# adthoms/dcora

Measured on AMD Instinct MI355X. Metric: RBCD iterations/sec, sphere2500 5-agent split, higher is better.
Workload: dtype f64

## Files before the change

### dcora_amd/__init__.py

```python
import ctypes as C
import gzip
import os
import shutil
import tempfile

import numpy as np

from . import capi
from .capi import DcoraError, Dims, ROptParams, ROptResult, RbcdOptions, F, unF, check

__all__ = ["QuadraticProblem", "QuadraticOptimizer", "ROptParameters", "Dataset", "Csr", "RbcdSession", "RaRbcdSession", "DcoraError",
           "build_Q_pgo", "dual_certificate", "is_psd", "min_eig", "fast_verification", "manifold_project",
           "device_count"]


def device_count():
    return capi.lib().dcora_device_count()


class Csr:

    def __init__(self, n, rp, ci, v):
        self.n = int(n)
        self.rp = np.ascontiguousarray(rp, dtype=np.int32)
# ... 521 lines not shown
        a = np.ascontiguousarray(agents, dtype=np.int32)
        check(capi.lib().dcora_rbcd_iterate_set(self.h, a, a.size, int(allow_adjacent)))

    def set_acceleration(self, on):
        check(capi.lib().dcora_rbcd_set_acceleration(self.h, int(bool(on))))

    def colours(self):
        col, nc = np.zeros(self.R, np.int32), C.c_int()
        check(capi.lib().dcora_rbcd_agent_colours(self.h, col, C.byref(nc)))
        return col, nc.value

    def evaluate(self):
        c2, gn, nxt = C.c_double(), C.c_double(), C.c_int()
        bn = np.zeros(self.R)
        check(capi.lib().dcora_rbcd_evaluate(self.h, C.byref(c2), C.byref(gn), bn.ctypes.data_as(C.c_void_p),
                                             C.byref(nxt)))
        return c2.value, gn.value, bn, nxt.value

    def run(self, max_iters=1000, rgrad_tol=0.1):
        it = C.c_int()
        cost, gn = np.zeros(max_iters), np.zeros(max_iters)
        sel = np.zeros(max_iters, np.int32)
        check(capi.lib().dcora_rbcd_run(self.h, max_iters, rgrad_tol, C.byref(it), cost.ctypes.data_as(C.c_void_p),
                                        gn.ctypes.data_as(C.c_void_p), sel.ctypes.data_as(C.c_void_p)))
        n = it.value
        return dict(iters=n, cost=cost[:n], gradnorm=gn[:n], selected=sel[:n])

    def run_coloured(self, max_sweeps=1000, rgrad_tol=0.1):
        return _run_coloured(capi.lib().dcora_rbcd_run_coloured, self.h, max_sweeps, rgrad_tol)

    def last_result(self):
        r = ROptResult()
        check(capi.lib().dcora_rbcd_last_result(self.h, C.byref(r)))
        return r.as_dict()

    def update_weights(self, reset_to_initial=False):
        c = np.zeros(3, np.int32)
        check(capi.lib().dcora_rbcd_update_weights(self.h, int(bool(reset_to_initial)), c.ctypes.data_as(C.c_void_p)))
        return {"accepted": int(c[0]), "rejected": int(c[1]), "undecided": int(c[2])}

    def set_weights(self, w):
        w = np.ascontiguousarray(w, np.float64)
        if w.shape != (self.m,):
            raise ValueError("set_weights needs one weight per measurement")
        check(capi.lib().dcora_rbcd_set_weights(self.h, w))

    def get_weights(self):
        w = np.zeros(self.m)
        check(capi.lib().dcora_rbcd_get_weights(self.h, w))
        return w

    def robust_info(self):
        mu, n = C.c_double(), C.c_int()
        check(capi.lib().dcora_rbcd_robust_info(self.h, C.byref(mu), C.byref(n)))
        return {"mu": mu.value, "updates": n.value}

    def X_device_ptr(self):
        p = C.c_void_p()
        check(capi.lib().dcora_rbcd_X_device_ptr(self.h, C.byref(p)))
        return p.value

    def public_count(self, agent):
        c = C.c_int()
        check(capi.lib().dcora_rbcd_public_count(self.h, agent, C.byref(c)))
        return c.value

    def public_indices(self, agent):
        idx = np.zeros(max(self.public_count(agent), 1), np.int32)
        check(capi.lib().dcora_rbcd_public_indices(self.h, agent, idx))
        return idx[:self.public_count(agent)]

    def pack_public_dev(self, agent, ptr):
        check(capi.lib().dcora_rbcd_pack_public_dev(self.h, agent, C.c_void_p(ptr)))

    def unpack_public_dev(self, agent, ptr):
        check(capi.lib().dcora_rbcd_unpack_public_dev(self.h, agent, C.c_void_p(ptr)))

    def phase_nonselected(self, selected):
        check(capi.lib().dcora_rbcd_phase_nonselected(self.h, selected))

    def phase_selected(self, selected):
        check(capi.lib().dcora_rbcd_phase_selected(self.h, selected))

    def phase_evaluate_dev(self, ptr):
        check(capi.lib().dcora_rbcd_phase_evaluate_dev(self.h, C.c_void_p(ptr)))

    def synchronize(self):
        check(capi.lib().dcora_rbcd_synchronize(self.h))

    def profile_tcg_runs(self, enable=True):
        check(capi.lib().dcora_rbcd_profile_tcg_runs(self.h, int(enable)))

    def profile_tcg_read(self):
        out = np.zeros(2)
        check(capi.lib().dcora_rbcd_profile_tcg_read(self.h, out))
        return {"launches": int(out[0]), "total_us": float(out[1])}


class Exchange:
    IPC, STAGED = 1, 2

    def __init__(self, session, job_name, _handle=None):
        self.s = session
        self.h = C.c_void_p()
        if _handle is not None:
            self.h = _handle
            return
        create = capi.lib().dcora_exchange_create_ra if isinstance(session, RaRbcdSession) else capi.lib().dcora_exchange_create
        check(create(session.h, job_name.encode(), C.byref(self.h)))

    def close(self):
        if getattr(self, "h", None):
            capi.lib().dcora_exchange_destroy(self.h)
            self.h = None

    def __del__(self):
        try:
            self.close()
        except Exception:
            pass

    def info(self):
        v = np.zeros(10)
        check(capi.lib().dcora_exchange_info(self.h, v))
        return dict(transport={1: "ipc peer stores", 2: "shared host segment"}.get(int(v[0]), "?"), mode=int(v[0]),
                    halo_finegrained=bool(v[8]), wait="device (the scatter kernel polls the flag)" if v[9] else "host spin",
                    peers=int(v[1]), posts=int(v[2]), waits=int(v[3]), bytes_posted=float(v[4]), post_s=float(v[5]),
                    wait_s=float(v[6]), eval_wait_s=float(v[7]))

    def link_report(self):
        v = np.zeros(4)
        check(capi.lib().dcora_exchange_link_report(self.h, v))
        return dict(rounds=int(v[0]), gave_up_device_wait=bool(v[1]), gave_up_ipc=bool(v[2]), last_round_us=float(v[3]))

    def all_ready(self, ready):
        out = C.c_int()
        check(capi.lib().dcora_exchange_all_ready(self.h, int(bool(ready)), C.byref(out)))
        return bool(out.value)

    def certify(self, Q, eta, k):
        cert, dist = C.c_int(), C.c_int()
        th, lm, mv = C.c_double(), C.c_double(), C.c_longlong()
        v = np.zeros(k)
        if Q is None:
            check(capi.lib().dcora_exchange_certify(self.h, k, None, None, None, eta, C.byref(cert), C.byref(th),
                                                    C.byref(lm), v, C.byref(mv), C.byref(dist)))
        else:
            check(capi.lib().dcora_exchange_certify(self.h, k, Q.rp.ctypes.data, Q.ci.ctypes.data, Q.v.ctypes.data, eta,
                                                    C.byref(cert), C.byref(th), C.byref(lm), v, C.byref(mv),
                                                    C.byref(dist)))
        return bool(cert.value), th.value, lm.value, v, mv.value, bool(dist.value)

    def post(self, agents):
        a = np.ascontiguousarray(agents, dtype=np.int32)
        check(capi.lib().dcora_exchange_post(self.h, a, a.size))

    def wait(self, agents):
        a = np.ascontiguousarray(agents, dtype=np.int32)
        check(capi.lib().dcora_exchange_wait(self.h, a, a.size))

    def _eval(self, fn, *first):
        c2, gn, nxt = C.c_double(), C.c_double(), C.c_int()
        bn = np.zeros(self.s.R)
        check(fn(self.h, *first, C.byref(c2), C.byref(gn), bn.ctypes.data_as(C.c_void_p), C.byref(nxt)))
        return c2.value, gn.value, bn, nxt.value

# ... 316 lines not shown
```

### dcora_amd/capi.py

```python
import ctypes as C
import os
import subprocess

import numpy as np

_HERE = os.path.dirname(os.path.abspath(__file__))
LIB_PATH = os.path.join(_HERE, "lib", "libdcora_hip.so")
HEADER_PATH = os.path.join(os.path.dirname(_HERE), "include", "dcora_hip.h")


class DcoraError(RuntimeError):
    def __init__(self, status, msg):
        super().__init__("dcora status %d: %s" % (status, msg))
        self.status = status


class Dims(C.Structure):
    _fields_ = [("r", C.c_int), ("d", C.c_int), ("n", C.c_int), ("l", C.c_int), ("b", C.c_int), ("layout", C.c_int)]


LAYOUT_AUTO, LAYOUT_SE, LAYOUT_RA = 0, 1, 2


class ROptParams(C.Structure):
# ... 78 lines not shown
    "dcora_csr_copy": (C.c_int, [_vp, _ip, _ip, _dp]),
    "dcora_csr_destroy": (C.c_int, [_vp]),
    "dcora_cert_dual_matrix": (C.c_int, [C.POINTER(Dims), _dp, _ip, _ip, _dp, C.c_int, C.POINTER(_vp)]),
    "dcora_cert_is_psd": (C.c_int, [C.c_int, _ip, _ip, _dp, C.c_int, _PI]),
    "dcora_cert_is_psd_device": (C.c_int, [C.c_int, _ip, _ip, _dp, C.c_int, C.c_int, _PI, _dp]),
    "dcora_chol_host_selftest": (C.c_int, [C.c_int, _ip, _ip, _dp, C.c_int, _PI, _PD, _dp]),
    "dcora_chol_cache_clear": (C.c_int, []),
    "dcora_cert_min_eig": (C.c_int, [C.c_int, _ip, _ip, _dp, C.c_int, C.c_double, C.c_int, C.c_ulonglong, C.c_int,
                                     _PD, _dp, C.POINTER(C.c_long)]),
    "dcora_cert_fast_verification": (C.c_int, [C.c_int, _ip, _ip, _dp, C.c_double, C.c_int, C.c_int, _PI, _PD, _dp,
                                               _PD]),
    "dcora_cert_lambda_min_certified": (C.c_int, [C.c_int, _ip, _ip, _dp, C.c_double, C.c_int, C.c_int, _PD, _PI]),
    "dcora_cert_suboptimality_gap": (C.c_int, [C.POINTER(Dims), _dp, C.c_double, _PD, _PD]),
    "dcora_dataset_load_g2o": (C.c_int, [C.c_char_p, C.POINTER(_vp)]),
    "dcora_dataset_create": (C.c_int, [C.c_int, C.c_int, C.c_int, _ip, _dp, C.POINTER(_vp)]),
    "dcora_dataset_info": (C.c_int, [_vp, _PI, _PI, _PI]),
    "dcora_dataset_copy": (C.c_int, [_vp, _ip, _dp]),
    "dcora_dataset_destroy": (C.c_int, [_vp]),
    "dcora_dataset_chordal_init": (C.c_int, [_vp, _dp]),
    "dcora_dataset_chordal_init_device": (C.c_int, [_vp, C.c_int, _dp]),
    "dcora_graph_build_Q_pgo": (C.c_int, [C.c_int, C.c_int, C.c_int, C.c_int, _ip, _dp, C.POINTER(_vp)]),
    "dcora_radataset_load_pyfg": (C.c_int, [C.c_char_p, C.POINTER(_vp)]),
    "dcora_radataset_info": (C.c_int, [_vp, _ip]),
    "dcora_radataset_create": (C.c_int, [C.c_int] * 5 + [_vp, _vp, C.c_int, _vp, _vp, C.c_int, _vp, _vp, _vp, C.POINTER(_vp)]),
    "dcora_radataset_copy": (C.c_int, [_vp] * 7),
    "dcora_radataset_ground_truth": (C.c_int, [_vp, _dp]),
    "dcora_radataset_build_Q": (C.c_int, [_vp, C.POINTER(_vp)]),
    "dcora_radataset_odometry_init": (C.c_int, [_vp, C.c_ulonglong, _dp]),
    "dcora_radataset_ownership": (C.c_int, [_vp, _vp, _vp, _vp]),
    "dcora_radataset_agent_columns": (C.c_int, [_vp, C.c_int, _ip, _vp, _PI]),
    "dcora_radataset_agent_colours": (C.c_int, [_vp, _ip, _PI]),
    "dcora_graph_extract_agent_blocks": (C.c_int, [C.c_int, _ip, _ip, _dp, C.c_int, _ip, C.POINTER(_vp),
                                                   C.POINTER(_vp)]),
    "dcora_radataset_destroy": (C.c_int, [_vp]),
    "dcora_graph_precond_regularization": (C.c_int, [C.c_int, _ip, _ip, _dp, C.c_int, _PD]),
    "dcora_rbcd_options_default": (None, [C.POINTER(RbcdOptions)]),
    "dcora_rbcd_create": (C.c_int, [_vp, C.POINTER(RbcdOptions), C.POINTER(_vp)]),
    "dcora_rbcd_destroy": (C.c_int, [_vp]),
    "dcora_rbcd_set_X": (C.c_int, [_vp, _dp]),
    "dcora_rbcd_get_X": (C.c_int, [_vp, _dp]),
    "dcora_rbcd_iterate": (C.c_int, [_vp, C.c_int, _PD, _PD, _vp, _PI]),
    "dcora_rbcd_run": (C.c_int, [_vp, C.c_int, C.c_double, _PI, _vp, _vp, _vp]),
    "dcora_rbcd_iterate_set": (C.c_int, [_vp, _ip, C.c_int, C.c_int]),
    "dcora_rbcd_set_acceleration": (C.c_int, [_vp, C.c_int]),
    "dcora_rbcd_agent_colours": (C.c_int, [_vp, _ip, _PI]),
    "dcora_rbcd_run_coloured": (C.c_int, [_vp, C.c_int, C.c_double, _PI, _vp, _vp]),
    "dcora_rbcd_evaluate": (C.c_int, [_vp, _PD, _PD, _vp, _PI]),
    "dcora_rbcd_agent_iterate": (C.c_int, [_vp, C.c_int, C.c_int]),
    "dcora_rbcd_agent_get_X": (C.c_int, [_vp, C.c_int, _dp]),
    "dcora_rbcd_agent_set_X": (C.c_int, [_vp, C.c_int, _dp]),
    "dcora_rbcd_agent_update_neighbor": (C.c_int, [_vp, C.c_int, C.c_int, C.c_int, _ip, _dp, C.c_int]),
    "dcora_rbcd_agent_last_skipped": (C.c_int, [_vp, C.c_int, _PI]),
    "dcora_rbcd_agent_info": (C.c_int, [_vp, C.c_int, _PI, _PI, _PI]),
    "dcora_rbcd_last_result": (C.c_int, [_vp, C.POINTER(ROptResult)]),
    "dcora_rbcd_profile_tcg_runs": (C.c_int, [_vp, C.c_int]),
    "dcora_rbcd_profile_tcg_read": (C.c_int, [_vp, _dp]),
    "dcora_rbcd_create_robust": (C.c_int, [_vp, C.POINTER(RbcdOptions), C.POINTER(RobustParams), _vp, C.POINTER(_vp)]),
    "dcora_rbcd_update_weights": (C.c_int, [_vp, C.c_int, _vp]),
    "dcora_rbcd_set_weights": (C.c_int, [_vp, _dp]),
    "dcora_rbcd_get_weights": (C.c_int, [_vp, _dp]),
    "dcora_rbcd_robust_info": (C.c_int, [_vp, _PD, _PI]),
    "dcora_rbcd_create_robust_ranks": (C.c_int, [_vp, C.POINTER(RbcdOptions), C.POINTER(RobustParams), _vp, C.c_char_p,
                                                 C.POINTER(_vp), C.POINTER(_vp)]),
    "dcora_team_params_default": (None, [C.POINTER(TeamParams)]),
    "dcora_team_ready_to_terminate": (C.c_int, [C.POINTER(TeamParams), C.c_int, C.c_int, C.c_int, C.c_double, C.c_int,
                                                C.c_int, C.c_int, _PI]),
    "dcora_team_decide": (C.c_int, [C.POINTER(TeamParams), C.c_int, C.c_int, C.c_int, C.c_int, C.c_int,
                                    C.POINTER(AgentStatus), _vp, _vp, C.c_int, _PI, _PI]),
    "dcora_max_translation_distance": (C.c_int, [C.c_int, C.c_int, C.c_int, _dp, _dp, _PD]),
    "dcora_rbcd_team_enable": (C.c_int, [_vp, C.POINTER(TeamParams)]),
    "dcora_rbcd_agent_status": (C.c_int, [_vp, C.c_int, C.POINTER(AgentStatus), _PI]),
    "dcora_rbcd_loop_closure_stats": (C.c_int, [_vp, C.c_int, _ip]),
    "dcora_rbcd_should_terminate": (C.c_int, [_vp, _PI]),
    "dcora_rbcd_should_update_weights": (C.c_int, [_vp, _PI]),
    "dcora_rbcd_team_info": (C.c_int, [_vp, _ip]),
    "dcora_rbcd_run_team": (C.c_int, [_vp, _PI, _vp, _vp, _vp, _vp, _PI, _PI]),
    "dcora_rbcd_X_device_ptr": (C.c_int, [_vp, C.POINTER(_vp)]),
    "dcora_rbcd_public_count": (C.c_int, [_vp, C.c_int, _PI]),
    "dcora_rbcd_public_indices": (C.c_int, [_vp, C.c_int, _ip]),
    "dcora_rbcd_pack_public_dev": (C.c_int, [_vp, C.c_int, _vp]),
    "dcora_rbcd_unpack_public_dev": (C.c_int, [_vp, C.c_int, _vp]),
    "dcora_rbcd_phase_nonselected": (C.c_int, [_vp, C.c_int]),
    "dcora_rbcd_phase_selected": (C.c_int, [_vp, C.c_int]),
    "dcora_rbcd_phase_evaluate_dev": (C.c_int, [_vp, _vp]),
    "dcora_rbcd_synchronize": (C.c_int, [_vp]),
    "dcora_exchange_create": (C.c_int, [_vp, C.c_char_p, C.POINTER(_vp)]),
    "dcora_exchange_destroy": (C.c_int, [_vp]),
    "dcora_exchange_create_ra": (C.c_int, [_vp, C.c_char_p, C.POINTER(_vp)]),
    "dcora_exchange_info": (C.c_int, [_vp, _dp]),
    "dcora_exchange_link_report": (C.c_int, [_vp, _dp]),
    "dcora_exchange_post": (C.c_int, [_vp, _ip, C.c_int]),
    "dcora_exchange_wait": (C.c_int, [_vp, _ip, C.c_int]),
    "dcora_exchange_evaluate": (C.c_int, [_vp, _PD, _PD, _vp, _PI]),
    "dcora_exchange_rbcd_iterate": (C.c_int, [_vp, C.c_int, _PD, _PD, _vp, _PI]),
    "dcora_exchange_rbcd_tick": (C.c_int, [_vp, _ip, C.c_int, C.c_int]),
    "dcora_exchange_run_coloured": (C.c_int, [_vp, C.c_int, C.c_double, _PI, _vp, _vp]),
    "dcora_exchange_set_X": (C.c_int, [_vp, _dp]),
    "dcora_exchange_gather_X": (C.c_int, [_vp, _dp]),
    "dcora_exchange_barrier": (C.c_int, [_vp]),
    "dcora_exchange_all_ready": (C.c_int, [_vp, C.c_int, _PI]),
    "dcora_exchange_update_weights": (C.c_int, [_vp, C.c_int, _vp]),
    "dcora_exchange_set_weights": (C.c_int, [_vp, _dp]),
    "dcora_exchange_get_weights": (C.c_int, [_vp, _dp]),
    "dcora_exchange_certify": (C.c_int, [_vp, C.c_int, _vp, _vp, _vp, C.c_double, _PI, _PD, _PD, _dp,
                                         C.POINTER(C.c_longlong), _PI]),
    "dcora_exchange_host_selftest": (C.c_int, [C.c_char_p, C.c_int, C.c_int, C.c_int, C.c_int, _PD]),
    "dcora_debug_exchange_leave_stale": (C.c_int, [C.c_char_p, C.c_int, C.c_int]),
    "dcora_debug_exchange_probe_fault": (C.c_int, [C.c_int]),
    "dcora_cert_prepare": (C.c_int, [C.POINTER(Dims), _ip, _ip, C.c_int, C.c_int]),
    "dcora_debug_tcg_run_fault": (C.c_int, [C.c_int]),
    "dcora_debug_tcg_run_fault_at": (C.c_int, [C.c_int, C.c_int]),
    "dcora_problem_solver_info": (C.c_int, [_vp, _dp]),
    "dcora_ra_rbcd_create": (C.c_int, [_vp, C.POINTER(RbcdOptions), C.POINTER(_vp)]),
    "dcora_ra_rbcd_destroy": (C.c_int, [_vp]),
    "dcora_ra_rbcd_info": (C.c_int, [_vp, _PI, _vp]),
    "dcora_ra_rbcd_set_X": (C.c_int, [_vp, _dp]),
    "dcora_ra_rbcd_get_X": (C.c_int, [_vp, _dp]),
    "dcora_ra_rbcd_iterate": (C.c_int, [_vp, C.c_int, _PD, _PD, _vp, _PI]),
    "dcora_ra_rbcd_evaluate": (C.c_int, [_vp, _PD, _PD, _vp, _PI]),
    "dcora_ra_rbcd_run": (C.c_int, [_vp, C.c_int, C.c_double, _PI, _vp, _vp, _vp]),
    "dcora_ra_rbcd_iterate_set": (C.c_int, [_vp, _ip, C.c_int, C.c_int]),
    "dcora_ra_rbcd_set_acceleration": (C.c_int, [_vp, C.c_int]),
    "dcora_ra_rbcd_agent_colours": (C.c_int, [_vp, _ip, _PI]),
    "dcora_ra_rbcd_run_coloured": (C.c_int, [_vp, C.c_int, C.c_double, _PI, _vp, _vp]),
    "dcora_ra_rbcd_last_result": (C.c_int, [_vp, C.POINTER(ROptResult)]),
    "dcora_problem_time_qapply": (C.c_int, [_vp, C.c_int, _PD, _PD]),
    "dcora_problem_time_qapply_rotating": (C.c_int, [C.POINTER(_vp), C.c_int, C.c_int, _PD]),
    "dcora_problem_qapply_info": (C.c_int, [_vp, _dp]),
    "dcora_problem_time_precond": (C.c_int, [_vp, C.c_int, _PD, _PD]),
    "dcora_problem_precond_info": (C.c_int, [_vp, _dp]),
    "dcora_precond_cache_info": (C.c_int, [_dp]),
    "dcora_precond_cache_clear": (C.c_int, []),
    "dcora_robust_params_default": (None, [C.POINTER(RobustParams)]),
    "dcora_robust_weights": (C.c_int, [C.POINTER(RobustParams), C.c_int, C.c_int, _dp, _dp]),
    "dcora_chi2inv": (C.c_int, [C.c_double, C.c_int, _PD]),
    "dcora_robust_error_threshold_at_quantile": (C.c_int, [C.c_double, C.c_int, _PD]),
    "dcora_robust_single_rotation_averaging": (C.c_int, [C.c_int, C.c_int, _dp, _vp, C.c_double, _dp, _ip]),
    "dcora_robust_single_pose_averaging": (C.c_int, [C.c_int, C.c_int, _dp, _dp, _vp, _vp, C.c_double, _dp, _dp, _ip]),
    "dcora_agent_neighbor_transforms": (C.c_int, [C.c_int, C.c_int, _ip, _dp, _dp, _dp, _dp, _dp]),
    "dcora_agent_robust_neighbor_transform": (C.c_int, [C.c_int, C.c_int, _dp, C.c_int, C.c_int, _dp, _PI, _PI]),
    "dcora_log_trajectory": (C.c_int, [C.c_char_p, C.c_int, C.c_int, _dp]),
    "dcora_fixed_stiefel_variable": (C.c_int, [C.c_int, C.c_int, _dp]),
    "dcora_agent_initialize_in_global_frame": (C.c_int, [C.POINTER(Dims), _dp, _dp, _dp, _dp]),
    "dcora_measurement_errors": (C.c_int, [_vp, C.c_int, _dp, _dp, C.c_int]),
    "dcora_solve_pgo": (C.c_int, [_vp, C.POINTER(ROptParams), _vp, _dp, C.POINTER(ROptResult), C.c_int]),
    "dcora_solve_robust_pgo": (C.c_int, [_vp, C.POINTER(ROptParams), C.POINTER(RobustParams), _vp, _vp, _dp, _vp,
                                         C.c_int]),
    "dcora_round_align_trajectory": (C.c_int, [C.POINTER(Dims), _dp, _vp, C.c_int, _dp, _vp, _vp, C.c_int]),
    "dcora_round_project_solution_raslam": (C.c_int, [C.POINTER(Dims), _dp, _dp, C.c_int]),
}

_lib = None


def lib():
    global _lib
    if _lib is None:
        if not os.path.exists(LIB_PATH):
            raise DcoraError(-1, "libdcora_hip.so is not built (run __graft_entry__.build()); there is no fallback")
        L = C.CDLL(LIB_PATH)
        for name, (res, args) in SIGNATURES.items():
            fn = getattr(L, name)
            fn.restype = res
            fn.argtypes = args
        _lib = L
    return _lib
# ... 26 lines not shown
```

### dcora_amd/csrc/capi.hip

```cpp
#include <cstdio>
#include <cstring>
#include <new>

#include "../../include/dcora_hip.h"
#include "cert.h"
#include "device_chol.h"
#include "device_problem.h"
#include "host_graph.h"
#include "host_threads.h"
#include "ra_rbcd.h"
#include "rbcd.h"
#include "precond_cache.h"
#include "exchange.h"
#include "host_robust.h"
#include "robust.h"
#include "round.h"

namespace dcora {
const std::string &get_last_error();
}
using namespace dcora;

struct dcora_problem_s {
  DeviceProblem p;
// ... 1137 lines not shown
    const int rc = team_session(s);
    if (rc) return rc;
    if (!agent_ok(s, agent)) return bad("bad agent");
    for (int c = 0; c < 3; ++c) counts[c] = s->s.team->lc[(size_t)agent * 3 + c];
    return (int)DCORA_OK;
  });
}
int dcora_rbcd_should_terminate(dcora_rbcd_t s, int *yes) {
  return abi_call({s, yes}, [&] {
    const int rc = team_session(s);
    return rc ? rc : s->s.team_decide(yes, nullptr);
  });
}
int dcora_rbcd_should_update_weights(dcora_rbcd_t s, int *yes) {
  return abi_call({s, yes}, [&] {
    const int rc = team_session(s);
    return rc ? rc : s->s.team_decide(nullptr, yes);
  });
}
int dcora_rbcd_team_info(dcora_rbcd_t s, int info[4]) {
  return abi_call({s, info}, [&] {
    const int rc = team_session(s);
    if (rc) return rc;
    info[0] = s->s.team_inner_iter();
    info[1] = s->s.team->latest_weight_update_iteration;
    info[2] = s->s.team_weight_updates();
    info[3] = s->s.team->resets_done;
    return (int)DCORA_OK;
  });
}
int dcora_rbcd_run_team(dcora_rbcd_t s, int *iters_done, double *cost2_trace, double *gradnorm_trace,
                        int *selected_trace, int *updated_trace, int *weight_updates, int *stop_reason) {
  return abi_call({s}, [&] {
    const int rc = team_session(s);
    return rc ? rc
              : s->s.run_team(iters_done, cost2_trace, gradnorm_trace, selected_trace, updated_trace, weight_updates,
                              stop_reason);
  });
}
int dcora_rbcd_last_result(dcora_rbcd_t s, dcora_ropt_result *res) {
  return abi_call({s, res}, [&] { return s->s.last_result(res); });
}
int dcora_rbcd_X_device_ptr(dcora_rbcd_t s, double **X_dev) {
  return abi_call({s, X_dev}, [&] {
    *X_dev = s->s.Xg.p;
    return DCORA_OK;
  });
}
int dcora_rbcd_public_count(dcora_rbcd_t s, int agent, int *count) {
  return abi_call({s, count}, [&] {
    if (!agent_ok(s, agent)) return bad("bad agent");
    *count = (int)s->s.agents[agent].public_poses.size();
    return (int)DCORA_OK;
  });
}
int dcora_rbcd_public_indices(dcora_rbcd_t s, int agent, int *idx) {
  return abi_call({s, idx}, [&] {
    if (!agent_ok(s, agent)) return bad("bad agent");
    const auto &v = s->s.agents[agent].public_poses;
    std::copy(v.begin(), v.end(), idx);
    return (int)DCORA_OK;
  });
}
int dcora_rbcd_pack_public_dev(dcora_rbcd_t s, int agent, double *packed_dev) {
  return abi_call({s}, [&] {
    if (!agent_ok(s, agent)) return bad("bad agent");
    if (!packed_dev && !s->s.agents[agent].public_poses.empty()) return bad("null argument");
    return s->s.pack_public(agent, packed_dev);
  });
}
int dcora_rbcd_unpack_public_dev(dcora_rbcd_t s, int agent, const double *packed_dev) {
  return abi_call({s}, [&] {
    if (!agent_ok(s, agent)) return bad("bad agent");
    if (!packed_dev && !s->s.agents[agent].public_poses.empty()) return bad("null argument");
    return s->s.unpack_public(agent, packed_dev);
  });
}
int dcora_rbcd_phase_nonselected(dcora_rbcd_t s, int selected) {
  return abi_call({s}, [&] { return s->s.phase_nonselected(selected); });
}
int dcora_rbcd_phase_selected(dcora_rbcd_t s, int selected) {
  return abi_call({s}, [&] { return s->s.phase_selected(selected); });
}
int dcora_rbcd_phase_evaluate_dev(dcora_rbcd_t s, double *out_dev) {
  return abi_call({s, out_dev}, [&] { return s->s.phase_evaluate_dev(out_dev); });
}
int dcora_rbcd_profile_tcg_runs(dcora_rbcd_t s, int enable) {
  return abi_call({s}, [&] {
    for (auto &a : s->s.agents)
      if (a.prob) a.prob->profile_tcg_runs = enable != 0;
    return DCORA_OK;
  });
}
int dcora_rbcd_profile_tcg_read(dcora_rbcd_t s, double *out2) {
  return abi_call({s, out2}, [&] {
    out2[0] = out2[1] = 0;
    for (auto &a : s->s.agents) {
      if (!a.prob) continue;
      double n = 0, us = 0;
      const int rc = a.prob->profile_tcg_read(&n, &us);
      if (rc) return rc;
      out2[0] += n;
      out2[1] += us;
    }
    return (int)DCORA_OK;
  });
}
int dcora_rbcd_synchronize(dcora_rbcd_t s) {
  return abi_call({s}, [&]() -> int {
    DCORA_HIP(hipStreamSynchronize(s->s.st));
    return DCORA_OK;
  });
}

int dcora_exchange_create(dcora_rbcd_t s, const char *job_name, dcora_exchange_t *out) {
  return abi_call({s, job_name, out}, [&] {
    return create(out, [&](dcora_exchange_s &h) { return h.e.init(&s->s, job_name); });
  });
}
int dcora_exchange_destroy(dcora_exchange_t ex) {
  delete ex;
  return DCORA_OK;
}
int dcora_exchange_info(dcora_exchange_t ex, double *info) {
  return abi_call({ex, info}, [&] {
    const Exchange &e = ex->e;
    info[0] = e.mode;
    info[1] = e.num_peers();
    info[2] = (double)e.posts;
    info[3] = (double)e.waits;
    info[4] = e.bytes_posted;
    info[5] = e.post_s;
    info[6] = e.wait_s;
    info[7] = e.eval_wait_s;
    info[8] = e.halo_is_finegrained() ? 1 : 0;
    info[9] = e.waits_on_device() ? 1 : 0;
    return DCORA_OK;
  });
}
int dcora_debug_exchange_probe_fault(int rounds) {
  g_probe_fault_rounds.store(rounds);
  return DCORA_OK;
}
int dcora_exchange_link_report(dcora_exchange_t ex, double *out4) {
  return abi_call({ex, out4}, [&] {
    const Exchange &e = ex->e;
    out4[0] = e.link_rounds;
    out4[1] = e.link_gave_up_device_wait;
    out4[2] = e.link_gave_up_ipc;
    out4[3] = e.link_last_us;
    return DCORA_OK;
  });
}
int dcora_exchange_post(dcora_exchange_t ex, const int *agents, int count) {
  return abi_call({ex}, [&] { return !agents && count > 0 ? bad("null argument") : ex->e.post(agents, count); });
}
int dcora_exchange_wait(dcora_exchange_t ex, const int *agents, int count) {
  return abi_call({ex}, [&] { return !agents && count > 0 ? bad("null argument") : ex->e.wait(agents, count); });
}
int dcora_exchange_evaluate(dcora_exchange_t ex, double *cost2, double *gradnorm, double *block_norms,
                            int *next_selected) {
  return abi_call({ex}, [&] { return ex->e.evaluate(cost2, gradnorm, block_norms, next_selected); });
}
int dcora_exchange_rbcd_iterate(dcora_exchange_t ex, int selected, double *cost2, double *gradnorm,
                                double *block_norms, int *next_selected) {
  return abi_call({ex}, [&] { return ex->e.rbcd_iterate(selected, cost2, gradnorm, block_norms, next_selected); });
// ... 454 lines not shown
```

### dcora_amd/csrc/device_problem.h

```cpp
#pragma once
#include <hip/hip_runtime.h>

#include <functional>
#include <memory>
#include <string>
#include <vector>

#include "../../include/dcora_hip.h"
#include "host_sparse.h"
#include "kernels.h"
#include "sparse_precond.h"

namespace dcora {

void set_last_error(const std::string &s);
int hip_fail(hipError_t e, const char *what, const char *file, int line);
#define DCORA_HIP(call)                                                        \
  do {                                                                         \
    hipError_t e_ = (call);                                                    \
    if (e_ != hipSuccess) return ::dcora::hip_fail(e_, #call, __FILE__, __LINE__); \
  } while (0)

template <class T>
struct DevBuf {
// ... 84 lines not shown

struct SpImage {
  int k = 0, npieces = 0;
  long nnzL = 0, nmwaves_total = 0;
  double weights_per_apply = 0, rows_total = 0;
  std::vector<SpLevel> levels;
  DevBuf<double> vals;
  DevBuf<int> idxs, perm, out_off;
  DevBuf<MWave> mwaves;
  int nhub = 0;
  long hub_nnz = 0;
  DevBuf<int> hub_idx;
  DevBuf<double> hub_U, hub_Sinv;
  DevBuf<int> in_pos, out_pos;
  int upload(const PartInvHost &P, struct DeviceWeightSink *streamed = nullptr);
  size_t device_bytes() const;
};

struct DeviceWeightSink : WeightSink {
  explicit DeviceWeightSink(int device_) : device(device_) {}
  ~DeviceWeightSink() override;
  bool fill_on_device(const std::vector<partinv::Fill> &fills, long long total, const std::vector<MirrorRange> &mirrors,
                      int nthreads) override;
  bool wants_device_sources() const override;
  bool begin(long long total) override;
  long long chunk_cap() const override { return kChunk; }
  double *acquire(long long n) override;
  bool commit(long long off, long long n) override;
  bool end() override;
  static constexpr long long kChunk = 8ll << 20;
  static constexpr int kBuffers = 3;
  int device;
  DevBuf<double> vals;
  hipStream_t st = nullptr;
  double *pin[kBuffers] = {nullptr, nullptr, nullptr};
  hipEvent_t ev[kBuffers] = {nullptr, nullptr, nullptr};
  bool busy[kBuffers] = {false, false, false};
  int cur = -1;
};

class SparsePrecond {
 public:
  std::shared_ptr<const SpImage> im;
  int rcap = 0;
  DevBuf<double> y, hub_w, hub_x2;
  double weights_per_apply = 0;
  bool foldable() const { return im && im->nhub == 0 && im->in_pos.p != nullptr; }
  SpFold fold() const {
    SpFold f;
    if (foldable()) {
      f.y = y.p;
      f.in_pos = im->in_pos.p;
      f.out_pos = im->out_pos.p;
    }
    return f;
  }
  SpFold fold_generic() const;
  int attach(std::shared_ptr<const SpImage> image, int rcap);
  int launches() const { return (int)im->levels.size() + 2; }
  void apply(hipStream_t st, int r, Buf2 R, double *Z, Gate g, bool levels_only = false,
             const std::function<bool()> *after_first = nullptr) const;
  double bytes_per_apply(int r) const;
};

int stream_acquire(int device, hipStream_t *out);
void stream_release(int device, hipStream_t st);
int host_flags_acquire(HostFlags **host, HostFlags **dev, int *slot);
void host_flags_release(HostFlags *host, int slot);

int precond_prebuild_dense(const std::vector<const HostCsr *> &Qs, double reg, int block, int device);

class DeviceProblem {
 public:
  ManiDesc m{};
  int device = 0;
  hipStream_t st = nullptr;
  bool own_stream = false;
  DevCsr Q;
  DevBsr Qb;
  bool has_bsr = false;
  int enq_qapply(Buf2 X, int selX, const double *Gp, Buf2 Y, int selY, double *partials, Gate g);
  DevBuf<double> G;
  bool has_G = false;
  DevBuf<double> Minv;
  int ldm = 0;
  SparsePrecond sp;
  std::shared_ptr<const DevBuf<double>> Minv_shared;
  bool precond_cache_hit = false;
  bool sparse_precond = false;
  bool has_precond = false;
  double precond_setup_ms = 0;
  long precond_nnzL = 0;

  DevBuf<double> X0, X1, EG0, EG1, RG0, RG1, S0, S1;
  DevBuf<double> delta, eta, Heta, res, z, Hd, W, Zt;
  DevBuf<double> delta2, res2, Zpart;
  bool tcg_run_ok = false;
  bool concurrent_solves = false;
  DevBuf<unsigned> tcg_sync;
  bool profile_tcg_runs = false;
  std::vector<hipEvent_t> run_events;
  size_t run_events_used = 0;
  int profile_tcg_read(double *launches, double *total_us);
  bool fused = false;
  bool group = false;
  DevBuf<double> pA, pB, pC, p1, p2, p3, scal;
  DevBuf<SolverCtl> ctl;
  DevBuf<double> arena;
  int hf_slot = -1;
  HostFlags *hf = nullptr;
  HostFlags *hf_dev = nullptr;
  std::vector<double> stage;

  long nelem() const { return (long)m.r * m.k; }
  Buf2 Xb() const { return Buf2{{X0.p, X1.p}}; }
  Buf2 EGb() const { return Buf2{{EG0.p, EG1.p}}; }
  Buf2 RGb() const { return Buf2{{RG0.p, RG1.p}}; }
  Buf2 Sb() const { return Buf2{{S0.p, S1.p}}; }

  ~DeviceProblem();
  int init(const dcora_dims &dims, const HostCsr &Qh, const double *Gh, double reg, int device_, hipStream_t shared);
  int set_G_host(const double *Gh);
  int build_preconditioner(const HostCsr &Qh, double reg);
  int set_values(const HostCsr &Q_on_pattern, hipStream_t stream, std::vector<double> *stage);

  int npA() const { return has_bsr ? spmm_bsr_grid(m.n) : spmm_grid(m.k, m.r) + Q.n_long; }
  int npPose() const { return pose_grid(m); }
  int enq_rgrad(Buf2 X, Buf2 EG, Buf2 RG, Buf2 S, int sel, double *partials, Gate g, double *posenorm = nullptr);
  int enq_retract(Buf2 X, const double *V, double alpha, Buf2 out, int selOut, Buf2 grad, const double *HV,
                  double *partials, Gate g);
  int npVec() const { return vec_grid(nelem()); }
  void enqueue_egrad(const double *X, double *EG, double *partials);
  void enqueue_precond(const double *X, const double *V, double *out);
  void enq_minv(Buf2 R, double *Z, const double *p2, int np2, Gate g);

  int cost(const double *Xh, double *f);
  int eucgrad(const double *Xh, double *out);
  int riegrad(const double *Xh, double *out, double *norm);
  int hessvec(const double *Xh, const double *Vh, double *out);
  int hessvec_solver_form(const double *Xh, const double *Vh, double *out, double *dots);
  bool hess_one_launch() const;
  int precondition(const double *Xh, const double *Vh, double *out);
  int retract(const double *Xh, const double *Vh, double *out);
  int tangent_project(const double *Xh, const double *Vh, double *out);
  int optimize(const dcora_ropt_params &prm, const double *X0h, double *Xout, dcora_ropt_result *res);
  int escape_saddle(const double *Xopt, double theta, const double *v, double gtol, double pgtol, bool second_order,
                    double *Xout, int *success);

  int optimize_dev(const dcora_ropt_params &prm);
  int fetch_result(dcora_ropt_result *res);
  Buf2 result_pick(const SolverCtl **c) const;
  int result(double **X);
  int eval_dev(const double *Xd, double *f, double *gradnorm);

  int time_qapply(int reps, double *avg_ms, double *bytes);
  int time_precond(int reps, double *avg_ms, double *bytes);
  bool use_pc() const;

 private:
  enum class TcgForm { generic, split, pc, run };
  struct RtrForm;
  int rtr_dev(const dcora_ropt_params &prm, TcgForm form);
  int rgd_dev(const dcora_ropt_params &prm);
  int seq_ = 0;
  bool pending_ = false;
  bool rgd_ = false;
  double t0_ms_ = 0;
  dcora_ropt_result last_res_{};
  int cur_after_fetch_ = 0;
  int upload(const double *h, double *d, size_t n);
  int download(const double *d, double *h, size_t n);
};

}
```

### dcora_amd/csrc/device_problem.hip

```cpp
#include <atomic>

#include "device_problem.h"
#include "env.h"
#include "device_chol.h"
#include "host_threads.h"
#include "precond_cache.h"

#include <algorithm>
#include <chrono>
#include <cmath>
#include <cstdio>
#include <cstdlib>
#include <cstring>
#include <map>
#include <mutex>

namespace dcora {

static thread_local std::string g_last_error;
void set_last_error(const std::string &s) { g_last_error = s; }
const std::string &get_last_error() { return g_last_error; }
int hip_fail(hipError_t e, const char *what, const char *file, int line) {
  char buf[512];
  std::snprintf(buf, sizeof buf, "HIP error %d (%s) at %s:%d in %s", (int)e, hipGetErrorString(e), file, line, what);
// ... 546 lines not shown
  for (double &v : neg) v = -v;
  rc = upload(neg.data(), z.p, nelem());
  if (rc) return rc;
  rc = upload(Vh, delta2.p, nelem());
  if (rc) return rc;
  enqueue_egrad(X0.p, EG0.p, nullptr);
  launch_rgrad(st, m, buf1(X0.p), buf1(EG0.p), buf1(RG0.p), buf1(S0.p), 0, pB.p, Gate{});
  DCORA_HIP(hipMemsetAsync(p3.p, 0, sizeof(double), st));
  const int np = launch_spmm_dir_fix(st, m, Q.view(), buf1(X0.p), buf1(S0.p), z.p, delta2.p, delta.p, Hd.p, p3.p, 1, p1.p,
                                     ctl.p, 0, 0);
  std::vector<double> part((size_t)np);
  rc = download(p1.p, part.data(), part.size());
  if (rc) return rc;
  dots[0] = 0;
  for (double v : part) dots[0] += v;
  rc = download(Hd.p, out, nelem());
  if (rc) return rc;
  launch_spmm(st, m.r, Q.view(), buf1(delta.p), 0, nullptr, buf1(W.p), 0, nullptr, Gate{});
  launch_hessfix(st, m, buf1(X0.p), buf1(S0.p), delta.p, W.p, Hd.p, p1.p, Gate{});
  part.assign((size_t)npPose(), 0.0);
  rc = download(p1.p, part.data(), part.size());
  if (rc) return rc;
  dots[1] = 0;
  for (double v : part) dots[1] += v;
  return DCORA_OK;
}
int DeviceProblem::precondition(const double *Xh, const double *Vh, double *out) {
  if (!has_precond) {
    set_last_error("problem has no preconditioner");
    return DCORA_ERR_NO_PRECONDITIONER;
  }
  DCORA_HIP(hipSetDevice(device));
  int rc = upload(Xh, X0.p, nelem());
  if (rc) return rc;
  rc = upload(Vh, res.p, nelem());
  if (rc) return rc;
  enqueue_precond(X0.p, res.p, z.p);
  return download(z.p, out, nelem());
}
int DeviceProblem::retract(const double *Xh, const double *Vh, double *out) {
  DCORA_HIP(hipSetDevice(device));
  int rc = upload(Xh, X0.p, nelem());
  if (rc) return rc;
  rc = upload(Vh, eta.p, nelem());
  if (rc) return rc;
  launch_retract(st, m, buf1(X0.p), eta.p, 1.0, buf1(X1.p), 0, buf1(RG0.p), nullptr, nullptr, Gate{});
  return download(X1.p, out, nelem());
}
int DeviceProblem::tangent_project(const double *Xh, const double *Vh, double *out) {
  DCORA_HIP(hipSetDevice(device));
  int rc = upload(Xh, X0.p, nelem());
  if (rc) return rc;
  rc = upload(Vh, eta.p, nelem());
  if (rc) return rc;
  launch_tangent(st, m, buf1(X0.p), eta.p, z.p, nullptr, nullptr, nullptr, 0, nullptr, nullptr, 0, 0, 0);
  return download(z.p, out, nelem());
}

int DeviceProblem::eval_dev(const double *Xd, double *f, double *gradnorm) {
  enqueue_egrad(Xd, EG1.p, pA.p);
  launch_rgrad(st, m, buf1(Xd), buf1(EG1.p), Buf2{{nullptr, nullptr}}, Buf2{{nullptr, nullptr}}, 0, pB.p, Gate{});
  launch_sum_partials(st, pA.p, npA(), 2, 2, scal.p);
  launch_sum_partials(st, pB.p, npPose(), 1, 1, scal.p + 2);
  double s[3];
  int rc = download(scal.p, s, 3);
  if (rc) return rc;
  if (f) *f = 0.5 * s[0] + s[1];
  if (gradnorm) *gradnorm = std::sqrt(s[2]);
  return DCORA_OK;
}

int DeviceProblem::optimize(const dcora_ropt_params &prm, const double *X0h, double *Xout, dcora_ropt_result *res_out) {
  DCORA_HIP(hipSetDevice(device));
  int rc = upload(X0h, X0.p, nelem());
  if (rc) return rc;
  double *X = nullptr;
  if ((rc = optimize_dev(prm)) || (rc = result(&X)) || (rc = fetch_result(res_out))) return rc;
  return download(X, Xout, nelem());
}

int DeviceProblem::optimize_dev(const dcora_ropt_params &prm) {
  pending_ = false;
  rgd_ = prm.method != 0;
  if (rgd_) return rgd_dev(prm);
  if (!has_precond) {
    set_last_error("RTR requires the preconditioner (ref src/QuadraticProblem.cpp:78-82)");
    return DCORA_ERR_NO_PRECONDITIONER;
  }
  TcgForm form = TcgForm::generic;
  if (fused) form = !use_pc() ? TcgForm::split : (tcg_run_ok && !concurrent_solves) ? TcgForm::run : TcgForm::pc;
  return rtr_dev(prm, form);
}

int DeviceProblem::fetch_result(dcora_ropt_result *res_out) {
  if (pending_) {
    SolverCtl h;
    DCORA_HIP(hipMemcpyAsync(&h, ctl.p, sizeof h, hipMemcpyDeviceToHost, st));
    DCORA_HIP(hipStreamSynchronize(st));
    DCORA_HIP(hipGetLastError());
    const double now = std::chrono::duration<double, std::milli>(std::chrono::steady_clock::now().time_since_epoch())
                           .count();
    cur_after_fetch_ = h.cur & 1;
    last_res_.success = 1;
    last_res_.fInit = h.fInit;
    last_res_.gradNormInit = h.gradNormInit;
    last_res_.fOpt = h.f1;
    last_res_.gradNormOpt = h.ngf;
    last_res_.elapsedMs = now - t0_ms_;
    last_res_.tCGStatus = h.tcg_status;
    last_res_.outer_iterations = h.outer_it;
    last_res_.inner_iterations = h.inner_total;
    last_res_.accepted_steps = h.accepted;
    pending_ = false;
  }
  if (res_out) *res_out = last_res_;
  return DCORA_OK;
}

Buf2 DeviceProblem::result_pick(const SolverCtl **c) const {
  *c = rgd_ ? nullptr : ctl.p;
  return rgd_ ? buf1(X1.p) : Xb();
}

int DeviceProblem::result(double **X) {
  const int rc = fetch_result(nullptr);
  if (rc) return rc;
  *X = cur_after_fetch_ ? X1.p : X0.p;
  return DCORA_OK;
}

int DeviceProblem::rgd_dev(const dcora_ropt_params &prm) {
  const auto t0 = std::chrono::steady_clock::now();
  double f0 = 0, g0 = 0;
  int rc = eval_dev(X0.p, &f0, &g0);
  if (rc) return rc;
  enqueue_egrad(X0.p, EG0.p, nullptr);
  launch_rgrad(st, m, buf1(X0.p), buf1(EG0.p), buf1(RG0.p), buf1(S0.p), 0, pB.p, Gate{});
  const double *dir = RG0.p;
  if (prm.RGD_use_preconditioner) {
    if (!has_precond) {
      set_last_error("RGD with preconditioning requested but the problem has none");
      return DCORA_ERR_NO_PRECONDITIONER;
    }
    enqueue_precond(X0.p, RG0.p, z.p);
    dir = z.p;
  }
  launch_retract(st, m, buf1(X0.p), dir, -prm.RGD_stepsize, buf1(X1.p), 0, buf1(RG0.p), nullptr, nullptr, Gate{});
  double f1 = 0, g1 = 0;
  rc = eval_dev(X1.p, &f1, &g1);
  if (rc) return rc;
  last_res_.success = 1;
  last_res_.fInit = f0;
  last_res_.gradNormInit = g0;
  last_res_.fOpt = f1;
  last_res_.gradNormOpt = g1;
  last_res_.elapsedMs = std::chrono::duration<double, std::milli>(std::chrono::steady_clock::now() - t0).count();
  last_res_.tCGStatus = TR_MAXITER;
  last_res_.outer_iterations = 1;
  last_res_.inner_iterations = 0;
  last_res_.accepted_steps = 1;
  cur_after_fetch_ = 1;
  return DCORA_OK;
}

namespace {
template <class Pred>
bool spin_until(Pred p, double timeout_s) {
  const auto t0 = std::chrono::steady_clock::now();
  unsigned it = 0;
  while (!p()) {
    if ((++it & 1023u) == 0) {
      if (std::chrono::duration<double>(std::chrono::steady_clock::now() - t0).count() > timeout_s) return false;
    }
// ... 1 lines not shown
    __builtin_ia32_pause();
#endif
  }
  return true;
}
}

int DeviceProblem::profile_tcg_read(double *launches, double *total_us) {
  DCORA_HIP(hipSetDevice(device));
  DCORA_HIP(hipStreamSynchronize(st));
  double us = 0;
  for (size_t i = 0; i + 1 < run_events_used; i += 2) {
    float ms = 0;
    if (hipEventElapsedTime(&ms, run_events[i], run_events[i + 1]) == hipSuccess) us += 1e3 * ms;
  }
  *launches = (double)(run_events_used / 2);
  *total_us = us;
  run_events_used = 0;
  return DCORA_OK;
}

bool DeviceProblem::use_pc() const {
  const int forced = env::solver_bc();
  if (sparse_precond || !has_precond) return false;
  if (forced < 0) return false;
  if (!forced && !fused_pc_preferred(m, ldm)) return false;
  return fused_pc_ready(m, ldm);
}

struct DeviceProblem::RtrForm {
  DeviceProblem &p;
  TcgForm form;
  int &seq;
  const int solve_first;
  SolverCtl *const c;
  const CsrDev Qv;
  const BsrDev Qbv;
  const double *const Gp;
  const long N;
  const int nA, nP, nV, nPB;
  const bool sparse;
  const SpFold sfg;
  const bool hess_fused;
  const int nPG;
  const double *const Mi;
  const bool folded;
  const SpFold sf;
  const int nsl;
  const int nZ;
  const bool gf, gfb;
  unsigned *const sync_p;
  const int nsync;
  double *const dbuf[2];
  double *const rbuf[2];

  RtrForm(DeviceProblem &p_, TcgForm f, int &seq_)
      : p(p_), form(f), seq(seq_), solve_first(seq_ + 1), c(p.ctl.p), Qv(p.Q.view()),
        Qbv(p.has_bsr ? p.Qb.view() : BsrDev{}), Gp(p.has_G ? p.G.p : nullptr), N(p.nelem()), nA(p.npA()),
        nP(p.npPose()), nV(p.npVec()), nPB(fused_pose_blocks(p.m)), sparse(p.sparse_precond),
        sfg(f == TcgForm::generic && sparse ? p.sp.fold_generic() : SpFold()),
        hess_fused(f == TcgForm::generic && p.hess_one_launch()),
        nPG(sparse ? fused_update_grid(p.m) : fused_precond_grid(p.m)), Mi(sparse ? nullptr : p.Minv.p),
        folded(sparse && p.sp.foldable()), sf(folded ? p.sp.fold() : SpFold{}), nsl(sparse ? 1 : -1),
        nZ(f == TcgForm::pc || f == TcgForm::run ? fused_pc_blocks(p.m) : nPB),
        gf(f != TcgForm::generic && !p.has_bsr && p.Q.n_long == 0), gfb(f != TcgForm::generic && p.has_bsr),
        sync_p(f == TcgForm::run ? p.tcg_sync.p : nullptr), nsync(f == TcgForm::run ? tcg_run_sync_words() : 0),
        dbuf{p.delta.p, p.delta2.p}, rbuf{p.res.p, p.res2.p} {}

  bool outer_done() const { return p.hf->outer_done_seq >= solve_first; }
  bool stopped(int tcg_first) const { return p.hf->tcg_done_seq >= tcg_first || outer_done(); }
  int nAe() const { return gf ? nPB : nA; }

  int eval(int sel) {
    const auto g = [&] {
      ++seq;
      return sel ? Gate{c, seq, 1} : Gate{};
    };
    const Buf2 kNoBuf{{nullptr, nullptr}};
    if (form == TcgForm::generic) {
      p.enq_qapply(p.Xb(), sel, Gp, p.EGb(), sel, p.pA.p, g());
      launch_rgrad(p.st, p.m, p.Xb(), p.EGb(), p.RGb(), p.Sb(), sel, p.pB.p, g());
      return nP;
    }
    if (gf) return launch_fused_grad(p.st, p.m, Qv, p.Xb(), Gp, p.EGb(), p.RGb(), p.Sb(), sel, p.pA.p, p.pB.p, nullptr, g());
    if (gfb)
      return launch_fused_grad_bsr(p.st, p.m.r, p.m.d, Qbv, p.Xb(), Gp, kNoBuf, p.RGb(), p.Sb(), sel, p.pA.p, p.pB.p,
                                   nullptr, g());
    p.enq_qapply(p.Xb(), sel, Gp, p.EGb(), sel, p.pA.p, g());
    return p.enq_rgrad(p.Xb(), p.EGb(), p.RGb(), p.Sb(), sel, p.pB.p, g());
  }

  int first() {
    switch (form) {
      case TcgForm::generic: {
        launch_tcg_begin(p.st, N, p.RGb(), p.eta.p, p.Heta.p, p.res.p, c, ++seq);
        const int s = seq;
        p.enq_minv(buf1(p.res.p), p.Zt.p, nullptr, 0, Gate{c, ++seq, 1});
        launch_tangent(p.st, p.m, p.Xb(), p.Zt.p, p.z.p, p.res.p, p.p3.p, nullptr, 0, c, p.hf_dev, ++seq, 1, 0);
        return s;
      }
      case TcgForm::run: {
        const int s = launch_run();
        if (s != 0) return s;
        p.tcg_run_ok = false;
        form = TcgForm::pc;
      }
        [[fallthrough]];
      case TcgForm::pc:
        if (launch_fused_pc(p.st, p.m, p.ldm, Mi, p.RGb(), p.Xb(), nullptr, nullptr, p.eta.p, p.Heta.p, nullptr, rbuf[0],
                            p.z.p, nullptr, 0, p.p3.p, c, p.hf_dev, ++seq, 0, 1) < 0) {
          set_last_error("k_fused_pc could not be launched on this device");
          return -1;
        }
        return seq;
      case TcgForm::split:
        launch_fused_precond(p.st, p.m, p.ldm, Mi, p.RGb(), nullptr, nullptr, p.eta.p, p.Heta.p, nullptr, rbuf[0],
                             p.Zpart.p, nullptr, 0, p.p2.p, c, p.hf_dev, ++seq, 0, 1, sf);
        return seq;
    }
    return -1;
  }
  int launch_run() {
    hipEvent_t e1 = nullptr;
    if (p.profile_tcg_runs) {
      while (p.run_events.size() < p.run_events_used + 2) {
        hipEvent_t e = nullptr;
        if (hipEventCreate(&e) != hipSuccess) {
          set_last_error("hipEventCreate failed (k_tcg_run profile)");
          return -1;
        }
        p.run_events.push_back(e);
      }
      (void)hipEventRecord(p.run_events[p.run_events_used], p.st);
      e1 = p.run_events[p.run_events_used + 1];
      p.run_events_used += 2;
    }
    if (launch_tcg_run(p.st, p.m, p.ldm, Mi, Qv, p.RGb(), p.Xb(), p.Sb(), dbuf[0], dbuf[1], p.Hd.p, p.eta.p, p.Heta.p,
                       p.z.p, p.p1.p, p.p3.p, p.pC.p, p.tcg_sync.p, c, p.hf_dev, ++seq) < 0) {
      if (e1) p.run_events_used -= 2;
      return 0;
    }
    if (e1) (void)hipEventRecord(e1, p.st);
    return seq;
  }
  void rest(bool rejected) {
    if (form != TcgForm::split) return;
    if (sparse && rejected) {
      launch_fused_finish(p.st, p.m, p.Xb(), p.W.p, rbuf[0], p.z.p, nullptr, 0, p.p3.p, c, p.hf_dev, ++seq, 0, 1, 1,
                          SpFold{});
      return;
    }
    if (sparse) p.sp.apply(p.st, p.m.r, buf1(rbuf[0]), p.Zpart.p, Gate{c, ++seq, 1}, folded);
    launch_fused_finish(p.st, p.m, p.Xb(), p.Zpart.p, rbuf[0], p.z.p, nullptr, 0, p.p3.p, c, p.hf_dev, ++seq, 0, 1, nsl,
                        sf, sparse ? p.W.p : nullptr);
  }

  int replay(Buf2 R, double *Z, bool levels_only, int tcg_first) {
    const int seq_step = seq;
    bool timed = false;
    const std::function<bool()> verdict = [&]() {
      if (!spin_until([&] { return p.hf->go_seq >= seq_step || stopped(tcg_first); }, 20.0)) {
        timed = true;
        return false;
      }
      return !stopped(tcg_first);
    };
    p.sp.apply(p.st, p.m.r, R, Z, Gate{c, ++seq, 2}, levels_only, &verdict);
// ... 276 lines not shown
```

### dcora_amd/csrc/env.cpp

```cpp
#include "env.h"

#include <cstdlib>
#include <cstring>

namespace dcora {
namespace env {
namespace {
bool is(const char *name, const char *value) {
  const char *e = std::getenv(name);
  return e && std::strcmp(e, value) == 0;
}
}

bool init_timing() {
  static const bool v = std::getenv("DCORA_INIT_TIMING") != nullptr;
  return v;
}
int precond_mode() {
  return is("DCORA_PRECOND", "dense") ? 1 : is("DCORA_PRECOND", "sparse") ? 2 : 0;
}
bool generic_solver() {
  return is("DCORA_SOLVER", "generic");
}
int solver_tcg() {
  return is("DCORA_SOLVER_TCG", "launch") ? -1 : is("DCORA_SOLVER_TCG", "run") ? 1 : 0;
}
int solver_bc() {
  static const int v = is("DCORA_SOLVER_BC", "pc") ? 1 : is("DCORA_SOLVER_BC", "split") ? -1 : 0;
  return v;
}
bool factor_on_host() {
  static const bool v = is("DCORA_FACTOR", "host");
  return v;
}
bool fill_on_host() {
  static const bool v = is("DCORA_SP_FILL", "host");
  return v;
}
bool lanczos_sync() {
  static const bool v = is("DCORA_LANCZOS", "sync");
  return v;
}
int host_threads() {
  static const int v = [] {
    const char *e = std::getenv("DCORA_HOST_THREADS");
    return e ? (std::atoi(e) > 0 ? std::atoi(e) : 1) : 0;
  }();
  return v;
}
double precond_cache_mb() {
  static const double v = [] {
    const char *e = std::getenv("DCORA_PRECOND_CACHE_MB");
    return e ? std::atof(e) : 8192.0;
  }();
  return v;
}
const char *exchange() {
  static const char *v = std::getenv("DCORA_EXCHANGE");
  return v;
}
const char *exchange_wait() {
  static const char *v = std::getenv("DCORA_EXCHANGE_WAIT");
  return v;
}
double exchange_timeout_s() {
  static const double v = [] {
    const char *e = std::getenv("DCORA_EXCHANGE_TIMEOUT_S");
    const double x = e ? std::atof(e) : 0.0;
    return x > 0 ? x : 120.0;
  }();
  return v;
}

}
}
```

### dcora_amd/csrc/env.h

```cpp
#pragma once

namespace dcora {
namespace env {

bool init_timing();
int precond_mode();
bool generic_solver();
int solver_tcg();
int solver_bc();
bool factor_on_host();
bool fill_on_host();
bool lanczos_sync();
int host_threads();
double precond_cache_mb();
const char *exchange();
const char *exchange_wait();
double exchange_timeout_s();

}
}
```

### dcora_amd/csrc/kernels.h

```cpp
#pragma once
#include <hip/hip_runtime.h>

#include <atomic>
#include <climits>
#include <vector>

namespace dcora {

constexpr int kMaxPartials = 1024;
constexpr int kBsrMaxGrid = 4096;
constexpr int kBlock = 256;

struct ManiDesc {
  int r, d, n, l, b, k, se;
  __host__ __device__ int rot_col(int i) const { return se ? i * (d + 1) : i * d; }
  __host__ __device__ int sphere_col(int i) const { return d * n + i; }
  __host__ __device__ int num_euc() const { return se ? n : n + b; }
  __host__ __device__ int euc_col(int e) const { return se ? e * (d + 1) + d : d * n + l + e; }
};
inline ManiDesc make_mani(int r, int d, int n, int l, int b, int layout = 0) {
  ManiDesc m;
  m.r = r; m.d = d; m.n = n; m.l = l; m.b = b;
  m.se = (layout == 2) ? 0 : ((l == 0 && b == 0) ? 1 : 0);
  m.k = (d + 1) * n + l + b;
  return m;
}
template <class Dims>
inline ManiDesc make_mani(const Dims &dims) {
  return make_mani(dims.r, dims.d, dims.n, dims.l, dims.b, dims.layout);
}

constexpr int kLongSplit = 8;
constexpr int kLongRow = 512;
struct CsrDev {
  int nrows = 0;
  int nnz = 0;
  const int *rp = nullptr;
  const int *ci = nullptr;
  const double *v = nullptr;
  int n_long = 0;
  const int *long_rows = nullptr;
  double *long_part = nullptr;
  int *long_cnt = nullptr;
};

struct BsrDev {
  int nbrows = 0;
  int nblocks = 0;
  const int *bp = nullptr;
  const int *bc = nullptr;
  const double *bv = nullptr;
};

struct Buf2 {
  double *p[2];
};
inline Buf2 buf1(double *x) { return Buf2{{x, x}}; }
inline Buf2 buf1(const double *x) { return Buf2{{const_cast<double *>(x), const_cast<double *>(x)}}; }

struct SolverCtl {
  double f1, ngf, Delta, maxDelta, tol, f2, rho, fInit, gradNormInit;
  int cur;
  int outer_it, max_outer, accepted, last_accepted, stop_on_accept;
  int outer_done_stamp;
  double z_r[2], d_Pd[2], e_Pe[2], e_Pd[2];
  double alpha, e_Pe_n, norm_r0;
  int tcg_done_stamp, tcg_status, tcg_iters, inner_total, max_inner;
};
enum TcgStatus : int { TR_NEGCURVTURE = 0, TR_EXCREGION = 1, TR_LCON = 2, TR_SCON = 3, TR_MAXITER = 4 };
constexpr int kMaxAgents = 64;
struct EvalOut {
  double cost2, gradnorm;
  double block_norms[kMaxAgents];
  int next;
  volatile int seq;
};
struct HostFlags {
  volatile int last_seq_done;
  volatile int tcg_done_seq;
  volatile int outer_done_seq;
  volatile int go_seq;
  volatile int reject_seq;
  volatile int tcg_abort_seq;
};

struct Gate {
  const SolverCtl *ctl = nullptr;
  int seq = 0;
  int gate = 0;
};

int spmm_grid(int nrows, int r);
int spmm_dir_fix_grid(const ManiDesc &m, int nrows);
int launch_spmm_dir_fix(hipStream_t st, const ManiDesc &m, const CsrDev &A, Buf2 X, Buf2 Sblk, const double *z,
                        const double *d_old, double *d_new, double *Hd, const double *p3, int np3, double *p1,
                        SolverCtl *ctl, int seq, int iter);
void launch_spmm_dir(hipStream_t st, int r, const CsrDev &A, const double *z, const double *d_old, double *d_new,
                     double *W, const double *p3, int np3, SolverCtl *ctl, int seq, int iter);
inline int spmm_slots(const CsrDev &A, int r) { return spmm_grid(A.nrows, r) + A.n_long; }
void launch_spmm(hipStream_t st, int r, const CsrDev &A, Buf2 X, int selX, const double *G, Buf2 Y, int selY,
                 double *partials, Gate g);

int spmm_bsr_grid(int nbrows);
void launch_spmm_bsr(hipStream_t st, int r, int d, const BsrDev &A, Buf2 X, int selX, const double *G, Buf2 Y,
                     int selY, double *partials, Gate g);

int pose_grid(const ManiDesc &m);
void launch_rgrad(hipStream_t st, const ManiDesc &m, Buf2 X, Buf2 EG, Buf2 RG, Buf2 Sblk, int sel,
                  double *partials, Gate g);
struct SpFold {
  double *y = nullptr;
  const int *in_pos = nullptr, *out_pos = nullptr;
  int h = 0;
  const int *hub_idx = nullptr;
  const double *hub_U = nullptr, *hub_x2 = nullptr;
};
void launch_tangent(hipStream_t st, const ManiDesc &m, Buf2 X, const double *V, double *out, const double *R,
                    double *partials, const double *p2, int np2, SolverCtl *ctl, HostFlags *hf, int seq,
                    int gate, int iter, SpFold sf = SpFold());
void launch_hessfix(hipStream_t st, const ManiDesc &m, Buf2 X, Buf2 Sblk, const double *V, const double *W,
                    double *HV, double *partials, Gate g);
void launch_retract(hipStream_t st, const ManiDesc &m, Buf2 X, const double *V, double alpha, Buf2 out,
                    int selOut, Buf2 grad, const double *HV, double *partials, Gate g);
void launch_polar(hipStream_t st, const ManiDesc &m, double c0, const double *A, double c1, const double *B,
                  double c2, const double *C, double *out);

void launch_nesterov(hipStream_t st, const ManiDesc &m, int mode, int restart, int skip_lo, int skip_hi, double alpha,
                     double gamma, double *X, double *V, double *Y, double *XPrev, double *Yloc,
                     const double *Xloc);

void launch_dense_apply(hipStream_t st, int r, int k, int ldm, const double *Minv, Buf2 R, double *Z,
                        const double *p2, int np2, Gate g);

int vec_grid(long nelem);
struct CtlInit {
  int enable = 0;
  double tol = 0, Delta = 0, maxDelta = 0;
  int max_outer = 0, stop_on_accept = 0, max_inner = 0;
};
void launch_rtr_init(hipStream_t st, const double *pA, int npA, const double *pB, int npB, SolverCtl *ctl,
                     HostFlags *hf, int seq, CtlInit ci = CtlInit(), unsigned *tcg_sync = nullptr, int nsync = 0);
void launch_tcg_begin(hipStream_t st, long nelem, Buf2 grad, double *eta, double *Heta, double *res,
                      SolverCtl *ctl, int seq);
void launch_tcg_update1(hipStream_t st, long nelem, const double *delta, const double *Hd, double *eta,
                        double *Heta, double *res, const double *p1, int np1, double *p2, SolverCtl *ctl,
                        HostFlags *hf, int seq, int iter, int r = 1, SpFold sf = SpFold());
void launch_tcg_update2(hipStream_t st, long nelem, const double *z, double *delta, const double *p3, int np3,
                        SolverCtl *ctl, HostFlags *hf, int seq, int iter);
void launch_rtr_decide(hipStream_t st, const double *pA, int npA, const double *pB, int npB, const double *pC,
                       int npC, SolverCtl *ctl, HostFlags *hf, int seq, unsigned *tcg_sync = nullptr, int nsync = 0);

void launch_axpby(hipStream_t st, long nelem, double a, const double *x, double b, const double *y, double *out);
void launch_sum_partials(hipStream_t st, const double *partials, int np, int stride, int count, double *out);
void launch_dot(hipStream_t st, long nelem, const double *x, const double *y, double *partials);
void launch_gather_cols(hipStream_t st, int r, int ncols, const int *src_col, const double *X, double *out);
void launch_scatter_cols(hipStream_t st, int r, int ncols, const int *dst_col, const double *in, double *X);
void launch_block_dots(hipStream_t st, int r, int nagents, const int *col_start, const double *A, const double *B,
                       double *out);

void launch_lambda_blocks(hipStream_t st, const ManiDesc &m, const double *X, const double *XQ, double *Lblk);
void launch_lanczos_proj(hipStream_t st, int n, int nv, const double *V, const double *w, double *partials);
void launch_lanczos_sub(hipStream_t st, int n, int nv, const double *V, const double *h, double *w);
constexpr int kLanczosFuseParts = 256;
void launch_lanczos_sub_sum(hipStream_t st, int n, int nv, const double *V, const double *partials, int npart,
                            double *hout, double *w, double *dotpart);
void launch_lanczos_keep(hipStream_t st, int nv, const double *h, double *hout);
constexpr double kLanczosDead = 1e-10;
void launch_lanczos_next(hipStream_t st, int n, const double *partials, int npart, double *beta_out, int *flag,
                         const double *w, double *vnext, const double *hrow, int nv);
void launch_scale_shift(hipStream_t st, int n, double shift, const double *x, double *y);
void launch_scale(hipStream_t st, int n, const double *alpha_dev_inv_sqrt ,
                  const double *w, double *out);

bool fused_supported(const ManiDesc &m);
bool group_supported(const ManiDesc &m);
int fused_pose_blocks(const ManiDesc &m);
int fused_nsplit(const ManiDesc &m);
int fused_precond_grid(const ManiDesc &m);
int fused_update_grid(const ManiDesc &m);
int launch_fused_hess(hipStream_t st, const ManiDesc &m, const CsrDev &Q, const double *z, const double *d_old,
                       double *d_new, Buf2 X, Buf2 S, double *Hd, const double *p3, int np3, double *p1,
                       SolverCtl *ctl, int seq, int iter,
                      const BsrDev *Ab = nullptr );
void launch_fused_precond(hipStream_t st, const ManiDesc &m, int ldm, const double *Minv, Buf2 grad,
                          const double *delta, const double *Hd, double *eta, double *Heta, const double *res_old,
                          double *res_new, double *Zpart, const double *p1, int np1, double *p2, SolverCtl *ctl,
                          HostFlags *hf, int seq, int iter, int first, SpFold sf = SpFold());
int fused_pc_blocks(const ManiDesc &m);
bool tcg_run_supported(const ManiDesc &m, int ldm, int cus, int max_rows_nnz);
int tcg_run_sync_words();
extern std::atomic<int> g_tcg_run_fault;
extern std::atomic<int> g_tcg_run_fault_skip;
int tcg_run_max_rows_nnz(const ManiDesc &m, const int *rowptr);
int launch_tcg_run(hipStream_t st, const ManiDesc &m, int ldm, const double *Minv, const CsrDev &Q, Buf2 grad, Buf2 X,
                   Buf2 S, double *d0, double *d1, double *Hd, double *eta, double *Heta, double *z, double *p1r,
                   double *p3, double *pC, unsigned *sync, SolverCtl *ctl, HostFlags *hf, int seq);
bool fused_pc_preferred(const ManiDesc &m, int ldm);
bool fused_pc_ready(const ManiDesc &m, int ldm);
int launch_fused_pc(hipStream_t st, const ManiDesc &m, int ldm, const double *Minv, Buf2 grad, Buf2 X,
                    const double *delta, const double *Hd, double *eta, double *Heta, const double *res_old,
                    double *res_new, double *z, const double *p1, int np1, double *p3, SolverCtl *ctl, HostFlags *hf,
                    int seq, int iter, int first, double *pC = nullptr );
void launch_fused_finish(hipStream_t st, const ManiDesc &m, Buf2 X, const double *Zpart, const double *res,
                         double *z, const double *p2, int np2, double *p3, SolverCtl *ctl, HostFlags *hf, int seq,
                         int iter, int first, int nsplit = -1 , SpFold sf = SpFold(),
                         double *zraw = nullptr );
int launch_fused_grad_bsr(hipStream_t st, int r, int d, const BsrDev &A, Buf2 X, const double *G, Buf2 EG, Buf2 RG, Buf2 S,
                          int sel, double *pA, double *pB, double *posenorm, Gate g,
                          const int *agent_start = nullptr, int agents = 0, int *wg_per_agent = nullptr);
int launch_fused_grad(hipStream_t st, const ManiDesc &m, const CsrDev &Q, Buf2 X, const double *G, Buf2 EG, Buf2 RG,
                      Buf2 Sblk, int sel, double *pA, double *pB, double *posenorm, Gate g);
int launch_g_rgrad(hipStream_t st, const ManiDesc &m, Buf2 X, Buf2 EG, Buf2 RG, Buf2 Sblk, int sel, double *partials,
                   double *posenorm, Gate g);
void launch_ctl_init(hipStream_t st, SolverCtl *c, double tol, double Delta, double maxDelta, int max_outer,
                     int stop_on_accept, int max_inner);
void launch_eval_finish(hipStream_t st, int R, const int *pose_start, const double *posenorm, const double *pA,
                        int npA, EvalOut *out_dev, int seq, double *split_scratch = nullptr, int nposes = 0,
                        const double *agent_partials = nullptr, int wg_per_agent = 0);
int eval_split_doubles();
struct RelChangeSet {
  int count;
  int agent[kMaxAgents];
};
void launch_rel_change(hipStream_t st, int r, int d, const double *X, const double *XPrev, const int *pose_start,
                       const RelChangeSet &set, double *out);
int max_translation_distance(int r, int d, int n, const double *X, const double *Y, double *out);
int launch_g_retract(hipStream_t st, const ManiDesc &m, Buf2 X, const double *V, double alpha, Buf2 out, int selOut,
                     Buf2 grad, const double *HV, double *partials, Gate g);
void launch_g_nesterov(hipStream_t st, const ManiDesc &m, int mode, int restart, int skip_lo, int skip_hi,
                       double alpha, double gamma, double *X, double *V, double *Y, double *XPrev, double *Yloc,
                       Buf2 Xloc, const SolverCtl *ctl, double *inner_Yloc = nullptr);

#if defined(__HIPCC__)
template <int CTRL>
__device__ __forceinline__ double dpp_move(double v) {
  int lo = __double2loint(v), hi = __double2hiint(v);
  lo = __builtin_amdgcn_update_dpp(0, lo, CTRL, 0xF, 0xF, true);
  hi = __builtin_amdgcn_update_dpp(0, hi, CTRL, 0xF, 0xF, true);
  return __hiloint2double(hi, lo);
}
__device__ __forceinline__ double readlane_f64(double v, int lane) {
  const int lo = __builtin_amdgcn_readlane(__double2loint(v), lane);
  const int hi = __builtin_amdgcn_readlane(__double2hiint(v), lane);
  return __hiloint2double(hi, lo);
}
__device__ __forceinline__ double wave_sum_dpp(double v) {
  v += dpp_move<0xB1>(v);
  v += dpp_move<0x4E>(v);
  v += dpp_move<0x141>(v);
  v += dpp_move<0x140>(v);
  return (readlane_f64(v, 0) + readlane_f64(v, 16)) + (readlane_f64(v, 32) + readlane_f64(v, 48));
}
__device__ __forceinline__ double wave_sum(double v) { return wave_sum_dpp(v); }
__device__ __forceinline__ double block_sum(double v, double *sm) {
  v = wave_sum(v);
  const int w = threadIdx.x >> 6, nw = (blockDim.x + 63) >> 6;
  __syncthreads();
  if ((threadIdx.x & 63) == 0) sm[w] = v;
  __syncthreads();
  double t = 0;
  for (int i = 0; i < nw; ++i) t += sm[i];
  return t;
}
__device__ __forceinline__ double sum_partials(const double *p, int np, int stride, int off, double *sm) {
  double v = 0;
  for (int i = threadIdx.x; i < np; i += blockDim.x) v += p[(size_t)i * stride + off];
  return block_sum(v, sm);
}
__device__ __forceinline__ void host_store(volatile int *p, int v) {
  __hip_atomic_store(const_cast<int *>(p), v, __ATOMIC_RELAXED, __HIP_MEMORY_SCOPE_SYSTEM);
}

__device__ __forceinline__ bool gated(const SolverCtl *ctl, int seq, int gate) {
  if (ctl == nullptr || gate == 0) return false;
  if (seq > ctl->outer_done_stamp) return true;
  if (gate == 2 && seq > ctl->tcg_done_stamp) return true;
  return false;
}
struct GateWords {
  int outer, tcg;
};
__device__ __forceinline__ GateWords gate_words(const SolverCtl *ctl) {
  GateWords w{0x7fffffff, 0x7fffffff};
  if (ctl) {
    w.outer = ctl->outer_done_stamp;
    w.tcg = ctl->tcg_done_stamp;
  }
  return w;
}
__device__ __forceinline__ bool gated(const GateWords &w, const SolverCtl *ctl, int seq, int gate) {
  if (ctl == nullptr || gate == 0) return false;
  if (seq > w.outer) return true;
  if (gate == 2 && seq > w.tcg) return true;
  return false;
// ... 8 lines not shown
```

### dcora_amd/csrc/kernels.hip

```cpp
#include "kernels.h"
#include "tcg_rules.h"

namespace dcora {

template <int N>
__device__ __forceinline__ void sum_partials_n(const double *const (&p)[N], const int (&np)[N], const int (&st)[N],
                                               const int (&off)[N], double *sm, double (&out)[N]) {
  double v[N];
#pragma unroll
  for (int q = 0; q < N; ++q) v[q] = ((int)threadIdx.x < np[q]) ? p[q][(size_t)threadIdx.x * st[q] + off[q]] : 0.0;
#pragma unroll
  for (int q = 0; q < N; ++q)
    for (int i = threadIdx.x + blockDim.x; i < np[q]; i += blockDim.x) v[q] += p[q][(size_t)i * st[q] + off[q]];
#pragma unroll
  for (int q = 0; q < N; ++q) v[q] = wave_sum(v[q]);
  const int w = threadIdx.x >> 6, nw = (blockDim.x + 63) >> 6;
  __syncthreads();
  if ((threadIdx.x & 63) == 0)
#pragma unroll
    for (int q = 0; q < N; ++q) sm[q * 4 + w] = v[q];
  __syncthreads();
#pragma unroll
  for (int q = 0; q < N; ++q) {
    double t = 0;
    for (int i = 0; i < nw; ++i) t += sm[q * 4 + i];
    out[q] = t;
  }
}

int vec_grid(long nelem) {
  long g = (nelem + kBlock - 1) / kBlock;
  if (g < 1) g = 1;
  if (g > kMaxPartials) g = kMaxPartials;
  return (int)g;
}

constexpr int kSpmmTile = 1536;

int spmm_grid(int nrows, int r) {
  const int RB = kBlock / r;
  long nrb = (nrows + RB - 1) / RB;
  if (nrb < 1) nrb = 1;
  if (nrb > kMaxPartials) nrb = kMaxPartials;
  return (int)nrb;
}

template <bool DOTS>
__global__ __launch_bounds__(kBlock) void k_spmm(int r, CsrDev A, Buf2 Xb, int selX, const double *__restrict__ G,
                                                 Buf2 Yb, int selY, double *__restrict__ partials, Gate g,
                                                 int main_grid) {
  if (gated(g.ctl, g.seq, g.gate)) return;
  __shared__ int s_ci[kSpmmTile];
  __shared__ double s_v[kSpmmTile];
  __shared__ double s_red[16];
  const double *__restrict__ X = pick(Xb, g.ctl, selX);
  double *__restrict__ Y = pick(Yb, g.ctl, selY);
  const int RB = kBlock / r;
  const int nrb = (A.nrows + RB - 1) / RB;
  const int lj = threadIdx.x / r, t = threadIdx.x - lj * r;
  double d0 = 0, d1 = 0;
  if ((int)blockIdx.x >= main_grid) {
    const int li = ((int)blockIdx.x - main_grid) / kLongSplit, sl = ((int)blockIdx.x - main_grid) % kLongSplit;
    const int j = A.long_rows[li];
    const int rb0 = A.rp[j], re0 = A.rp[j + 1];
    const int per = (re0 - rb0 + kLongSplit - 1) / kLongSplit;
    const int pb = rb0 + sl * per, pe = min(re0, pb + per);
    double acc = 0;
    if (lj < RB) {
      for (int p = pb + lj; p < pe; p += 8 * RB) {
        int c8[8];
        double w8[8], x8[8];
#pragma unroll
        for (int q = 0; q < 8; ++q) {
          const int pp = p + q * RB;
          const bool ok = pp < pe;
          c8[q] = A.ci[ok ? pp : rb0];
          w8[q] = ok ? A.v[pp] : 0.0;
        }
#pragma unroll
        for (int q = 0; q < 8; ++q) x8[q] = X[(size_t)c8[q] * r + t];
#pragma unroll
        for (int q = 0; q < 8; ++q) acc += w8[q] * x8[q];
      }
    }
    double *s_part = s_v;
    __shared__ int s_last;
    __syncthreads();
    s_part[threadIdx.x] = (lj < RB) ? acc : 0.0;
    __syncthreads();
    if ((int)threadIdx.x < r) {
      double y = 0;
      for (int q = 0; q < RB; ++q) y += s_part[q * r + threadIdx.x];
      __hip_atomic_store(A.long_part + ((size_t)li * kLongSplit + sl) * 16 + threadIdx.x, y, __ATOMIC_RELAXED,
                         __HIP_MEMORY_SCOPE_AGENT);
    }
    __threadfence();
    __syncthreads();
    if (threadIdx.x == 0)
      s_last = (__hip_atomic_fetch_add(A.long_cnt + li, 1, __ATOMIC_ACQ_REL, __HIP_MEMORY_SCOPE_AGENT) ==
                kLongSplit - 1);
    __syncthreads();
    if (!s_last) return;
    if (threadIdx.x == 0) __hip_atomic_store(A.long_cnt + li, 0, __ATOMIC_RELAXED, __HIP_MEMORY_SCOPE_AGENT);
    if ((int)threadIdx.x < r) {
      double y = 0;
      for (int q = 0; q < kLongSplit; ++q)
        y += __hip_atomic_load(A.long_part + ((size_t)li * kLongSplit + q) * 16 + threadIdx.x, __ATOMIC_RELAXED,
                               __HIP_MEMORY_SCOPE_AGENT);
      const size_t o = (size_t)j * r + threadIdx.x;
      if (DOTS) {
        const double x = X[o];
        d0 = y * x;
        if (G) d1 = x * G[o];
      }
      if (G) y += G[o];
      Y[o] = y;
    }
    if (DOTS) {
      const double a = block_sum(d0, s_red);
      const double b = block_sum(d1, s_red);
// ... 396 lines not shown
      kind = (a < D) ? 0 : 2;
    } else if (active && !m.se && j < n_rot_rows + m.l) {
      kind = 1;
      it = j - n_rot_rows;
    }
    __syncthreads();
    s_V[threadIdx.x] = own;
    s_Y[threadIdx.x] = xo;
    __syncthreads();
    double T = acc;
    const int l0 = lj - a;
    if (kind == 0) {
      double sres = 0;
#pragma unroll
      for (int b = 0; b < D; ++b) sres += s_V[(l0 + b) * r + t] * Sblk[(size_t)it * D * D + b + a * D];
      T = acc - sres;
    } else if (kind == 1) {
      T = acc - own * Sblk[(size_t)m.n * D * D + it];
    }
    s_T[threadIdx.x] = T;
    __syncthreads();
    double hv = T;
    if (kind == 0) {
      double sres = 0;
#pragma unroll
      for (int b = 0; b < D; ++b) {
        double pba = 0, pab = 0;
        for (int u = 0; u < r; ++u) {
          pba += s_Y[(l0 + b) * r + u] * s_T[(l0 + a) * r + u];
          pab += s_Y[(l0 + a) * r + u] * s_T[(l0 + b) * r + u];
        }
        sres += s_Y[(l0 + b) * r + t] * (0.5 * (pba + pab));
      }
      hv = T - sres;
    } else if (kind == 1) {
      double yt = 0;
      for (int u = 0; u < r; ++u) yt += s_Y[lj * r + u] * s_T[lj * r + u];
      hv = T - xo * yt;
    }
    if (active && !is_long) {
      Hd[o] = hv;
      d_new[o] = own;
      dacc += own * hv;
    }
  }
  const double tot = block_sum(dacc, s_red);
  if (threadIdx.x == 0) p1[blockIdx.x] = tot;
}

int spmm_dir_fix_grid(const ManiDesc &m, int nrows) {
  const int al = m.se ? m.d + 1 : m.d;
  const int RB = ((kBlock / m.r) / al) * al;
  if (RB < al) return 0;
  long nrb = (nrows + RB - 1) / RB;
  if (nrb < 1) nrb = 1;
  if (nrb > kMaxPartials) nrb = kMaxPartials;
  return (int)nrb;
}

int launch_spmm_dir_fix(hipStream_t st, const ManiDesc &m, const CsrDev &A, Buf2 X, Buf2 Sblk, const double *z,
                        const double *d_old, double *d_new, double *Hd, const double *p3, int np3, double *p1,
                        SolverCtl *ctl, int seq, int iter) {
  const int main_grid = spmm_dir_fix_grid(m, A.nrows);
  const int grid = main_grid + A.n_long * kLongSplit;
  if (m.d == 3)
    hipLaunchKernelGGL(k_spmm_dir_fix<3>, dim3(grid), dim3(kBlock), 0, st, m, A, X, Sblk, z, d_old, d_new, Hd, p3, np3,
                       p1, ctl, seq, iter, main_grid);
  else
    hipLaunchKernelGGL(k_spmm_dir_fix<2>, dim3(grid), dim3(kBlock), 0, st, m, A, X, Sblk, z, d_old, d_new, Hd, p3, np3,
                       p1, ctl, seq, iter, main_grid);
  return main_grid + A.n_long;
}

void launch_spmm_dir(hipStream_t st, int r, const CsrDev &A, const double *z, const double *d_old, double *d_new,
                     double *W, const double *p3, int np3, SolverCtl *ctl, int seq, int iter) {
  const int main_grid = spmm_grid(A.nrows, r);
  const int grid = main_grid + A.n_long * kLongSplit;
  hipLaunchKernelGGL(k_spmm_dir, dim3(grid), dim3(kBlock), 0, st, r, A, z, d_old, d_new, W, p3, np3, ctl, seq, iter,
                     main_grid);
}

void launch_spmm(hipStream_t st, int r, const CsrDev &A, Buf2 X, int selX, const double *G, Buf2 Y, int selY,
                 double *partials, Gate g) {
  const int main_grid = spmm_grid(A.nrows, r);
  const int grid = main_grid + A.n_long * kLongSplit;
  if (partials)
    hipLaunchKernelGGL(k_spmm<true>, dim3(grid), dim3(kBlock), 0, st, r, A, X, selX, G, Y, selY, partials, g,
                       main_grid);
  else
    hipLaunchKernelGGL(k_spmm<false>, dim3(grid), dim3(kBlock), 0, st, r, A, X, selX, G, Y, selY, partials, g,
                       main_grid);
}

template <int D, int RM>
struct Blk {
  double a[D][RM];
};
template <int D, int RM>
__device__ __forceinline__ void ld_blk(const double *__restrict__ p, int r, Blk<D, RM> &B) {
#pragma unroll
  for (int c = 0; c < D; ++c)
#pragma unroll
    for (int t = 0; t < RM; ++t) B.a[c][t] = (t < r) ? p[c * r + t] : 0.0;
}
template <int D, int RM>
__device__ __forceinline__ void st_blk(double *__restrict__ p, int r, const Blk<D, RM> &B) {
#pragma unroll
  for (int c = 0; c < D; ++c)
#pragma unroll
    for (int t = 0; t < RM; ++t)
      if (t < r) p[c * r + t] = B.a[c][t];
}
template <int D, int RM>
__device__ __forceinline__ void sym_gram(const Blk<D, RM> &Y, const Blk<D, RM> &E, double (&S)[D][D]) {
  double P[D][D];
#pragma unroll
  for (int a = 0; a < D; ++a)
#pragma unroll
    for (int b = 0; b < D; ++b) {
      double s = 0;
#pragma unroll
      for (int t = 0; t < RM; ++t) s += Y.a[a][t] * E.a[b][t];
      P[a][b] = s;
    }
#pragma unroll
  for (int a = 0; a < D; ++a)
#pragma unroll
    for (int b = 0; b < D; ++b) S[a][b] = 0.5 * (P[a][b] + P[b][a]);
}
template <int D, int RM>
__device__ __forceinline__ void sub_AS(Blk<D, RM> &V, const Blk<D, RM> &A, const double (&S)[D][D]) {
#pragma unroll
  for (int b = 0; b < D; ++b)
#pragma unroll
    for (int t = 0; t < RM; ++t) {
      double s = 0;
#pragma unroll
      for (int a = 0; a < D; ++a) s += A.a[a][t] * S[a][b];
      V.a[b][t] -= s;
    }
}
template <int D, int RM>
__device__ __forceinline__ double blk_dot(const Blk<D, RM> &A, const Blk<D, RM> &B) {
  double s = 0;
#pragma unroll
  for (int c = 0; c < D; ++c)
#pragma unroll
    for (int t = 0; t < RM; ++t) s += A.a[c][t] * B.a[c][t];
  return s;
}
template <int D, int RM>
__device__ __forceinline__ void qf_blk(Blk<D, RM> &A) {
#pragma unroll
  for (int j = 0; j < D; ++j) {
#pragma unroll
    for (int pass = 0; pass < 2; ++pass)
#pragma unroll
      for (int c = 0; c < D; ++c)
        if (c < j) {
          double s = 0;
#pragma unroll
          for (int t = 0; t < RM; ++t) s += A.a[c][t] * A.a[j][t];
#pragma unroll
          for (int t = 0; t < RM; ++t) A.a[j][t] -= s * A.a[c][t];
        }
    double nn = 0;
// ... 795 lines not shown
    const double h = Hd[i];
    eta[i] += step * delta[i];
    Heta[i] += step * h;
    if (!boundary) {
      const double rr = res[i] + alpha * h;
      res[i] = rr;
      acc += rr * rr;
      if (sf.y) {
        const long col = i / r;
        const int jp = sf.in_pos[col];
        if (jp >= 0) sf.y[(size_t)jp * r + (i - col * r)] = rr;
      }
    }
  }
  const double tot = block_sum(acc, s_red);
  if (threadIdx.x == 0) p2[blockIdx.x] = tot;
  if (blockIdx.x == 0 && threadIdx.x == 0) {
    ctl->alpha = alpha;
    ctl->e_Pe_n = e_Pe_new;
    if (boundary) tcg_end_run(ctl, hf, seq, tcg_boundary_status(d_Hd), iter + 1);
  }
}

__global__ __launch_bounds__(kBlock) void k_tcg_update2(long nelem, const double *__restrict__ z,
                                                        double *__restrict__ delta, const double *__restrict__ p3,
                                                        int np3, SolverCtl *ctl, HostFlags *hf, int seq, int iter) {
  if (gated(ctl, seq, 2)) return;
  __shared__ double s_red[16];
  const int par = iter & 1;
  const double z_r_new = sum_partials(p3, np3, 1, 0, s_red);
  const double beta = tcg_beta(z_r_new, ctl->z_r[par]);
  for (long i = (long)blockIdx.x * kBlock + threadIdx.x; i < nelem; i += (long)gridDim.x * kBlock)
    delta[i] = -z[i] + beta * delta[i];
  if (blockIdx.x == 0 && threadIdx.x == 0) {
    tcg_put_dir(ctl, par ^ 1, tcg_dir_next(z_r_new, beta, ctl->alpha, ctl->d_Pd[par], ctl->e_Pd[par]), ctl->e_Pe_n);
    if (iter + 1 >= ctl->max_inner) tcg_end_run_at_cap(ctl, hf, seq, iter + 1);
    host_store(&hf->last_seq_done, seq);
  }
}

__global__ __launch_bounds__(kBlock) void k_rtr_decide(const double *pA, int npA, const double *pB, int npB,
                                                       const double *pC, int npC, SolverCtl *ctl, HostFlags *hf,
                                                       int seq, unsigned *tcg_sync, int nsync) {
  if (gated(ctl, seq, 1)) return;
  __shared__ double s_red[20];
  for (int i = threadIdx.x; i < nsync; i += kBlock) tcg_sync[i] = 0u;
  const double *const ps[5] = {pA, pA, pB, pC, pC};
  const int nps[5] = {npA, npA, npB, npC, npC}, sts[5] = {2, 2, 1, 2, 2}, offs[5] = {0, 1, 0, 0, 1};
  double sums[5];
  sum_partials_n<5>(ps, nps, sts, offs, s_red, sums);
  const double fq = sums[0], fg = sums[1], g2 = sums[2], eg = sums[3], eh = sums[4];
  if (threadIdx.x == 0) {
    const double f2 = 0.5 * fq + fg;
    const double rho = (ctl->f1 - f2) / (-(eg + 0.5 * eh));
    ctl->f2 = f2;
    ctl->rho = rho;
    if (rho > 0.75) {
      if (ctl->tcg_status == TR_NEGCURVTURE || ctl->tcg_status == TR_EXCREGION) ctl->Delta = fmin(2.0 * ctl->Delta, ctl->maxDelta);
    } else if (rho < 0.25) {
      ctl->Delta *= 0.25;
    }
    const bool accept = (rho > 0.1) && isfinite(rho);
    if (accept) {
      ctl->cur ^= 1;
      ctl->f1 = f2;
      ctl->ngf = sqrt(g2);
      ctl->accepted += 1;
      ctl->last_accepted = 1;
    } else {
      ctl->last_accepted = 0;
      host_store(&hf->reject_seq, seq);
    }
    ctl->outer_it += 1;
    if (ctl->ngf < ctl->tol || ctl->outer_it >= ctl->max_outer || (ctl->stop_on_accept && accept)) {
      ctl->outer_done_stamp = seq;
      host_store(&hf->outer_done_seq, seq);
    }
    host_store(&hf->last_seq_done, seq);
  }
}

void launch_rtr_init(hipStream_t st, const double *pA, int npA, const double *pB, int npB, SolverCtl *ctl,
                     HostFlags *hf, int seq, CtlInit ci, unsigned *tcg_sync, int nsync) {
  hipLaunchKernelGGL(k_rtr_init, dim3(1), dim3(kBlock), 0, st, pA, npA, pB, npB, ctl, hf, seq, ci, tcg_sync, nsync);
}
void launch_tcg_begin(hipStream_t st, long nelem, Buf2 grad, double *eta, double *Heta, double *res,
                      SolverCtl *ctl, int seq) {
  hipLaunchKernelGGL(k_tcg_begin, dim3(vec_grid(nelem)), dim3(kBlock), 0, st, nelem, grad, eta, Heta, res, ctl,
                     seq);
}
void launch_tcg_update1(hipStream_t st, long nelem, const double *delta, const double *Hd, double *eta,
                        double *Heta, double *res, const double *p1, int np1, double *p2, SolverCtl *ctl,
                        HostFlags *hf, int seq, int iter, int r, SpFold sf) {
  hipLaunchKernelGGL(k_tcg_update1, dim3(vec_grid(nelem)), dim3(kBlock), 0, st, nelem, delta, Hd, eta, Heta, res,
                     p1, np1, p2, ctl, hf, seq, iter, r, sf);
}
void launch_tcg_update2(hipStream_t st, long nelem, const double *z, double *delta, const double *p3, int np3,
                        SolverCtl *ctl, HostFlags *hf, int seq, int iter) {
  hipLaunchKernelGGL(k_tcg_update2, dim3(vec_grid(nelem)), dim3(kBlock), 0, st, nelem, z, delta, p3, np3, ctl, hf,
                     seq, iter);
}
void launch_rtr_decide(hipStream_t st, const double *pA, int npA, const double *pB, int npB, const double *pC,
                       int npC, SolverCtl *ctl, HostFlags *hf, int seq, unsigned *tcg_sync, int nsync) {
  hipLaunchKernelGGL(k_rtr_decide, dim3(1), dim3(kBlock), 0, st, pA, npA, pB, npB, pC, npC, ctl, hf, seq, tcg_sync,
                     nsync);
}

__global__ __launch_bounds__(kBlock) void k_axpby(long nelem, double a, const double *__restrict__ x, double b,
                                                  const double *__restrict__ y, double *__restrict__ out) {
  for (long i = (long)blockIdx.x * kBlock + threadIdx.x; i < nelem; i += (long)gridDim.x * kBlock)
    out[i] = a * x[i] + (y ? b * y[i] : 0.0);
}
void launch_axpby(hipStream_t st, long nelem, double a, const double *x, double b, const double *y, double *out) {
  hipLaunchKernelGGL(k_axpby, dim3(vec_grid(nelem)), dim3(kBlock), 0, st, nelem, a, x, b, y, out);
}

__global__ __launch_bounds__(kBlock) void k_sum_partials(const double *partials, int np, int stride, int count,
                                                         double *out) {
  __shared__ double s_red[16];
  for (int c = 0; c < count; ++c) {
    const double s = sum_partials(partials, np, stride, c, s_red);
    if (threadIdx.x == 0) out[c] = s;
  }
}
void launch_sum_partials(hipStream_t st, const double *partials, int np, int stride, int count, double *out) {
  hipLaunchKernelGGL(k_sum_partials, dim3(1), dim3(kBlock), 0, st, partials, np, stride, count, out);
}

__global__ __launch_bounds__(kBlock) void k_dot(long nelem, const double *__restrict__ x,
                                                const double *__restrict__ y, double *__restrict__ partials) {
  __shared__ double s_red[16];
  double acc = 0;
  for (long i = (long)blockIdx.x * kBlock + threadIdx.x; i < nelem; i += (long)gridDim.x * kBlock)
    acc += x[i] * y[i];
  const double t = block_sum(acc, s_red);
  if (threadIdx.x == 0) partials[blockIdx.x] = t;
}
void launch_dot(hipStream_t st, long nelem, const double *x, const double *y, double *partials) {
  hipLaunchKernelGGL(k_dot, dim3(vec_grid(nelem)), dim3(kBlock), 0, st, nelem, x, y, partials);
}

__global__ __launch_bounds__(kBlock) void k_gather_cols(int r, int ncols, const int *__restrict__ src,
                                                        const double *__restrict__ X, double *__restrict__ out) {
  const long N = (long)ncols * r;
  for (long i = (long)blockIdx.x * kBlock + threadIdx.x; i < N; i += (long)gridDim.x * kBlock) {
    const int c = (int)(i / r), t = (int)(i - (long)c * r);
    out[i] = X[(size_t)src[c] * r + t];
  }
}
__global__ __launch_bounds__(kBlock) void k_scatter_cols(int r, int ncols, const int *__restrict__ dst,
                                                         const double *__restrict__ in, double *__restrict__ X) {
  const long N = (long)ncols * r;
  for (long i = (long)blockIdx.x * kBlock + threadIdx.x; i < N; i += (long)gridDim.x * kBlock) {
    const int c = (int)(i / r), t = (int)(i - (long)c * r);
    X[(size_t)dst[c] * r + t] = in[i];
  }
}
void launch_gather_cols(hipStream_t st, int r, int ncols, const int *src_col, const double *X, double *out) {
  if (ncols <= 0) return;
  hipLaunchKernelGGL(k_gather_cols, dim3(vec_grid((long)ncols * r)), dim3(kBlock), 0, st, r, ncols, src_col, X, out);
}
void launch_scatter_cols(hipStream_t st, int r, int ncols, const int *dst_col, const double *in, double *X) {
  if (ncols <= 0) return;
  hipLaunchKernelGGL(k_scatter_cols, dim3(vec_grid((long)ncols * r)), dim3(kBlock), 0, st, r, ncols, dst_col, in, X);
}

__global__ __launch_bounds__(kBlock) void k_block_dots(int r, const int *__restrict__ cs,
                                                       const double *__restrict__ A, const double *__restrict__ B,
                                                       double *__restrict__ out) {
  __shared__ double s_red[16];
  const int a = blockIdx.x;
  const long lo = (long)cs[a] * r, hi = (long)cs[a + 1] * r;
  double s0 = 0, s1 = 0;
  for (long i = lo + threadIdx.x; i < hi; i += kBlock) {
    const double x = A[i];
    s0 += x * x;
    if (B) s1 += x * B[i];
  }
  const double t0 = block_sum(s0, s_red);
  const double t1 = block_sum(s1, s_red);
  if (threadIdx.x == 0) {
    out[2 * a] = t0;
    out[2 * a + 1] = t1;
  }
}
void launch_block_dots(hipStream_t st, int r, int nagents, const int *col_start, const double *A, const double *B,
// ... 123 lines not shown
```

### dcora_amd/csrc/rbcd.h

```cpp
#pragma once
#include <chrono>
#include <functional>
#include <memory>
#include <string>
#include <vector>

#include "device_problem.h"
#include "host_graph.h"
#include "host_robust.h"
#include "robust.h"
#include "session_core.h"
#include "team_rules.h"

namespace dcora {

struct AgentDev : AgentCore {
  int id = 0, n = 0, col0 = 0;
  bool v_feasible = false;
  std::vector<int> public_poses;
  std::vector<int> required;
  bool detached = false;
  DevBuf<double> nbr[2];
  std::vector<char> got[2];
  bool last_skipped = false;
// ... 7 lines not shown
  std::vector<PoseMeas> meas;
  std::vector<char> update;
  std::vector<char> meas_zero;
  RobustEdges edges;
  bool ranked = false;
  std::vector<int> edge_ids;
  DevBuf<double> X_initial;
  std::vector<HostCsr> Qpat, Cpat;
  HostCsr central_pat;
};

struct TeamState {
  dcora_team_params params{};
  double *rel_host = nullptr, *rel_dev = nullptr;
  TeamState() = default;
  TeamState(const TeamState &) = delete;
  TeamState &operator=(const TeamState &) = delete;
  ~TeamState() {
    if (rel_host) (void)hipHostFree((void *)rel_host);
  }
  std::vector<dcora_agent_status> status;
  std::vector<int> have;
  struct Pending {
    bool on = false, success = false;
    int updates = 0, lc[3] = {0, 0, 0};
  };
  std::vector<Pending> pending;
  std::vector<int> lc;
  int latest_weight_update_iteration = 0, resets_done = 0;
};

class RbcdSession : public SessionCore {
 public:
  int d = 0, n = 0;
  Partition P;
  ManiDesc mg{};
  std::vector<AgentDev> agents;
  std::unique_ptr<DeviceProblem> central;
  DevBuf<double> Vg, Yg, XPrevg;
  DevBuf<int> col_start;
  DevBuf<double> evalbuf, posenorm, eval_split;
  DevBuf<int> pose_start;
  EvalOut *eval_host = nullptr;
  double *x_stage = nullptr;
  EvalOut *eval_dev = nullptr;
  int eval_seq = 0;
  dcora_ropt_result last{};
  int last_result(dcora_ropt_result *res);

  RbcdSession() : SessionCore("rbcd") { R = 1; }
  ~RbcdSession();
  int init(const HostDataset &ds, const dcora_rbcd_options &o);
  std::unique_ptr<RobustSession> robust;
  int init_robust(const HostDataset &ds, const dcora_rbcd_options &o, const dcora_robust_params &p, const int *fixed,
                  bool ranked = false);
  int update_weights(bool reset_to_initial, int counts[3]);
  int compute_weights(double *shared_w, std::vector<double> *w, double counts[3]);
  int apply_weights(const std::vector<double> &w, bool reset_to_initial);
  int set_weights(const double *w);
  int get_weights(double *w) const;
  int set_X(const double *Xh) override;
  int get_X(double *Xh);
  int set_acceleration(bool on);
  int phase_nonselected(int selected) override;
  int phase_selected(int selected) override;
  int evaluate_central(double *cost2, double *gradnorm, double *block_norms, int *next_selected);
  int phase_evaluate_dev(double *out_dev) override;
  int iterate(int selected, double *cost2, double *gradnorm, double *block_norms, int *next_selected);
  int agent_iterate(int agent, bool do_optimization);
  int agent_get_X(int agent, double *Xh);
  int agent_set_X(int agent, const double *Xh);
  int agent_update_neighbor(int agent, int neighbor, int count, const int *frames, const double *poses, bool aux);
  std::vector<int> agent_it;
  int agent_iteration_number(int agent) const;
  std::unique_ptr<TeamState> team;
  int team_enable(const dcora_team_params &p);
  int team_agent_status(int agent, dcora_agent_status *status, int *known);
  int team_decide(int *should_terminate, int *should_update_weights);
  bool team_robust() const { return robust && robust->params.cost_type != DCORA_ROBUST_L2; }
  int team_weight_updates() const { return robust ? robust->updates : 0; }
  int team_inner_iter() const { return team_robust() ? inner_rounds : 0; }
  int run_team(int *iters_done, double *cost2_trace, double *gradnorm_trace, int *selected_trace, int *updated_trace,
               int *weight_updates, int *stop_reason);
  int pack_public(int agent, double *packed_dev);
  int unpack_public(int agent, const double *packed_dev);

  AgentCore &agent_core(int a) override { return agents[(size_t)a]; }
  long num_cols() const override { return (long)(d + 1) * n; }
  int x_stage_hosted(double *host_area) override;

 private:
  bool seq_advanced_ = false;
  int staged_selected_ = -1;
  int staged_iteration_ = -1;
  bool pending_reset_ = false;
  std::vector<char> set_marks_;
  int update_nonselected_agent(AgentDev &a, bool restart);
  int update_selected_agent(AgentDev &a, bool restart);
  int restart_step(AgentDev &a);
  void tick_begins() override;
  int stage(AgentCore &a) override;
  int write_back(AgentCore &a, hipStream_t run_on) override;
  bool serial_set(const std::vector<AgentCore *> &work) override;
  int tick_done(const std::vector<AgentCore *> &work) override;
  int team_note_optimized(const int *ids, int count);
  int team_settle(bool visible);
  void team_refresh_counts();
  void team_clear_statuses();
  void team_restart_rounds();
  std::vector<int> lc_id_, lc_r1_, lc_r2_;
  std::vector<double> lc_w0_;
  struct MeasSplit;
  struct Assembly {
    std::vector<int> ids;
    std::vector<HostCsr> Q, C;
  };
  int assemble(const MeasSplit &split, const std::function<void(size_t, const Assembly &)> &each,
               const std::function<int(const Assembly &)> &agents_ready,
               const std::function<int(const HostCsr &)> &central_ready);
  int attach_preconditioners(const std::vector<HostCsr> &Q, const std::function<int(size_t)> &attach);
  std::chrono::steady_clock::time_point t0_;
  void lap(const char *what) const;
  int rebuild_values(const std::vector<PoseMeas> &meas);
  int adopt_weights(std::vector<PoseMeas> &meas, bool from_device, bool reset_to_initial);
  int initialize_acceleration();
};

}
```

### dcora_amd/csrc/rbcd.hip

```cpp
#include "rbcd.h"
#include "env.h"
#include "host_threads.h"

#include <algorithm>
#include <atomic>
#include <chrono>
#include <cmath>
#include <cstdlib>
#include <cstring>
#include <set>

namespace dcora {

static bool group_kernels(const ManiDesc &m) {
  return group_supported(m) && !env::generic_solver();
}

static void nesterov(hipStream_t st, const ManiDesc &m, int mode, int restart, int skip_lo, int skip_hi, double alpha,
                     double gamma, double *X, double *V, double *Y, double *XPrev, double *Yloc, Buf2 Xloc,
                     const SolverCtl *ctl) {
  if (group_kernels(m))
    launch_g_nesterov(st, m, mode, restart, skip_lo, skip_hi, alpha, gamma, X, V, Y, XPrev, Yloc, Xloc, ctl);
  else
    launch_nesterov(st, m, mode, restart & 1, skip_lo, skip_hi, alpha, gamma, X, V, Y, XPrev, Yloc, Xloc.p[0]);
}

static int nesterov_solved(hipStream_t st, DeviceProblem &pb, int mode, double alpha, double gamma, double *X,
                           double *V, double *Y, double *XPrev) {
  const SolverCtl *c = nullptr;
  Buf2 Xres = pb.result_pick(&c);
  if (!group_kernels(pb.m)) {
    const int rc = pb.result(&Xres.p[0]);
    if (rc) return rc;
    c = nullptr;
  }
  nesterov(st, pb.m, mode, 0, -1, -1, alpha, gamma, X, V, Y, XPrev, nullptr, Xres, c);
  return DCORA_OK;
}

namespace {
constexpr double kPrecondReg = 0.1;
constexpr int kAgentThreads = 8;

int first_failure(const std::vector<int> &rcs, const std::vector<std::string> &errs) {
  for (size_t i = 0; i < rcs.size(); ++i)
    if (rcs[i]) {
      set_last_error(errs[i]);
      return rcs[i];
    }
  return DCORA_OK;
}
}

struct RbcdSession::MeasSplit {
  std::vector<std::vector<PoseMeas>> touching;
  std::vector<PoseMeas> global;
  MeasSplit(const std::vector<PoseMeas> &meas, const Partition &P) : touching((size_t)P.R), global(meas) {
    for (PoseMeas e : meas) {
      e.r1 = P.robot_of(e.p1);
      e.r2 = P.robot_of(e.p2);
      e.p1 -= P.start(e.r1);
      e.p2 -= P.start(e.r2);
      touching[(size_t)e.r1].push_back(e);
      if (e.r2 != e.r1) touching[(size_t)e.r2].push_back(e);
    }
    for (PoseMeas &e : global) e.r1 = e.r2 = 0;
  }
};

RbcdSession::~RbcdSession() {
  if (eval_host) (void)hipHostFree((void *)eval_host);
  if (x_stage) (void)hipHostFree((void *)x_stage);
  team.reset();
  for (AgentDev &a : agents) release_tick_resources(a);
  agents.clear();
  central.reset();
  release_stream();
}

int RbcdSession::init(const HostDataset &ds, const dcora_rbcd_options &o) {
  t0_ = std::chrono::steady_clock::now();
  opt = o;
  d = ds.d;
  n = ds.n;
  r = o.r;
  R = o.num_robots;
  if (R < 1 || n / R < 1 || o.world_size < 1 || o.rank < 0 || o.rank >= o.world_size) {
    set_last_error("rbcd: bad num_robots / rank / world_size");
    return DCORA_ERR_BAD_ARG;
  }
  if (o.acceleration && o.restart_interval < 1) {
    set_last_error("rbcd: acceleration needs restart_interval >= 1 (AgentParameters::restartInterval)");
    return DCORA_ERR_BAD_ARG;
  }
  if (r < d || r > 16) {
    set_last_error("rbcd: relaxation rank must satisfy d <= r <= 16");
    return DCORA_ERR_BAD_ARG;
  }
  P.R = R;
  P.n = n;
  P.per = n / R;
  const int dh = d + 1;
  int ndev = 0;
  if (hipGetDeviceCount(&ndev) != hipSuccess || ndev <= 0) {
    set_last_error("no HIP device available: libdcora_hip has no CPU fallback");
    return DCORA_ERR_NO_DEVICE;
  }
  DCORA_HIP(hipSetDevice(o.device));
  {
    const int rcs = acquire_stream(o.stream);
    if (rcs) return rcs;
  }
  mg = make_mani(r, d, n, 0, 0);
  const size_t N = (size_t)r * dh * n;
  DCORA_HIP(Xg.alloc(N));
  DCORA_HIP(Vg.alloc(N));
  DCORA_HIP(Yg.alloc(N));
  DCORA_HIP(XPrevg.alloc(N));
  if (R > kMaxAgents) {
    set_last_error("rbcd: more agents than kMaxAgents");
    return DCORA_ERR_UNSUPPORTED;
  }
  DCORA_HIP(posenorm.alloc(n));
  DCORA_HIP(eval_split.alloc((size_t)eval_split_doubles()));
  DCORA_HIP(hipHostMalloc((void **)&eval_host, sizeof(EvalOut), hipHostMallocMapped));
  std::memset((void *)eval_host, 0, sizeof(EvalOut));
  DCORA_HIP(hipHostGetDevicePointer((void **)&eval_dev, (void *)eval_host, 0));
  DCORA_HIP(hipHostMalloc((void **)&x_stage, sizeof(double) * N, hipHostMallocDefault));
  DCORA_HIP(hipMemcpyAsync(x_stage, Xg.p, sizeof(double) * N, hipMemcpyDeviceToHost, st));
  DCORA_HIP(hipStreamSynchronize(st));
  DCORA_HIP(evalbuf.alloc(2 * R + 16));
  DCORA_HIP(hipMemset(evalbuf.p, 0, sizeof(double) * (2 * R + 16)));

  lap("buffers");
  const MeasSplit split(ds.meas, P);
  for (size_t e = 0; e < ds.meas.size(); ++e) {
    const PoseMeas &q = ds.meas[e];
    const int r1 = P.robot_of(q.p1), r2 = P.robot_of(q.p2);
    if (r1 == r2 && q.p2 == q.p1 + 1) continue;
    lc_id_.push_back((int)e);
    lc_r1_.push_back(r1);
    lc_r2_.push_back(r2);
    lc_w0_.push_back(q.weight);
  }
  agents.resize(R);
  std::vector<int> cs(R + 1);
  for (int b = 0; b < R; ++b) {
    AgentDev &a = agents[b];
    a.id = b;
    a.n = P.end(b) - P.start(b);
    a.col0 = P.start(b) * dh;
    cs[b] = a.col0;
    a.hosted = (b / ((R + o.world_size - 1) / o.world_size)) == o.rank;
    std::set<int> pub, nb, req;
    for (const PoseMeas &e : split.touching[(size_t)b]) {
      if (e.r1 == e.r2) continue;
      const bool first = e.r1 == b;
      const int other = first ? e.r2 : e.r1;
      pub.insert(P.start(b) + (first ? e.p1 : e.p2));
      req.insert(P.start(other) + (first ? e.p2 : e.p1));
      nb.insert(other);
    }
    a.public_poses.assign(pub.begin(), pub.end());
    a.neighbors.assign(nb.begin(), nb.end());
    a.required.assign(req.begin(), req.end());
// ... 395 lines not shown
               Buf2{{nullptr, nullptr}}, nullptr);
    }
    for (AgentDev &a : agents)
      if (a.id != selected) a.v_feasible = true;
  } else {
    for (AgentDev &a : agents) {
      if (!a.hosted || a.id == selected) continue;
      const int rc = update_nonselected_agent(a, (restart & 1) != 0);
      if (rc) return rc;
    }
  }
  return DCORA_OK;
}

int RbcdSession::update_nonselected_agent(AgentDev &a, bool restart) {
  const size_t off = (size_t)a.col0 * r;
  nesterov(st, a.prob->m, 0, (restart ? 1 : 0) | (a.v_feasible ? 2 : 0), -1, -1, alpha, gamma, Xg.p + off, Vg.p + off,
           Yg.p + off, XPrevg.p + off, nullptr, Buf2{{nullptr, nullptr}}, nullptr);
  a.v_feasible = true;
  return DCORA_OK;
}

int RbcdSession::phase_selected(int selected) {
  if (const int rc = check_selected(selected)) return rc;
  DCORA_HIP(hipSetDevice(opt.device));
  if (!seq_advanced_) advance_sequences();
  seq_advanced_ = false;
  const bool restart = restart_now();
  AgentDev &a = agents[selected];
  if (a.hosted) {
    int rc = update_selected_agent(a, restart);
    if (!rc && team) rc = team_note_optimized(&selected, 1);
    if (rc) return rc;
  }
  if (restart) gamma = alpha = 0;
  return DCORA_OK;
}

static bool cache_complete(const AgentDev &a, int which) {
  return std::find(a.got[which].begin(), a.got[which].end(), 0) == a.got[which].end();
}

int RbcdSession::restart_step(AgentDev &a) {
  DeviceProblem &pb = *a.prob;
  const size_t off = (size_t)a.col0 * r;
  if (a.detached && !cache_complete(a, 0)) {
    const Buf2 Xprev{{XPrevg.p + off, XPrevg.p + off}};
    nesterov(st, pb.m, 3, 0, -1, -1, alpha, gamma, Xg.p + off, Vg.p + off, Yg.p + off, XPrevg.p + off, nullptr, Xprev,
             nullptr);
    return DCORA_OK;
  }
  if (a.detached)
    launch_spmm(st, r, a.coupling.view(), buf1(a.nbr[0].p), 0, nullptr, buf1(pb.G.p), 0, nullptr, Gate{});
  pb.has_G = true;
  last_solver = &pb;
  DCORA_HIP(hipMemcpyAsync(pb.X0.p, XPrevg.p + off, sizeof(double) * (size_t)pb.nelem(), hipMemcpyDeviceToDevice, st));
  const int rc = pb.optimize_dev(opt.local);
  return rc ? rc : nesterov_solved(st, pb, 3, alpha, gamma, Xg.p + off, Vg.p + off, Yg.p + off, XPrevg.p + off);
}

int RbcdSession::update_selected_agent(AgentDev &a, bool restart) {
  int rc = DCORA_OK;
  {
    DeviceProblem &pb = *a.prob;
    const size_t off = (size_t)a.col0 * r;
    const size_t B = sizeof(double) * (size_t)pb.nelem();
    a.last_skipped = false;
    if (a.detached && !cache_complete(a, opt.acceleration ? 1 : 0)) {
      a.last_skipped = true;
      if (opt.acceleration) {
        if (staged_selected_ != a.id || staged_iteration_ != iteration)
          nesterov(st, pb.m, 1, 0, -1, -1, alpha, gamma, Xg.p + off, Vg.p + off, Yg.p + off, XPrevg.p + off, pb.X0.p,
                   Buf2{{nullptr, nullptr}}, nullptr);
        staged_selected_ = -1;
        const Buf2 Xself{{Xg.p + off, Xg.p + off}};
        nesterov(st, pb.m, 2, 0, -1, -1, alpha, gamma, Xg.p + off, Vg.p + off, Yg.p + off, XPrevg.p + off, nullptr, Xself,
                 nullptr);
        a.v_feasible = true;
        if (restart) return restart_step(a);
      }
      return DCORA_OK;
    }
    const double *nsrc = a.detached ? a.nbr[opt.acceleration ? 1 : 0].p : Xg.p;
    launch_spmm(st, r, a.coupling.view(), buf1(nsrc), 0, nullptr, buf1(pb.G.p), 0, nullptr, Gate{});
    pb.has_G = true;
    last_solver = &pb;
    if (opt.acceleration) {
      if (staged_selected_ != a.id || staged_iteration_ != iteration)
        nesterov(st, pb.m, 1, 0, -1, -1, alpha, gamma, Xg.p + off, Vg.p + off, Yg.p + off, XPrevg.p + off, pb.X0.p,
                 Buf2{{nullptr, nullptr}}, nullptr);
      staged_selected_ = -1;
      rc = pb.optimize_dev(opt.local);
      if (!rc) rc = nesterov_solved(st, pb, 2, alpha, gamma, Xg.p + off, Vg.p + off, Yg.p + off, XPrevg.p + off);
      if (rc) return rc;
      a.v_feasible = true;
      if (restart) return restart_step(a);
    } else {
      DCORA_HIP(hipMemcpyAsync(XPrevg.p + off, Xg.p + off, B, hipMemcpyDeviceToDevice, st));
      DCORA_HIP(hipMemcpyAsync(pb.X0.p, Xg.p + off, B, hipMemcpyDeviceToDevice, st));
      double *Xres = nullptr;
      if ((rc = pb.optimize_dev(opt.local)) || (rc = pb.result(&Xres))) return rc;
      DCORA_HIP(hipMemcpyAsync(Xg.p + off, Xres, B, hipMemcpyDeviceToDevice, st));
    }
  }
  return DCORA_OK;
}

int RbcdSession::agent_iterate(int agent, bool do_optimization) {
  staged_selected_ = -1;
  if (agent < 0 || agent >= R) {
    set_last_error("rbcd: agent out of range");
    return DCORA_ERR_BAD_ARG;
  }
  AgentDev &a = agents[agent];
  if (!a.hosted) {
    set_last_error("rbcd: agent is hosted by another rank");
    return DCORA_ERR_BAD_ARG;
  }
  DCORA_HIP(hipSetDevice(opt.device));
  set_marks_.assign(R, 0);
  bool level = (int)agent_it.size() == R;
  for (int q = 0; level && q < R; ++q) level = !agents[q].hosted || agent_it[q] == agent_it[agent];
  if ((int)agent_it.size() != R || (level && agent_it[agent] != iteration)) agent_it.assign(R, iteration);
  if (agent_it[agent] == iteration) {
    for (int q = 0; q < R; ++q)
      if (agents[q].hosted && agent_it[q] != iteration) {
        set_last_error("rbcd: agent " + std::to_string(agent) + " starts a new round before agent " +
                       std::to_string(q) + " has iterated in the current one (agents advance in lockstep)");
        return DCORA_ERR_BAD_ARG;
      }
    if (pending_reset_) gamma = alpha = 0;
    pending_reset_ = false;
    advance_sequences();
    seq_advanced_ = false;
    for (int q = 0; q < R; ++q)
      if (!agents[q].hosted) agent_it[q] = iteration;
  } else if (agent_it[agent] != iteration - 1) {
    set_last_error("rbcd: agents advance in lockstep");
    return DCORA_ERR_BAD_ARG;
  }
  agent_it[agent] = iteration;
  const bool restart = restart_now();
  int rc;
  if (do_optimization) {
    rc = update_selected_agent(a, restart);
    if (!rc && team) rc = team_note_optimized(&agent, 1);
  } else {
    rc = opt.acceleration ? update_nonselected_agent(a, restart) : DCORA_OK;
  }
  if (restart) pending_reset_ = true;
  return rc;
}

int RbcdSession::agent_update_neighbor(int agent, int neighbor, int count, const int *frames, const double *poses,
                                       bool aux) {
  if (agent < 0 || agent >= R || neighbor < 0 || neighbor >= R || neighbor == agent || count < 0) {
    set_last_error("rbcd: bad agent / neighbour");
    return DCORA_ERR_BAD_ARG;
  }
  AgentDev &a = agents[agent];
  if (!a.hosted) {
    set_last_error("rbcd: agent is hosted by another rank");
    return DCORA_ERR_BAD_ARG;
  }
  DCORA_HIP(hipSetDevice(opt.device));
  const int dh = d + 1;
  const size_t blk = (size_t)r * dh;
// ... 91 lines not shown
  if (!gf && !gfb) c.enqueue_egrad(Xg.p, c.EG0.p, c.pA.p);
  if (c.group) {
    int nA = c.npA();
    int wpa = 0;
    if (gf)
      nA = launch_fused_grad(st, c.m, c.Q.view(), buf1(Xg.p), nullptr, buf1(c.EG0.p), buf1(c.RG0.p),
                             Buf2{{nullptr, nullptr}}, 0, c.pA.p, c.pB.p, posenorm.p, Gate{});
    else if (gfb)
      nA = launch_fused_grad_bsr(st, c.m.r, c.m.d, c.Qb.view(), buf1(Xg.p), nullptr, Buf2{{nullptr, nullptr}},
                                 Buf2{{nullptr, nullptr}}, Buf2{{nullptr, nullptr}}, 0, c.pA.p, c.pB.p, posenorm.p,
                                 Gate{}, pose_start.p, R, &wpa);
    else
      c.enq_rgrad(buf1(Xg.p), buf1(c.EG0.p), buf1(c.RG0.p), Buf2{{nullptr, nullptr}}, 0, c.pB.p, Gate{}, posenorm.p);
    const int want = ++eval_seq;
    launch_eval_finish(st, R, pose_start.p, posenorm.p, c.pA.p, nA, eval_dev, want, eval_split.p, n,
                       wpa > 0 ? c.pB.p : nullptr, wpa);
    const auto t0 = std::chrono::steady_clock::now();
    unsigned spins = 0;
    while (eval_host->seq != want) {
      if ((++spins & 4095u) == 0 &&
          std::chrono::duration<double>(std::chrono::steady_clock::now() - t0).count() > 20.0) {
        set_last_error("rbcd: evaluation epilogue did not complete (spin timeout)");
        return DCORA_ERR_HIP;
      }
    }
    std::atomic_thread_fence(std::memory_order_acquire);
    if (block_norms)
      for (int b = 0; b < R; ++b) block_norms[b] = eval_host->block_norms[b];
    if (cost2) *cost2 = eval_host->cost2;
    if (gradnorm) *gradnorm = eval_host->gradnorm;
    if (next_selected) *next_selected = eval_host->next;
    return team ? team_settle(true) : (int)DCORA_OK;
  }
  launch_rgrad(st, mg, buf1(Xg.p), buf1(c.EG0.p), buf1(c.RG0.p), Buf2{{nullptr, nullptr}}, 0, c.pB.p, Gate{});
  launch_block_dots(st, r, R, col_start.p, c.RG0.p, nullptr, evalbuf.p);
  launch_sum_partials(st, c.pA.p, c.npA(), 2, 2, evalbuf.p + 2 * R);
  std::vector<double> h(2 * R + 2);
  DCORA_HIP(hipMemcpyAsync(h.data(), evalbuf.p, sizeof(double) * (2 * R + 2), hipMemcpyDeviceToHost, st));
  DCORA_HIP(hipStreamSynchronize(st));
  double g2 = 0, best = -1;
  int arg = 0;
  for (int b = 0; b < R; ++b) {
    const double nb = std::sqrt(h[2 * b]);
    if (block_norms) block_norms[b] = nb;
    g2 += h[2 * b];
    if (nb > best) {
      best = nb;
      arg = b;
    }
  }
  if (cost2) *cost2 = 2.0 * (0.5 * h[2 * R] + h[2 * R + 1]);
  if (gradnorm) *gradnorm = std::sqrt(g2);
  if (next_selected) *next_selected = arg;
  return team ? team_settle(true) : (int)DCORA_OK;
}

int RbcdSession::last_result(dcora_ropt_result *res) {
  if (last_solver) return last_solver->fetch_result(res);
  *res = last;
  return DCORA_OK;
}

int RbcdSession::phase_evaluate_dev(double *out_dev) {
  DCORA_HIP(hipSetDevice(opt.device));
  DCORA_HIP(hipMemsetAsync(out_dev, 0, sizeof(double) * 2 * R, st));
  for (AgentDev &a : agents) {
    if (!a.hosted) continue;
    DeviceProblem &pb = *a.prob;
    const double *Xb = Xg.p + (size_t)a.col0 * r;
    launch_spmm(st, r, a.coupling.view(), buf1(Xg.p), 0, nullptr, buf1(pb.G.p), 0, nullptr, Gate{});
    pb.has_G = true;
    pb.enqueue_egrad(Xb, pb.EG1.p, nullptr);
    launch_rgrad(st, pb.m, buf1(Xb), buf1(pb.EG1.p), buf1(pb.RG1.p), Buf2{{nullptr, nullptr}}, 0, pb.pB.p, Gate{});
    launch_sum_partials(st, pb.pB.p, pb.npPose(), 1, 1, out_dev + 2 * a.id);
    launch_dot(st, pb.nelem(), Xb, pb.EG1.p, pb.p3.p);
    launch_sum_partials(st, pb.p3.p, pb.npVec(), 1, 1, out_dev + 2 * a.id + 1);
  }
  return DCORA_OK;
}

int RbcdSession::iterate(int selected, double *cost2, double *gradnorm, double *block_norms, int *next_selected) {
  int rc = check_selected(selected);
  if (rc) return rc;
  rc = phase_nonselected(selected);
  if (rc) return rc;
  rc = phase_selected(selected);
  if (rc) return rc;
  int nxt = selected;
  rc = evaluate_central(cost2, gradnorm, block_norms, &nxt);
  if (rc) return rc;
  if (next_selected) *next_selected = (agents[selected].coupling.nnz > 0) ? nxt : selected;
  return DCORA_OK;
}

void RbcdSession::tick_begins() {
  staged_selected_ = -1;
  seq_advanced_ = false;
  set_marks_.assign(R, 0);
}

int RbcdSession::stage(AgentCore &core) {
  AgentDev &a = static_cast<AgentDev &>(core);
  DeviceProblem &pb = *a.prob;
  const size_t off = (size_t)a.col0 * r;
  const size_t B = sizeof(double) * (size_t)pb.nelem();
  launch_spmm(st, r, a.coupling.view(), buf1(Xg.p), 0, nullptr, buf1(pb.G.p), 0, nullptr, Gate{});
  pb.has_G = true;
  DCORA_HIP(hipMemcpyAsync(XPrevg.p + off, Xg.p + off, B, hipMemcpyDeviceToDevice, st));
  DCORA_HIP(hipMemcpyAsync(pb.X0.p, Xg.p + off, B, hipMemcpyDeviceToDevice, st));
  return DCORA_OK;
}

int RbcdSession::write_back(AgentCore &core, hipStream_t run_on) {
  AgentDev &a = static_cast<AgentDev &>(core);
  DeviceProblem &pb = *a.prob;
  const size_t off = (size_t)a.col0 * r;
  if (group_kernels(pb.m))
    return nesterov_solved(run_on, pb, 3, 0.0, 0.0, Xg.p + off, Vg.p + off, Yg.p + off, XPrevg.p + off);
  double *Xres = nullptr;
  const int rc = pb.result(&Xres);
  if (rc) return rc;
  DCORA_HIP(hipMemcpyAsync(Xg.p + off, Xres, sizeof(double) * (size_t)pb.nelem(), hipMemcpyDeviceToDevice, run_on));
  return DCORA_OK;
}

bool RbcdSession::serial_set(const std::vector<AgentCore *> &work) {
  bool serial = true;
  for (const AgentCore *a : work) serial = serial && a->prob->tcg_run_ok && a->prob->use_pc();
  return serial;
}

int RbcdSession::tick_done(const std::vector<AgentCore *> &work) {
  if (!team) return DCORA_OK;
  std::vector<int> ids;
  for (const AgentCore *a : work) ids.push_back(static_cast<const AgentDev *>(a)->id);
  return team_note_optimized(ids.data(), (int)ids.size());
}

int RbcdSession::pack_public(int agent, double *packed_dev) {
  AgentDev &a = agents[agent];
  launch_gather_cols(st, r, (int)a.public_poses.size() * (d + 1), a.public_cols.p, Xg.p, packed_dev);
  return DCORA_OK;
}
int RbcdSession::unpack_public(int agent, const double *packed_dev) {
  AgentDev &a = agents[agent];
  launch_scatter_cols(st, r, (int)a.public_poses.size() * (d + 1), a.public_cols.p, packed_dev, Xg.p);
  return DCORA_OK;
}

int RbcdSession::x_stage_hosted(double *host_area) {
  DCORA_HIP(hipSetDevice(opt.device));
  for (const AgentDev &a : agents) {
    if (!a.hosted) continue;
    const size_t off = (size_t)a.col0 * r;
    DCORA_HIP(hipMemcpyAsync(host_area + off, Xg.p + off, sizeof(double) * (size_t)r * (d + 1) * a.n,
                             hipMemcpyDeviceToHost, st));
  }
  DCORA_HIP(hipStreamSynchronize(st));
  return DCORA_OK;
}

int RbcdSession::agent_iteration_number(int agent) const {
  if ((int)agent_it.size() != R) return iteration;
  for (int q = 0; q < R; ++q)
    if (agents[(size_t)q].hosted && agent_it[(size_t)q] != agent_it[(size_t)agent]) return agent_it[(size_t)agent];
  return iteration;
}

int RbcdSession::team_enable(const dcora_team_params &p) {
  if (opt.world_size != 1) {
    set_last_error("rbcd team: only single-process sessions (world_size 1) keep the team's statuses; the ranks of a "
                   "job exchange their flags with dcora_exchange_all_ready");
// ... 154 lines not shown
```

### dcora_amd/csrc/solver_fused.hip

```cpp
#include <algorithm>
#include <stdexcept>
#include <atomic>
#include <type_traits>
#include <vector>
#include <cstdlib>
#include <cstring>

#include "kernels.h"
#include "tcg_rules.h"

namespace dcora {

namespace {

constexpr int GW = 8;

__device__ __forceinline__ double f_partial4_load(const double *__restrict__ p, int np) {
  const int l = (int)(threadIdx.x & 63u);
  const double a = (l < np) ? p[l] : 0.0, b = (l + 64 < np) ? p[l + 64] : 0.0;
  const double c = (l + 128 < np) ? p[l + 128] : 0.0, d = (l + 192 < np) ? p[l + 192] : 0.0;
  return (a + b) + (c + d);
}
__device__ __forceinline__ int f_partial_index(int np) { return np <= 64 ? (int)(threadIdx.x & 63u) : (int)threadIdx.x; }
__device__ __forceinline__ double f_partial_total(double v, int np, double *sm) {
// ... 265 lines not shown
  ld_row<D>(X + o, r, tt, pact, Y);
  double S[D][D];
#pragma unroll
  for (int a = 0; a < D; ++a)
#pragma unroll
    for (int b = 0; b < D; ++b) S[a][b] = (g < npose) ? Sblk[(size_t)(pose0 + g) * D * D + a + b * D] : 0.0;
  for (int i = threadIdx.x + kBlock; i < np3; i += kBlock) myp += p3[i];
  if (seq > st_o || seq > st_t) return;
  __syncthreads();
  constexpr int GB = 16;
  double ga[GB], gz[GB], gw[GB];
  const int lo0 = myb - pbeg;
  const int hi0 = min(mye, pbeg + kHessTile) - pbeg;
#pragma unroll
  for (int q = 0; q < GB; ++q) {
    const bool ok = act && (lo0 + q < hi0);
    const size_t oo = ok ? (size_t)s_ci[lo0 + q] * r + t : 0;
    gw[q] = ok ? s_v[lo0 + q] : 0.0;
    gz[q] = z[oo];
    ga[q] = (iter > 0) ? d_old[oo] : 0.0;
  }
  const double z_r_new = p3_wave ? wave_sum(myp) : f_partial_total(myp, np3, s_red);
  double beta = 0;
  if (iter > 0) beta = tcg_beta(z_r_new, c_zr);
  if (blockIdx.x == 0 && threadIdx.x == 0) {
    if (iter == 0)
      tcg_put_dir(ctl, 0, tcg_dir_start(z_r_new), 0.0);
    else
      tcg_put_dir(ctl, par, tcg_dir_next(z_r_new, beta, c_alpha, c_dPd, c_ePd), c_ePen);
  }
  double acc = 0;
#pragma unroll
  for (int q = 0; q < GB; ++q) acc += gw[q] * (beta * ga[q] - gz[q]);
  for (int base = pbeg; base < pend; base += kHessTile) {
    const int cnt = min(kHessTile, pend - base);
    if (base != pbeg) {
      __syncthreads();
      for (int i = threadIdx.x; i < cnt; i += kBlock) {
        s_ci[i] = Q.ci[base + i];
        s_v[i] = Q.v[base + i];
      }
      __syncthreads();
    }
    int lo = max(myb, base) - base;
    const int hi = min(mye, base + cnt) - base;
    if (base == pbeg) lo += GB;
    for (int p = lo; p < hi; p += 8) {
      double a8[8], b8[8], w8[8];
#pragma unroll
      for (int q = 0; q < 8; ++q) {
        const bool ok = p + q < hi;
        const size_t oo = ok ? (size_t)s_ci[p + q] * r + t : 0;
        w8[q] = ok ? s_v[p + q] : 0.0;
        b8[q] = z[oo];
        a8[q] = (iter > 0) ? d_old[oo] : 0.0;
      }
#pragma unroll
      for (int q = 0; q < 8; ++q) acc += w8[q] * (beta * a8[q] - b8[q]);
    }
  }
  if (act) {
    const double dn = (iter > 0) ? beta * d_own - z_own : -z_own;
    d_new[oown] = dn;
    s_W[e] = acc;
    s_D[e] = dn;
  }
  __syncthreads();
  Row<D> V, W;
#pragma unroll
  for (int a = 0; a < DH; ++a) {
    W.e[a] = pact ? s_W[(g * DH + a) * r + tt] : 0.0;
    V.e[a] = pact ? s_D[(g * DH + a) * r + tt] : 0.0;
  }
  row_sub_AS<D>(W, V, S);
  row_tangent<D>(Y, W);
  st_row<D>(Hd + o, r, tt, pact, W);
  double dacc = 0;
#pragma unroll
  for (int a = 0; a < DH; ++a) dacc += V.e[a] * W.e[a];
  const double tot = block_sum(dacc, s_red);
  if (threadIdx.x == 0) p1[blockIdx.x] = tot;
}

template <int D>
__global__ __launch_bounds__(kBlock) void k_fused_grad(ManiDesc m, CsrDev Q, Buf2 Xb, const double *__restrict__ G,
                                                       Buf2 EGb, Buf2 RGb, Buf2 Sb, int sel,
                                                       double *__restrict__ pA, double *__restrict__ pB,
                                                       double *__restrict__ posenorm, Gate g) {
  if (gated(g.ctl, g.seq, g.gate)) return;
  __shared__ int s_ci[kHessTile];
  __shared__ double s_v[kHessTile];
  __shared__ double s_W[kBlock], s_X[kBlock];
  __shared__ double s_red[16];
  constexpr int DH = D + 1;
  const int idx = g.ctl ? ((g.ctl->cur ^ sel) & 1) : 0;
  const double *__restrict__ X = Xb.p[idx];
  double *__restrict__ EG = EGb.p[idx];
  double *__restrict__ RG = RGb.p[idx];
  double *__restrict__ Sblk = Sb.p[idx];
  const int r = m.r;
  const int PB = fused_pb(r, DH);
  const int pose0 = blockIdx.x * PB;
  const int npose = min(PB, m.n - pose0);
  const int j0 = pose0 * DH, ncol = npose * DH, nout = ncol * r;
  const int e = threadIdx.x;
  const bool act = e < nout;
  const int lc = e / r, t = e - lc * r;
  const int j = j0 + lc;
  const int pbeg = Q.rp[j0], pend = Q.rp[j0 + ncol];
  const int myb = act ? Q.rp[j] : 0, mye = act ? Q.rp[j + 1] : 0;
  const size_t oown = (size_t)j * r + t;
  const double x_own = act ? X[oown] : 0.0;
  const double g_own = (act && G) ? G[oown] : 0.0;
  double acc = 0;
  for (int base = pbeg; base < pend; base += kHessTile) {
    const int cnt = min(kHessTile, pend - base);
    if (base != pbeg) __syncthreads();
    {
      constexpr int SU = kHessTile / kBlock;
      int ci_r[SU];
      double v_r[SU];
      const int last = max(pend - 1, 0);
#pragma unroll
      for (int u = 0; u < SU; ++u) {
        const int i = min(base + (int)threadIdx.x + u * kBlock, last);
        ci_r[u] = Q.ci[i];
        v_r[u] = Q.v[i];
      }
#pragma unroll
      for (int u = 0; u < SU; ++u) {
        const int i = threadIdx.x + u * kBlock;
        if (i < cnt) {
          s_ci[i] = ci_r[u];
          s_v[i] = v_r[u];
        }
      }
    }
    __syncthreads();
    const int lo = max(myb, base) - base, hi = min(mye, base + cnt) - base;
    for (int p = lo; p < hi; p += 8) {
      double b8[8], w8[8];
#pragma unroll
      for (int q = 0; q < 8; ++q) {
        const bool ok = p + q < hi;
        const size_t oo = ok ? (size_t)s_ci[p + q] * r + t : 0;
        w8[q] = ok ? s_v[p + q] : 0.0;
        b8[q] = X[oo];
      }
#pragma unroll
      for (int q = 0; q < 8; ++q) acc += w8[q] * b8[q];
    }
  }
  double d0 = 0, d1 = 0;
  if (act) {
    const double eg = acc + g_own;
    EG[oown] = eg;
    s_W[e] = eg;
    s_X[e] = x_own;
    d0 = acc * x_own;
    d1 = x_own * g_own;
  }
  __syncthreads();
  const int gp = threadIdx.x >> 3, tt = threadIdx.x & (GW - 1);
  const bool pact = (gp < npose) && (tt < r);
  const int pose = pose0 + gp;
  const size_t o = (size_t)pose * DH * r;
  Row<D> Y, E;
#pragma unroll
  for (int a = 0; a < DH; ++a) {
    E.e[a] = pact ? s_W[(gp * DH + a) * r + tt] : 0.0;
    Y.e[a] = pact ? s_X[(gp * DH + a) * r + tt] : 0.0;
  }
  double S[D][D];
  grp_sym_gram<D>(Y, E, S);
  if (Sblk && gp < npose && tt == 0)
#pragma unroll
    for (int a = 0; a < D; ++a)
#pragma unroll
      for (int b = 0; b < D; ++b) Sblk[(size_t)pose * D * D + a + b * D] = S[a][b];
  row_sub_AS<D>(E, Y, S);
  double pa = 0;
#pragma unroll
  for (int a = 0; a < DH; ++a) pa += E.e[a] * E.e[a];
  if (posenorm) {
    const double ps = grp_sum(pa);
    if (gp < npose && tt == 0) posenorm[pose] = ps;
  }
  st_row<D>(RG + o, r, tt, pact, E);
  const double t0 = block_sum(d0, s_red);
  const double t1 = block_sum(d1, s_red);
  const double t2 = block_sum(pact ? pa : 0.0, s_red);
  if (threadIdx.x == 0) {
    pA[2 * blockIdx.x] = t0;
    pA[2 * blockIdx.x + 1] = t1;
    pB[blockIdx.x] = t2;
  }
// ... 1589 lines not shown
                                                        const double *__restrict__ pA, int npA, EvalOut *out,
                                                        int seq, const double *__restrict__ part,
                                                        const double *__restrict__ agent_partials, int wpa) {
  __shared__ double s_red[16];
  __shared__ double s_bn[kMaxAgents];
  double q0 = ((int)threadIdx.x < npA) ? pA[2 * threadIdx.x] : 0.0;
  double q1 = ((int)threadIdx.x < npA) ? pA[2 * threadIdx.x + 1] : 0.0;
  if (agent_partials) {
    const int w = threadIdx.x >> 6, lane = threadIdx.x & 63, nw = kBlock / 64;
    for (int b = w; b < R; b += nw) {
      const int lo = b * wpa, hi = lo + wpa;
      double v = 0;
      for (int i0 = lo + lane; i0 < hi; i0 += 64 * 8) {
        double t8[8];
#pragma unroll
        for (int u = 0; u < 8; ++u) t8[u] = agent_partials[min(i0 + 64 * u, hi - 1)];
#pragma unroll
        for (int u = 0; u < 8; ++u) v += (i0 + 64 * u < hi) ? t8[u] : 0.0;
      }
      v = wave_sum(v);
      if (lane == 0) s_bn[b] = v;
    }
  } else if (part) {
    if ((int)threadIdx.x < R) {
      double v = 0;
      for (int u = 0; u < kEvalSplit; ++u) v += part[threadIdx.x * kEvalSplit + u];
      s_bn[threadIdx.x] = v;
    }
  } else
  {
    const int w = threadIdx.x >> 6, lane = threadIdx.x & 63, nw = kBlock / 64;
    for (int b = w; b < R; b += nw) {
      const int lo = pose_start[b], hi = pose_start[b + 1];
      double v = 0;
      for (int i0 = lo + lane; i0 < hi; i0 += 64 * 8) {
        double t8[8];
#pragma unroll
        for (int u = 0; u < 8; ++u) t8[u] = posenorm[min(i0 + 64 * u, hi - 1)];
#pragma unroll
        for (int u = 0; u < 8; ++u) v += (i0 + 64 * u < hi) ? t8[u] : 0.0;
      }
      v = wave_sum(v);
      if (lane == 0) s_bn[b] = v;
    }
  }
  for (int i0 = threadIdx.x + kBlock; i0 < npA; i0 += 8 * kBlock) {
    double a8[8], c8[8];
#pragma unroll
    for (int u = 0; u < 8; ++u) {
      const int i = i0 + u * kBlock;
      a8[u] = i < npA ? pA[2 * i] : 0.0;
      c8[u] = i < npA ? pA[2 * i + 1] : 0.0;
    }
#pragma unroll
    for (int u = 0; u < 8; ++u) {
      q0 += a8[u];
      q1 += c8[u];
    }
  }
  const double fq = block_sum(q0, s_red);
  const double fg = block_sum(q1, s_red);
  if (threadIdx.x == 0) {
    double g2 = 0, best = -1;
    int arg = 0;
    for (int b = 0; b < R; ++b) {
      const double nb = sqrt(s_bn[b]);
      out->block_norms[b] = nb;
      g2 += s_bn[b];
      if (nb > best) {
        best = nb;
        arg = b;
      }
    }
    out->cost2 = 2.0 * (0.5 * fq + fg);
    out->gradnorm = sqrt(g2);
    out->next = arg;
    __threadfence_system();
    __hip_atomic_store(const_cast<int *>(&out->seq), seq, __ATOMIC_RELEASE, __HIP_MEMORY_SCOPE_SYSTEM);
  }
}
void launch_eval_finish(hipStream_t st, int R, const int *pose_start, const double *posenorm, const double *pA,
                        int npA, EvalOut *out_dev, int seq, double *split_scratch, int nposes,
                        const double *agent_partials, int wg_per_agent) {
  const bool split = !agent_partials && split_scratch && nposes >= 16384;
  if (split)
    hipLaunchKernelGGL(k_eval_partial, dim3(R * kEvalSplit), dim3(kBlock), 0, st, pose_start, posenorm, split_scratch);
  hipLaunchKernelGGL(k_eval_finish, dim3(1), dim3(kBlock), 0, st, R, pose_start, posenorm, pA, npA, out_dev, seq,
                     split ? split_scratch : nullptr, agent_partials, wg_per_agent);
}
int eval_split_doubles() { return kMaxAgents * kEvalSplit; }

int spmm_bsr_grid(int nbrows) {
  const int cap = kBsrMaxGrid, per = kPosesPerBlock;
  long g = ((long)nbrows + per - 1) / per;
  if (g < 1) g = 1;
  if (g > cap) g = cap;
  return (int)g;
}
template <bool DOTS, bool GRAD>
static bool launch_bsrq(hipStream_t st, int grid, int r, int d, const BsrDev &A, Buf2 X, int selX, const double *G, Buf2 Y,
                        int selY, double *partials, Gate g, const BsrGradOut &go) {
#define DCORA_BSRQ(D_, R_)                                                                                              \
  if (d == D_ && r == R_) {                                                                                             \
    hipLaunchKernelGGL((k_spmm_bsrq<D_, R_, DOTS, GRAD>), dim3(grid), dim3(kQBlock), 0, st, A, X, selX, G, Y, selY, \
                       partials, g, go);                                                                                \
    return true;                                                                                                        \
  }
  DCORA_BSRQ(3, 3) DCORA_BSRQ(3, 4) DCORA_BSRQ(3, 5) DCORA_BSRQ(3, 6) DCORA_BSRQ(3, 7) DCORA_BSRQ(3, 8)
  DCORA_BSRQ(2, 2) DCORA_BSRQ(2, 3) DCORA_BSRQ(2, 4) DCORA_BSRQ(2, 5) DCORA_BSRQ(2, 6) DCORA_BSRQ(2, 7) DCORA_BSRQ(2, 8)
#undef DCORA_BSRQ
  return false;
}
void launch_spmm_bsr(hipStream_t st, int r, int d, const BsrDev &A, Buf2 X, int selX, const double *G, Buf2 Y,
                     int selY, double *partials, Gate g) {
  const int grid = spmm_bsr_grid(A.nbrows);
  const BsrGradOut none{};
  const bool ok = partials ? launch_bsrq<true, false>(st, grid, r, d, A, X, selX, G, Y, selY, partials, g, none)
                           : launch_bsrq<false, false>(st, grid, r, d, A, X, selX, G, Y, selY, partials, g, none);
  if (!ok) throw std::logic_error("block Q-apply: no instantiation for this (d, r); the block structure is built for d <= r <= 8 only");
}
int launch_fused_grad_bsr(hipStream_t st, int r, int d, const BsrDev &A, Buf2 X, const double *G, Buf2 EG, Buf2 RG, Buf2 S,
                          int sel, double *pA, double *pB, double *posenorm, Gate g, const int *agent_start, int agents,
                          int *wg_per_agent) {
  int grid = spmm_bsr_grid(A.nbrows);
  BsrGradOut go;
  go.RG = RG;
  go.S = S;
  go.pB = pB;
  go.posenorm = posenorm;
  if (agent_start && agents > 0 && wg_per_agent) {
    const int wpa = std::max(1, grid / agents);
    grid = wpa * agents;
    go.agent_start = agent_start;
    go.wg_per_agent = wpa;
    go.posenorm = nullptr;
    *wg_per_agent = wpa;
  }
  if (!launch_bsrq<true, true>(st, grid, r, d, A, X, sel, G, EG, sel, pA, g, go))
    throw std::logic_error("block evaluation: no instantiation for this (d, r); the block structure is built for d <= r <= 8 only");
  return grid;
}

bool group_supported(const ManiDesc &m) { return m.se && m.r <= GW && m.n > 0; }
bool fused_supported(const ManiDesc &m) {
  return m.se && m.r <= GW && m.n > 0 && (m.n + fused_pb(m.r, m.d + 1) - 1) / fused_pb(m.r, m.d + 1) <= 2 * kMaxPartials;
}
int fused_pose_blocks(const ManiDesc &m) {
  const int pb = fused_pb(m.r, m.d + 1);
  return (m.n + pb - 1) / pb;
}
int fused_nsplit(const ManiDesc &m) {
  const int njc = (m.k + kJChunk - 1) / kJChunk;
  const int aim = 512, cap = 32;
  int ns = (aim + njc - 1) / njc;
  if (ns < 1) ns = 1;
  if (ns > cap) ns = cap;
  while (ns > 1 && (m.k + ns - 1) / ns < 16) --ns;
  return ns;
}
int fused_precond_grid(const ManiDesc &m) { return ((m.k + kJChunk - 1) / kJChunk) * fused_nsplit(m); }
int fused_update_grid(const ManiDesc &m) {
  const long blocks = ((long)m.r * m.k + kBlock - 1) / kBlock;
  return (int)(blocks < 1024 ? blocks : 1024);
}

int launch_fused_hess(hipStream_t st, const ManiDesc &m, const CsrDev &Q, const double *z, const double *d_old,
                      double *d_new, Buf2 X, Buf2 S, double *Hd, const double *p3, int np3, double *p1,
                      SolverCtl *ctl, int seq, int iter, const BsrDev *Ab) {
  if (Ab) {
    const int gridb = (m.n + kPosesPerBlock - 1) / kPosesPerBlock;
    if (m.d == 3)
      hipLaunchKernelGGL(k_fused_hess_bsr<3>, dim3(gridb), dim3(kBlock), 0, st, m, *Ab, z, d_old, d_new, X, S, Hd, p3,
                         np3, p1, ctl, seq, iter);
    else
      hipLaunchKernelGGL(k_fused_hess_bsr<2>, dim3(gridb), dim3(kBlock), 0, st, m, *Ab, z, d_old, d_new, X, S, Hd, p3,
                         np3, p1, ctl, seq, iter);
    return gridb;
  }
  const int grid = fused_pose_blocks(m);
  if (m.d == 3)
    hipLaunchKernelGGL(k_fused_hess<3>, dim3(grid), dim3(kBlock), 0, st, m, Q, z, d_old, d_new, X, S, Hd, p3, np3,
                       p1, ctl, seq, iter);
  else
    hipLaunchKernelGGL(k_fused_hess<2>, dim3(grid), dim3(kBlock), 0, st, m, Q, z, d_old, d_new, X, S, Hd, p3, np3,
                       p1, ctl, seq, iter);
  return grid;
}
void launch_fused_precond(hipStream_t st, const ManiDesc &m, int ldm, const double *Minv, Buf2 grad,
                          const double *delta, const double *Hd, double *eta, double *Heta, const double *res_old,
                          double *res_new, double *Zpart, const double *p1, int np1, double *p2, SolverCtl *ctl,
                          HostFlags *hf, int seq, int iter, int first, SpFold sf) {
  const int grid = Minv ? fused_precond_grid(m) : fused_update_grid(m);
  const int ns = Minv ? fused_nsplit(m) : 1;
#define DCORA_LAUNCH_PRECOND(RM, HM)                                                                               \
  hipLaunchKernelGGL((k_fused_precond<RM, HM>), dim3(grid), dim3(kBlock), 0, st, m.r, m.k, ldm, ns, Minv, grad,     \
                     delta, Hd, eta, Heta, res_old, res_new, Zpart, p1, np1, p2, ctl, hf, seq, iter, first, sf)
  if (m.r <= 4) {
    if (Minv) DCORA_LAUNCH_PRECOND(4, true); else DCORA_LAUNCH_PRECOND(4, false);
  } else {
    if (Minv) DCORA_LAUNCH_PRECOND(8, true); else DCORA_LAUNCH_PRECOND(8, false);
  }
#undef DCORA_LAUNCH_PRECOND
}
int fused_pc_pb(const ManiDesc &m) { return m.n <= 768 ? 2 : 4; }
int fused_pc_blocks(const ManiDesc &m) {
  const int pb = fused_pc_pb(m);
  return (m.n + pb - 1) / pb;
}
constexpr int kPcLdsCap = 128 * 1024;
static int pc_chunk(const ManiDesc &m, int ldm) { return std::min((kPcLdsCap / (8 * m.r)) / 128 * 128, ldm); }
bool fused_pc_preferred(const ManiDesc &m, int ldm) {
  return m.k <= pc_chunk(m, ldm) && (long)m.r * m.k <= 2L * kPcSB * kPcBlock && m.r <= 7;
}
template <int D, int PB, int R, bool MULTI>
static int pc_launch(hipStream_t st, const ManiDesc &m, int ldm, const double *Minv, Buf2 grad, Buf2 X,
                     const double *delta, const double *Hd, double *eta, double *Heta, const double *res_old,
                     double *res_new, double *z, const double *p1, int np1, double *p3, SolverCtl *ctl, HostFlags *hf,
                     int seq, int iter, int first, double *pC, bool prepare_only) {
  static std::atomic<unsigned long long> tried{0}, ok{0};
  int dev = 0;
  if (hipGetDevice(&dev) != hipSuccess || dev < 0 || dev >= 64) return -1;
  const unsigned long long bit = 1ull << dev;
  if (!(tried.load(std::memory_order_acquire) & bit)) {
    const hipError_t e = hipFuncSetAttribute(reinterpret_cast<const void *>(&k_fused_pc<D, PB, R, MULTI>),
                                             hipFuncAttributeMaxDynamicSharedMemorySize, kPcLdsCap);
    if (e == hipSuccess)
      ok.fetch_or(bit, std::memory_order_release);
    else
      (void)hipGetLastError();
    tried.fetch_or(bit, std::memory_order_release);
  }
  const int chk = pc_chunk(m, ldm);
  const size_t lds = (size_t)chk * m.r * sizeof(double);
  if (!(ok.load(std::memory_order_acquire) & bit) && lds > 64 * 1024) return -1;
  const int grid = (m.n + PB - 1) / PB;
  if (prepare_only) return grid;
  hipLaunchKernelGGL((k_fused_pc<D, PB, R, MULTI>), dim3(grid), dim3(kPcBlock), lds, st, m, ldm, chk, Minv, grad, X,
                     delta, Hd, eta, Heta, res_old, res_new, z, p1, np1, p3, ctl, hf, seq, iter, first, pC);
  if (hipGetLastError() != hipSuccess) return -1;
  return grid;
}
static int fused_pc_dispatch(hipStream_t st, const ManiDesc &m, int ldm, const double *Minv, Buf2 grad, Buf2 X,
                             const double *delta, const double *Hd, double *eta, double *Heta, const double *res_old,
                             double *res_new, double *z, const double *p1, int np1, double *p3, SolverCtl *ctl,
                             HostFlags *hf, int seq, int iter, int first, double *pC, bool prepare_only) {
#define DCORA_PC(D_, PB_, R_, MULTI_)                                                                                \
  return pc_launch<D_, PB_, R_, MULTI_>(st, m, ldm, Minv, grad, X, delta, Hd, eta, Heta, res_old, res_new, z, p1, np1, \
                                        p3, ctl, hf, seq, iter, first, pC, prepare_only)
#define DCORA_PC_FIXED_R(D_, PB_, MULTI_)      \
  do {                                          \
    if (D_ == 3 && m.r == 3) DCORA_PC(D_, PB_, 3, MULTI_); \
    if (D_ == 3 && m.r == 4) DCORA_PC(D_, PB_, 4, MULTI_); \
    if (D_ == 3 && m.r == 5) DCORA_PC(D_, PB_, 5, MULTI_); \
    if (D_ == 3 && m.r == 6) DCORA_PC(D_, PB_, 6, MULTI_); \
    if (D_ == 3 && m.r == 7) DCORA_PC(D_, PB_, 7, MULTI_); \
  } while (0)
#define DCORA_PC_R(D_, PB_, MULTI_)             \
  do {                                          \
    DCORA_PC_FIXED_R(D_, PB_, MULTI_);          \
    DCORA_PC(D_, PB_, 0, MULTI_);               \
  } while (0)
  const int pb = fused_pc_pb(m);
  const bool multi = m.k > pc_chunk(m, ldm);
  if (m.d == 3) {
    if (pb == 2 && !multi) DCORA_PC_R(3, 2, false);
    if (pb == 2) DCORA_PC_R(3, 2, true);
    if (m.r == 3) DCORA_PC(3, 4, 3, true);
    if (m.r == 4) DCORA_PC(3, 4, 4, true);
    if (m.r == 5) DCORA_PC(3, 4, 5, true);
    if (m.r == 6) DCORA_PC(3, 4, 6, true);
    return -1;
  }
  if (pb == 2 && !multi) DCORA_PC(2, 2, 0, false);
  if (pb == 2) DCORA_PC(2, 2, 0, true);
  DCORA_PC(2, 4, 0, true);
#undef DCORA_PC_R
#undef DCORA_PC_FIXED_R
#undef DCORA_PC
}
constexpr int kRunNS = 4;
int tcg_run_sync_words() { return kRunSyncWords; }
std::atomic<int> g_tcg_run_fault{0};
std::atomic<int> g_tcg_run_fault_skip{0};
int tcg_run_max_rows_nnz(const ManiDesc &m, const int *rp) {
  const int dh = m.d + 1;
  int worst = 0;
  for (int p0 = 0; p0 < m.n; p0 += 2) {
    const int j0 = p0 * dh, j1 = std::min(m.n, p0 + 2) * dh;
    worst = std::max(worst, rp[j1] - rp[j0]);
  }
  return worst;
}
bool tcg_run_supported(const ManiDesc &m, int ldm, int cus, int max_rows_nnz) {
  if (!m.se || m.d != 3 || m.r < 4 || m.r > 6) return false;
  if (fused_pb(m.r, m.d + 1) % 2 != 0) return false;
  if (!fused_pc_preferred(m, ldm) || fused_pc_pb(m) != 2) return false;
  const int grid = (m.n + 1) / 2;
  if (grid > cus || grid > 256) return false;
  if (m.k > kRunNS * kPcNW * 128) return false;
  const int rows_per = fused_pb(m.r, m.d + 1) / 2;
  if ((grid + rows_per - 1) / rows_per > 64) return false;
  return max_rows_nnz <= kRunQCap;
}
template <int R>
static int tcg_run_launch(hipStream_t st, const TcgRunArgs &a) {
  static std::atomic<unsigned long long> tried{0}, ok{0};
  int dev = 0;
  if (hipGetDevice(&dev) != hipSuccess || dev < 0 || dev >= 64) return -1;
  const unsigned long long bit = 1ull << dev;
  if (!(tried.load(std::memory_order_acquire) & bit)) {
    const hipError_t e = hipFuncSetAttribute(reinterpret_cast<const void *>(&k_tcg_run<3, R, kRunNS>),
                                             hipFuncAttributeMaxDynamicSharedMemorySize, kPcLdsCap);
    if (e == hipSuccess)
      ok.fetch_or(bit, std::memory_order_release);
    else
      (void)hipGetLastError();
    tried.fetch_or(bit, std::memory_order_release);
  }
  const int cpad = ((a.m.k + 127) / 128) * 128;
  const size_t lds = (size_t)cpad * R * sizeof(double);
  if (!(ok.load(std::memory_order_acquire) & bit) && lds > 40 * 1024) return -1;
  const int grid = (a.m.n + 1) / 2;
  hipLaunchKernelGGL((k_tcg_run<3, R, kRunNS>), dim3(grid), dim3(kPcBlock), lds, st, a);
  if (hipGetLastError() != hipSuccess) return -1;
  return grid;
}
int launch_tcg_run(hipStream_t st, const ManiDesc &m, int ldm, const double *Minv, const CsrDev &Q, Buf2 grad, Buf2 X,
                   Buf2 S, double *d0, double *d1, double *Hd, double *eta, double *Heta, double *z, double *p1r,
                   double *p3, double *pC, unsigned *sync, SolverCtl *ctl, HostFlags *hf, int seq) {
  int fault = 0;
  bool skipped = false;
  for (int sk = g_tcg_run_fault_skip.load(); sk > 0;)
    if (g_tcg_run_fault_skip.compare_exchange_weak(sk, sk - 1)) {
      skipped = true;
      break;
    }
  for (int left = skipped ? 0 : g_tcg_run_fault.load(); left > 0;)
    if (g_tcg_run_fault.compare_exchange_weak(left, left - 1)) {
      fault = 1;
      break;
    }
  TcgRunArgs a{m, ldm, Minv, Q, grad, X, S, d0, d1, Hd, eta, Heta, z, p1r, p3, pC, sync, ctl, hf, seq,
               fused_pb(m.r, m.d + 1), fault};
#ifdef DCORA_RUN_STAMPS
  {
    static long long *buf = nullptr;
    if (!buf) (void)hipHostMalloc((void **)&buf, 64 * sizeof(long long), hipHostMallocMapped);
    static int count = 0;
    if (buf && count > 0) {
      static double acc[64];
      static int n = 0;
      long long s0 = buf[0];
      if (buf[3] > s0 && buf[5 + 7 * 3] > 0) {
        for (int i = 0; i < 40; ++i) acc[i] += (double)(buf[i] - s0) * 0.01;
        ++n;
      }
      for (int i = 0; i < 64; ++i) buf[i] = 0;
      if (n == 500) {
        fprintf(stderr, "k_tcg_run stamps (us from start, workgroup 0, mean of %d runs with >= 4 iterations):", n);
        for (int i = 0; i < 34; ++i) fprintf(stderr, " %.2f", acc[i] / n);
        fprintf(stderr, "\n");
        n = -1000000;
      }
    }
    ++count;
    a.stamps = buf;
  }
#endif
  if (m.r == 4) return tcg_run_launch<4>(st, a);
  if (m.r == 5) return tcg_run_launch<5>(st, a);
  if (m.r == 6) return tcg_run_launch<6>(st, a);
  return -1;
}
int launch_fused_pc(hipStream_t st, const ManiDesc &m, int ldm, const double *Minv, Buf2 grad, Buf2 X,
                    const double *delta, const double *Hd, double *eta, double *Heta, const double *res_old,
                    double *res_new, double *z, const double *p1, int np1, double *p3, SolverCtl *ctl, HostFlags *hf,
                    int seq, int iter, int first, double *pC) {
  return fused_pc_dispatch(st, m, ldm, Minv, grad, X, delta, Hd, eta, Heta, res_old, res_new, z, p1, np1, p3, ctl, hf,
                           seq, iter, first, pC, false);
}
bool fused_pc_ready(const ManiDesc &m, int ldm) {
  Buf2 none{};
  return fused_pc_dispatch(nullptr, m, ldm, nullptr, none, none, nullptr, nullptr, nullptr, nullptr, nullptr, nullptr,
                           nullptr, nullptr, 0, nullptr, nullptr, nullptr, 0, 0, 0, nullptr, true) >= 0;
}
void launch_fused_finish(hipStream_t st, const ManiDesc &m, Buf2 X, const double *Zpart, const double *res,
                         double *z, const double *p2, int np2, double *p3, SolverCtl *ctl, HostFlags *hf, int seq,
                         int iter, int first, int nsplit, SpFold sf, double *zraw) {
  const int grid = fused_pose_blocks(m);
  const int ns = nsplit > 0 ? nsplit : fused_nsplit(m);
  if (m.d == 3)
    hipLaunchKernelGGL(k_fused_finish<3>, dim3(grid), dim3(kBlock), 0, st, m, ns, X, Zpart, res, z, p2, np2, p3, ctl,
                       hf, seq, iter, first, sf, zraw);
  else
    hipLaunchKernelGGL(k_fused_finish<2>, dim3(grid), dim3(kBlock), 0, st, m, ns, X, Zpart, res, z, p2, np2, p3, ctl,
                       hf, seq, iter, first, sf, zraw);
}

int launch_g_rgrad(hipStream_t st, const ManiDesc &m, Buf2 X, Buf2 EG, Buf2 RG, Buf2 Sblk, int sel, double *partials,
                   double *posenorm, Gate g) {
  const int grid = group_grid(m.n);
  if (m.d == 3)
    hipLaunchKernelGGL(k_g_rgrad<3>, dim3(grid), dim3(kBlock), 0, st, m, X, EG, RG, Sblk, sel, partials, posenorm, g);
  else
    hipLaunchKernelGGL(k_g_rgrad<2>, dim3(grid), dim3(kBlock), 0, st, m, X, EG, RG, Sblk, sel, partials, posenorm, g);
  return grid;
}
int launch_fused_grad(hipStream_t st, const ManiDesc &m, const CsrDev &Q, Buf2 X, const double *G, Buf2 EG, Buf2 RG,
                      Buf2 Sblk, int sel, double *pA, double *pB, double *posenorm, Gate g) {
  const int grid = fused_pose_blocks(m);
  if (m.d == 3)
    hipLaunchKernelGGL(k_fused_grad<3>, dim3(grid), dim3(kBlock), 0, st, m, Q, X, G, EG, RG, Sblk, sel, pA, pB, posenorm,
                       g);
  else
    hipLaunchKernelGGL(k_fused_grad<2>, dim3(grid), dim3(kBlock), 0, st, m, Q, X, G, EG, RG, Sblk, sel, pA, pB, posenorm,
                       g);
  return grid;
}
int launch_g_retract(hipStream_t st, const ManiDesc &m, Buf2 X, const double *V, double alpha, Buf2 out, int selOut,
                     Buf2 grad, const double *HV, double *partials, Gate g) {
  const int grid = group_grid(m.n);
  if (m.d == 3)
    hipLaunchKernelGGL(k_g_retract<3>, dim3(grid), dim3(kBlock), 0, st, m, X, V, alpha, out, selOut, grad, HV,
                       partials, g);
  else
    hipLaunchKernelGGL(k_g_retract<2>, dim3(grid), dim3(kBlock), 0, st, m, X, V, alpha, out, selOut, grad, HV,
                       partials, g);
  return grid;
}
void launch_g_nesterov(hipStream_t st, const ManiDesc &m, int mode, int restart, int skip_lo, int skip_hi,
                       double alpha, double gamma, double *X, double *V, double *Y, double *XPrev, double *Yloc,
                       Buf2 Xloc, const SolverCtl *ctl, double *inner_Yloc) {
  GNesterovArgs a{mode, restart, skip_lo, skip_hi, alpha, gamma, X, V, Y, XPrev, Yloc, inner_Yloc, Xloc, ctl};
  const int grid = group_grid(m.n);
  if (m.d == 3)
    hipLaunchKernelGGL(k_g_nesterov<3>, dim3(grid), dim3(kBlock), 0, st, m, a);
  else
    hipLaunchKernelGGL(k_g_nesterov<2>, dim3(grid), dim3(kBlock), 0, st, m, a);
}

}
```

### dcora_amd/csrc/team_status.hip

```cpp
#include "device_problem.h"
#include "kernels.h"

namespace dcora {

__device__ __forceinline__ double wave_max_dpp(double v) {
  v = fmax(v, dpp_move<0xB1>(v));
  v = fmax(v, dpp_move<0x4E>(v));
  v = fmax(v, dpp_move<0x141>(v));
  v = fmax(v, dpp_move<0x140>(v));
  return fmax(fmax(readlane_f64(v, 0), readlane_f64(v, 16)), fmax(readlane_f64(v, 32), readlane_f64(v, 48)));
}

__global__ __launch_bounds__(kBlock) void k_rel_change(int r, int dh, const double *__restrict__ X,
                                                       const double *__restrict__ XPrev,
                                                       const int *__restrict__ pose_start, RelChangeSet set,
                                                       double *out) {
  __shared__ double s_max[kBlock / 64];
  const int b = set.agent[blockIdx.x];
  const int lo = pose_start[b], hi = pose_start[b + 1];
  double m = 0;
  for (int i = lo + (int)threadIdx.x; i < hi; i += kBlock) {
    const size_t o = ((size_t)i * dh + (dh - 1)) * r;
    double s = 0;
    for (int k = 0; k < r; ++k) {
      const double e = X[o + k] - XPrev[o + k];
      s += e * e;
    }
    m = fmax(m, sqrt(s));
  }
  m = wave_max_dpp(m);
  if ((threadIdx.x & 63) == 0) s_max[threadIdx.x >> 6] = m;
  __syncthreads();
  if (threadIdx.x == 0) {
    for (int w = 1; w < kBlock / 64; ++w) m = fmax(m, s_max[w]);
    out[b] = m;
    __threadfence_system();
  }
}

void launch_rel_change(hipStream_t st, int r, int d, const double *X, const double *XPrev, const int *pose_start,
                       const RelChangeSet &set, double *out) {
  if (set.count < 1) return;
  hipLaunchKernelGGL(k_rel_change, dim3(set.count), dim3(kBlock), 0, st, r, d + 1, X, XPrev, pose_start, set, out);
}

int max_translation_distance(int r, int d, int n, const double *X, const double *Y, double *out) {
  if (r < 2 || r > 16 || (d != 2 && d != 3) || d > r || n < 1) {
    set_last_error("max_translation_distance: needs 2 <= r <= 16, d in {2, 3}, d <= r, n >= 1");
    return DCORA_ERR_BAD_ARG;
  }
  int ndev = 0;
  if (hipGetDeviceCount(&ndev) != hipSuccess || ndev <= 0) {
    set_last_error("no HIP device available: libdcora_hip has no CPU fallback");
    return DCORA_ERR_NO_DEVICE;
  }
  const size_t N = (size_t)r * (d + 1) * n;
  DevBuf<double> dX, dY, dout;
  DevBuf<int> dps;
  DCORA_HIP(dX.alloc(N));
  DCORA_HIP(dY.alloc(N));
  DCORA_HIP(dout.alloc(1));
  DCORA_HIP(dps.alloc(2));
  const int ps[2] = {0, n};
  DCORA_HIP(hipMemcpy(dX.p, X, sizeof(double) * N, hipMemcpyHostToDevice));
  DCORA_HIP(hipMemcpy(dY.p, Y, sizeof(double) * N, hipMemcpyHostToDevice));
  DCORA_HIP(hipMemcpy(dps.p, ps, sizeof(ps), hipMemcpyHostToDevice));
  RelChangeSet set{};
  set.count = 1;
  launch_rel_change(nullptr, r, d, dX.p, dY.p, dps.p, set, dout.p);
  DCORA_HIP(hipGetLastError());
  DCORA_HIP(hipMemcpy(out, dout.p, sizeof(double), hipMemcpyDeviceToHost));
  return DCORA_OK;
}

}
```

### include/dcora_hip.h

```cpp
#ifndef DCORA_HIP_H_
#define DCORA_HIP_H_

#ifdef __cplusplus
extern "C" {
#endif

typedef enum {
  DCORA_OK = 0,
  DCORA_ERR_BAD_ARG = 1,
  DCORA_ERR_NO_DEVICE = 2,
  DCORA_ERR_HIP = 3,
  DCORA_ERR_NOT_PD = 4,
  DCORA_ERR_NO_CONVERGENCE = 5,
  DCORA_ERR_NO_PRECONDITIONER = 6,
  DCORA_ERR_IO = 7,
  DCORA_ERR_UNSUPPORTED = 8,
  DCORA_ERR_EXCHANGE_LINK = 9
} dcora_status;

const char *dcora_status_string(int status);
const char *dcora_last_error(void);
int dcora_device_count(void);

enum {
// ... 71 lines not shown
                       double min_eig_num_tol, int num_lanczos_vectors, unsigned long long seed, int device,
                       double *lambda_min, double *v, long *num_matvecs);
int dcora_cert_fast_verification(int k, const int *rowptr, const int *colidx, const double *vals, double eta,
                                 int block, int device, int *is_psd, double *theta, double *x, double *lambda_min);

int dcora_cert_suboptimality_gap(const dcora_dims *dims, const double *X, double lambda_lower_bound, double *gap,
                                 double *n_eff);
int dcora_cert_lambda_min_certified(int k, const int *rowptr, const int *colidx, const double *vals, double eta,
                                    int block, int max_iterations, double *lambda_min, int *iterations);

typedef struct dcora_dataset_s *dcora_dataset_t;
int dcora_dataset_load_g2o(const char *path, dcora_dataset_t *out);
int dcora_dataset_create(int d, int n, int m, const int *ids, const double *vals, dcora_dataset_t *out);
int dcora_dataset_info(dcora_dataset_t ds, int *d, int *n, int *m);
int dcora_dataset_copy(dcora_dataset_t ds, int *ids, double *vals);
int dcora_dataset_destroy(dcora_dataset_t ds);
int dcora_dataset_chordal_init(dcora_dataset_t ds, double *T);
int dcora_dataset_chordal_init_device(dcora_dataset_t ds, int device, double *T);
int dcora_graph_build_Q_pgo(int d, int n, int agent_id, int m, const int *ids, const double *vals, dcora_csr_t *Q);

typedef struct dcora_radataset_s *dcora_radataset_t;
int dcora_radataset_load_pyfg(const char *path, dcora_radataset_t *out);
int dcora_radataset_info(dcora_radataset_t ds, int *info);
int dcora_radataset_create(int d, int n, int l, int b, int m_pp, const int *pp_ids, const double *pp_vals, int m_pl,
                           const int *pl_ids, const double *pl_vals, int m_rg, const int *rg_ids, const double *rg_vals,
                           const double *gt, dcora_radataset_t *out);
int dcora_radataset_copy(dcora_radataset_t ds, int *pp_ids, double *pp_vals, int *pl_ids, double *pl_vals, int *rg_ids,
                         double *rg_vals);
int dcora_radataset_ground_truth(dcora_radataset_t ds, double *gt);
int dcora_radataset_build_Q(dcora_radataset_t ds, dcora_csr_t *Q);
int dcora_radataset_odometry_init(dcora_radataset_t ds, unsigned long long seed, double *X0);
int dcora_radataset_ownership(dcora_radataset_t ds, int *pose_robot, int *sphere_robot, int *landmark_robot);
int dcora_radataset_agent_columns(dcora_radataset_t ds, int robot, int *dims3, int *own, int *k_a);
int dcora_radataset_agent_colours(dcora_radataset_t ds, int *colours, int *ncolours);
int dcora_graph_extract_agent_blocks(int k, const int *rowptr, const int *colidx, const double *vals, int k_a,
                                     const int *own, dcora_csr_t *Qaa, dcora_csr_t *C);
int dcora_radataset_destroy(dcora_radataset_t ds);
int dcora_graph_precond_regularization(int k, const int *rowptr, const int *colidx, const double *vals, int device,
                                       double *reg);

typedef struct dcora_rbcd_s *dcora_rbcd_t;
typedef struct {
  int num_robots;
  int r;
  int acceleration;
  int restart_interval;
  dcora_ropt_params local;
  int rank, world_size;
  int device;
  void *stream;
} dcora_rbcd_options;
void dcora_rbcd_options_default(dcora_rbcd_options *o);

int dcora_rbcd_create(dcora_dataset_t ds, const dcora_rbcd_options *opt, dcora_rbcd_t *out);
int dcora_rbcd_destroy(dcora_rbcd_t s);
int dcora_rbcd_set_X(dcora_rbcd_t s, const double *X);
int dcora_rbcd_get_X(dcora_rbcd_t s, double *X);
int dcora_rbcd_iterate(dcora_rbcd_t s, int selected, double *cost2, double *gradnorm, double *block_norms,
                       int *next_selected);
int dcora_rbcd_run(dcora_rbcd_t s, int max_iters, double rgrad_tol, int *iters_done, double *cost2_trace,
                   double *gradnorm_trace, int *selected_trace);
int dcora_rbcd_iterate_set(dcora_rbcd_t s, const int *set, int count, int allow_adjacent);
int dcora_rbcd_set_acceleration(dcora_rbcd_t s, int acceleration);
int dcora_rbcd_agent_colours(dcora_rbcd_t s, int *colours, int *ncolours);
int dcora_rbcd_run_coloured(dcora_rbcd_t s, int max_sweeps, double rgrad_tol, int *sweeps_done, double *cost2_trace,
                            double *gradnorm_trace);
int dcora_rbcd_evaluate(dcora_rbcd_t s, double *cost2, double *gradnorm, double *block_norms, int *next_selected);
int dcora_rbcd_agent_iterate(dcora_rbcd_t s, int agent, int do_optimization);
int dcora_rbcd_agent_update_neighbor(dcora_rbcd_t s, int agent, int neighbor, int count, const int *frames,
                                     const double *poses, int auxiliary);
int dcora_rbcd_agent_last_skipped(dcora_rbcd_t s, int agent, int *skipped);
int dcora_rbcd_agent_get_X(dcora_rbcd_t s, int agent, double *X);
int dcora_rbcd_agent_set_X(dcora_rbcd_t s, int agent, const double *X);
int dcora_rbcd_agent_info(dcora_rbcd_t s, int agent, int *num_poses, int *first_pose, int *iteration_number);
int dcora_rbcd_last_result(dcora_rbcd_t s, dcora_ropt_result *res);

int dcora_rbcd_X_device_ptr(dcora_rbcd_t s, double **X_dev);
int dcora_rbcd_public_count(dcora_rbcd_t s, int agent, int *count);
int dcora_rbcd_public_indices(dcora_rbcd_t s, int agent, int *global_pose_idx);
int dcora_rbcd_pack_public_dev(dcora_rbcd_t s, int agent, double *packed_dev);
int dcora_rbcd_unpack_public_dev(dcora_rbcd_t s, int agent, const double *packed_dev);
int dcora_rbcd_phase_nonselected(dcora_rbcd_t s, int selected);
int dcora_rbcd_phase_selected(dcora_rbcd_t s, int selected);
int dcora_rbcd_phase_evaluate_dev(dcora_rbcd_t s, double *out_dev);
int dcora_rbcd_synchronize(dcora_rbcd_t s);
int dcora_rbcd_profile_tcg_runs(dcora_rbcd_t s, int enable);
int dcora_rbcd_profile_tcg_read(dcora_rbcd_t s, double *out2);

typedef struct dcora_exchange_s *dcora_exchange_t;
int dcora_exchange_create(dcora_rbcd_t s, const char *job_name, dcora_exchange_t *out);
int dcora_exchange_destroy(dcora_exchange_t ex);
int dcora_exchange_info(dcora_exchange_t ex, double *info10);
int dcora_exchange_link_report(dcora_exchange_t ex, double *out4);
int dcora_exchange_post(dcora_exchange_t ex, const int *agents, int count);
int dcora_exchange_wait(dcora_exchange_t ex, const int *agents, int count);
int dcora_exchange_evaluate(dcora_exchange_t ex, double *cost2, double *gradnorm, double *block_norms,
                            int *next_selected);
int dcora_exchange_rbcd_iterate(dcora_exchange_t ex, int selected, double *cost2, double *gradnorm,
                                double *block_norms, int *next_selected);
int dcora_exchange_rbcd_tick(dcora_exchange_t ex, const int *set, int count, int allow_adjacent);
int dcora_exchange_run_coloured(dcora_exchange_t ex, int max_sweeps, double rgrad_tol, int *sweeps_done,
                                double *cost2_trace, double *gradnorm_trace);
int dcora_exchange_set_X(dcora_exchange_t ex, const double *X);
int dcora_exchange_gather_X(dcora_exchange_t ex, double *X);
int dcora_exchange_barrier(dcora_exchange_t ex);
int dcora_exchange_all_ready(dcora_exchange_t ex, int ready, int *all_ready);
int dcora_exchange_certify(dcora_exchange_t ex, int k, const int *rowptr, const int *colidx, const double *vals,
                           double eta, int *certified, double *theta, double *lambda_min, double *v, long long *matvecs,
                           int *distributed);
int dcora_exchange_host_selftest(const char *job_name, int rank, int world_size, int num_agents, int rounds,
                                 double *checksum);
int dcora_debug_exchange_leave_stale(const char *job_name, int world_size, int num_agents);
int dcora_debug_exchange_probe_fault(int rounds);

typedef struct dcora_ra_rbcd_s *dcora_ra_rbcd_t;
int dcora_ra_rbcd_create(dcora_radataset_t ds, const dcora_rbcd_options *opt, dcora_ra_rbcd_t *out);
int dcora_exchange_create_ra(dcora_ra_rbcd_t s, const char *job_name, dcora_exchange_t *out);
int dcora_ra_rbcd_destroy(dcora_ra_rbcd_t s);
int dcora_ra_rbcd_info(dcora_ra_rbcd_t s, int *num_agents, int *robots);
int dcora_ra_rbcd_set_X(dcora_ra_rbcd_t s, const double *X);
int dcora_ra_rbcd_get_X(dcora_ra_rbcd_t s, double *X);
int dcora_ra_rbcd_iterate(dcora_ra_rbcd_t s, int selected, double *cost2, double *gradnorm, double *block_norms,
                          int *next_selected);
int dcora_ra_rbcd_evaluate(dcora_ra_rbcd_t s, double *cost2, double *gradnorm, double *block_norms,
                           int *next_selected);
int dcora_ra_rbcd_run(dcora_ra_rbcd_t s, int max_iters, double rgrad_tol, int *iters_done, double *cost2_trace,
                      double *gradnorm_trace, int *selected_trace);
int dcora_ra_rbcd_last_result(dcora_ra_rbcd_t s, dcora_ropt_result *res);
int dcora_ra_rbcd_iterate_set(dcora_ra_rbcd_t s, const int *set, int count, int allow_adjacent);
int dcora_ra_rbcd_set_acceleration(dcora_ra_rbcd_t s, int acceleration);
int dcora_ra_rbcd_agent_colours(dcora_ra_rbcd_t s, int *colours, int *ncolours);
int dcora_ra_rbcd_run_coloured(dcora_ra_rbcd_t s, int max_sweeps, double rgrad_tol, int *sweeps_done,
                               double *cost2_trace, double *gradnorm_trace);

typedef enum {
  DCORA_ROBUST_L2 = 0,
  DCORA_ROBUST_L1 = 1,
  DCORA_ROBUST_TLS = 2,
  DCORA_ROBUST_HUBER = 3,
  DCORA_ROBUST_GM = 4,
  DCORA_ROBUST_GNC_TLS = 5
} dcora_robust_type;
typedef struct {
  int cost_type;
  int GNCMaxNumIters;
  double GNCBarc, GNCMuStep, GNCInitMu;
  double HuberThreshold, TLSThreshold;
} dcora_robust_params;
void dcora_robust_params_default(dcora_robust_params *p);
int dcora_rbcd_create_robust(dcora_dataset_t ds, const dcora_rbcd_options *opt, const dcora_robust_params *robust,
                             const int *fixed_weight, dcora_rbcd_t *out);
int dcora_rbcd_update_weights(dcora_rbcd_t s, int reset_to_initial, int counts[3]);
int dcora_rbcd_set_weights(dcora_rbcd_t s, const double *w);
int dcora_rbcd_get_weights(dcora_rbcd_t s, double *w);
int dcora_rbcd_robust_info(dcora_rbcd_t s, double *mu, int *updates);
int dcora_rbcd_create_robust_ranks(dcora_dataset_t ds, const dcora_rbcd_options *opt, const dcora_robust_params *robust,
                                   const int *fixed_weight, const char *job_name, dcora_rbcd_t *session,
                                   dcora_exchange_t *ex);
int dcora_exchange_update_weights(dcora_exchange_t ex, int reset_to_initial, int counts[3]);
int dcora_exchange_set_weights(dcora_exchange_t ex, const double *w);
int dcora_exchange_get_weights(dcora_exchange_t ex, double *w);

typedef struct {
  int max_num_iters;
  double rel_change_tol;
  int robust_opt_num_weight_updates, robust_opt_num_resets, robust_opt_inner_iters;
// ... 68 lines not shown
```

Measured before the change: 4228.

## Fold coupling SpMM into the first fused-gradient kernel launch

Instead of launching a separate SpMM to build the neighbour-coupling term G before each selected agent's solve, the session stashes the coupling matrix and source X on the problem. The first fused-gradient kernel then computes each row's coupling product inline and writes G as it goes. If the fused path is not taken, a fallback launches the SpMM at optimize time. This removes one kernel launch and a round trip of G through memory per iteration, at the cost of extra per-thread work in the gradient kernel and a second template instantiation. Launch counters and a debug query are added as well.

```diff
diff --git a/dcora_amd/__init__.py b/dcora_amd/__init__.py
--- a/dcora_amd/__init__.py
+++ b/dcora_amd/__init__.py
@@ -627,6 +627,11 @@
     def phase_selected(self, selected):
         check(capi.lib().dcora_rbcd_phase_selected(self.h, selected))
 
+    def debug_launches(self):
+        out = C.c_longlong(0)
+        check(capi.lib().dcora_debug_rbcd_launches(self.h, C.byref(out)))
+        return int(out.value)
+
     def phase_evaluate_dev(self, ptr):
         check(capi.lib().dcora_rbcd_phase_evaluate_dev(self.h, C.c_void_p(ptr)))
 
diff --git a/dcora_amd/capi.py b/dcora_amd/capi.py
--- a/dcora_amd/capi.py
+++ b/dcora_amd/capi.py
@@ -184,6 +184,7 @@
     "dcora_rbcd_unpack_public_dev": (C.c_int, [_vp, C.c_int, _vp]),
     "dcora_rbcd_phase_nonselected": (C.c_int, [_vp, C.c_int]),
     "dcora_rbcd_phase_selected": (C.c_int, [_vp, C.c_int]),
+    "dcora_debug_rbcd_launches": (C.c_int, [_vp, C.POINTER(C.c_longlong)]),
     "dcora_rbcd_phase_evaluate_dev": (C.c_int, [_vp, _vp]),
     "dcora_rbcd_synchronize": (C.c_int, [_vp]),
     "dcora_exchange_create": (C.c_int, [_vp, C.c_char_p, C.POINTER(_vp)]),
diff --git a/dcora_amd/csrc/capi.hip b/dcora_amd/csrc/capi.hip
--- a/dcora_amd/csrc/capi.hip
+++ b/dcora_amd/csrc/capi.hip
@@ -1243,6 +1243,12 @@
 int dcora_rbcd_phase_selected(dcora_rbcd_t s, int selected) {
   return abi_call({s}, [&] { return s->s.phase_selected(selected); });
 }
+int dcora_debug_rbcd_launches(dcora_rbcd_t s, long long *launches) {
+  return abi_call({s, launches}, [&] {
+    *launches = s->s.chain_launches;
+    return (int)DCORA_OK;
+  });
+}
 int dcora_rbcd_phase_evaluate_dev(dcora_rbcd_t s, double *out_dev) {
   return abi_call({s, out_dev}, [&] { return s->s.phase_evaluate_dev(out_dev); });
 }
diff --git a/dcora_amd/csrc/device_problem.h b/dcora_amd/csrc/device_problem.h
--- a/dcora_amd/csrc/device_problem.h
+++ b/dcora_amd/csrc/device_problem.h
@@ -190,6 +190,10 @@
   int enq_qapply(Buf2 X, int selX, const double *Gp, Buf2 Y, int selY, double *partials, Gate g);
   DevBuf<double> G;
   bool has_G = false;
+  void ride_G(const CsrDev &C, const double *Xsrc) {
+    ride_C_ = C;
+    ride_X_ = Xsrc;
+  }
   DevBuf<double> Minv;
   int ldm = 0;
   SparsePrecond sp;
@@ -270,6 +274,8 @@
   struct RtrForm;
   int rtr_dev(const dcora_ropt_params &prm, TcgForm form);
   int rgd_dev(const dcora_ropt_params &prm);
+  CsrDev ride_C_{};
+  const double *ride_X_ = nullptr;
   int seq_ = 0;
   bool pending_ = false;
   bool rgd_ = false;
diff --git a/dcora_amd/csrc/device_problem.hip b/dcora_amd/csrc/device_problem.hip
--- a/dcora_amd/csrc/device_problem.hip
+++ b/dcora_amd/csrc/device_problem.hip
@@ -652,13 +652,17 @@
 int DeviceProblem::optimize_dev(const dcora_ropt_params &prm) {
   pending_ = false;
   rgd_ = prm.method != 0;
+  TcgForm form = TcgForm::generic;
+  if (fused) form = !use_pc() ? TcgForm::split : (tcg_run_ok && !concurrent_solves) ? TcgForm::run : TcgForm::pc;
+  if (ride_X_ && (rgd_ || !has_precond || form == TcgForm::generic || has_bsr || Q.n_long != 0)) {
+    launch_spmm(st, m.r, ride_C_, buf1(ride_X_), 0, nullptr, buf1(G.p), 0, nullptr, Gate{});
+    ride_X_ = nullptr;
+  }
   if (rgd_) return rgd_dev(prm);
   if (!has_precond) {
     set_last_error("RTR requires the preconditioner (ref src/QuadraticProblem.cpp:78-82)");
     return DCORA_ERR_NO_PRECONDITIONER;
   }
-  TcgForm form = TcgForm::generic;
-  if (fused) form = !use_pc() ? TcgForm::split : (tcg_run_ok && !concurrent_solves) ? TcgForm::run : TcgForm::pc;
   return rtr_dev(prm, form);
 }
 
@@ -826,7 +830,19 @@
       launch_rgrad(p.st, p.m, p.Xb(), p.EGb(), p.RGb(), p.Sb(), sel, p.pB.p, g());
       return nP;
     }
-    if (gf) return launch_fused_grad(p.st, p.m, Qv, p.Xb(), Gp, p.EGb(), p.RGb(), p.Sb(), sel, p.pA.p, p.pB.p, nullptr, g());
+    if (gf) {
+      GradRide ride;
+      if (sel == 0 && p.ride_X_) {
+        ride.c_rp = p.ride_C_.rp;
+        ride.c_ci = p.ride_C_.ci;
+        ride.c_v = p.ride_C_.v;
+        ride.c_X = p.ride_X_;
+        ride.G_out = p.G.p;
+        p.ride_X_ = nullptr;
+      }
+      return launch_fused_grad(p.st, p.m, Qv, p.Xb(), Gp, p.EGb(), p.RGb(), p.Sb(), sel, p.pA.p, p.pB.p, nullptr, g(),
+                               ride.c_rp ? &ride : nullptr);
+    }
     if (gfb)
       return launch_fused_grad_bsr(p.st, p.m.r, p.m.d, Qbv, p.Xb(), Gp, kNoBuf, p.RGb(), p.Sb(), sel, p.pA.p, p.pB.p,
                                    nullptr, g());
diff --git a/dcora_amd/csrc/env.cpp b/dcora_amd/csrc/env.cpp
--- a/dcora_amd/csrc/env.cpp
+++ b/dcora_amd/csrc/env.cpp
@@ -28,6 +28,9 @@
 int solver_bc() {
   static const int v = is("DCORA_SOLVER_BC", "pc") ? 1 : is("DCORA_SOLVER_BC", "split") ? -1 : 0;
   return v;
+}
+bool chain_rides() {
+  return !is("DCORA_CHAIN", "launches");
 }
 bool factor_on_host() {
   static const bool v = is("DCORA_FACTOR", "host");
diff --git a/dcora_amd/csrc/env.h b/dcora_amd/csrc/env.h
--- a/dcora_amd/csrc/env.h
+++ b/dcora_amd/csrc/env.h
@@ -8,6 +8,7 @@
 bool generic_solver();
 int solver_tcg();
 int solver_bc();
+bool chain_rides();
 bool factor_on_host();
 bool fill_on_host();
 bool lanczos_sync();
diff --git a/dcora_amd/csrc/kernels.h b/dcora_amd/csrc/kernels.h
--- a/dcora_amd/csrc/kernels.h
+++ b/dcora_amd/csrc/kernels.h
@@ -10,6 +10,7 @@
 constexpr int kMaxPartials = 1024;
 constexpr int kBsrMaxGrid = 4096;
 constexpr int kBlock = 256;
+constexpr int kSpmmTile = 1536;
 
 struct ManiDesc {
   int r, d, n, l, b, k, se;
@@ -88,6 +89,15 @@
   const SolverCtl *ctl = nullptr;
   int seq = 0;
   int gate = 0;
+};
+
+extern std::atomic<long> g_chain_launches;
+inline void count_launch() { g_chain_launches.fetch_add(1, std::memory_order_relaxed); }
+
+struct GradRide {
+  const int *c_rp = nullptr, *c_ci = nullptr;
+  const double *c_v = nullptr, *c_X = nullptr;
+  double *G_out = nullptr;
 };
 
 int spmm_grid(int nrows, int r);
@@ -209,7 +219,8 @@
                           int sel, double *pA, double *pB, double *posenorm, Gate g,
                           const int *agent_start = nullptr, int agents = 0, int *wg_per_agent = nullptr);
 int launch_fused_grad(hipStream_t st, const ManiDesc &m, const CsrDev &Q, Buf2 X, const double *G, Buf2 EG, Buf2 RG,
-                      Buf2 Sblk, int sel, double *pA, double *pB, double *posenorm, Gate g);
+                      Buf2 Sblk, int sel, double *pA, double *pB, double *posenorm, Gate g,
+                      const GradRide *ride = nullptr);
 int launch_g_rgrad(hipStream_t st, const ManiDesc &m, Buf2 X, Buf2 EG, Buf2 RG, Buf2 Sblk, int sel, double *partials,
                    double *posenorm, Gate g);
 void launch_ctl_init(hipStream_t st, SolverCtl *c, double tol, double Delta, double maxDelta, int max_outer,
diff --git a/dcora_amd/csrc/kernels.hip b/dcora_amd/csrc/kernels.hip
--- a/dcora_amd/csrc/kernels.hip
+++ b/dcora_amd/csrc/kernels.hip
@@ -27,6 +27,8 @@
     out[q] = t;
   }
 }
+
+std::atomic<long> g_chain_launches{0};
 
 int vec_grid(long nelem) {
   long g = (nelem + kBlock - 1) / kBlock;
@@ -34,8 +36,6 @@
   if (g > kMaxPartials) g = kMaxPartials;
   return (int)g;
 }
-
-constexpr int kSpmmTile = 1536;
 
 int spmm_grid(int nrows, int r) {
   const int RB = kBlock / r;
@@ -598,6 +598,7 @@
 
 void launch_spmm(hipStream_t st, int r, const CsrDev &A, Buf2 X, int selX, const double *G, Buf2 Y, int selY,
                  double *partials, Gate g) {
+  count_launch();
   const int main_grid = spmm_grid(A.nrows, r);
   const int grid = main_grid + A.n_long * kLongSplit;
   if (partials)
@@ -1559,6 +1560,7 @@
 
 void launch_rtr_init(hipStream_t st, const double *pA, int npA, const double *pB, int npB, SolverCtl *ctl,
                      HostFlags *hf, int seq, CtlInit ci, unsigned *tcg_sync, int nsync) {
+  count_launch();
   hipLaunchKernelGGL(k_rtr_init, dim3(1), dim3(kBlock), 0, st, pA, npA, pB, npB, ctl, hf, seq, ci, tcg_sync, nsync);
 }
 void launch_tcg_begin(hipStream_t st, long nelem, Buf2 grad, double *eta, double *Heta, double *res,
@@ -1579,6 +1581,7 @@
 }
 void launch_rtr_decide(hipStream_t st, const double *pA, int npA, const double *pB, int npB, const double *pC,
                        int npC, SolverCtl *ctl, HostFlags *hf, int seq, unsigned *tcg_sync, int nsync) {
+  count_launch();
   hipLaunchKernelGGL(k_rtr_decide, dim3(1), dim3(kBlock), 0, st, pA, npA, pB, npB, pC, npC, ctl, hf, seq, tcg_sync,
                      nsync);
 }
diff --git a/dcora_amd/csrc/rbcd.h b/dcora_amd/csrc/rbcd.h
--- a/dcora_amd/csrc/rbcd.h
+++ b/dcora_amd/csrc/rbcd.h
@@ -113,6 +113,7 @@
   int team_inner_iter() const { return team_robust() ? inner_rounds : 0; }
   int run_team(int *iters_done, double *cost2_trace, double *gradnorm_trace, int *selected_trace, int *updated_trace,
                int *weight_updates, int *stop_reason);
+  long chain_launches = 0;
   int pack_public(int agent, double *packed_dev);
   int unpack_public(int agent, const double *packed_dev);
 
@@ -121,6 +122,7 @@
   int x_stage_hosted(double *host_area) override;
 
  private:
+  bool chain_rides_ = false;
   bool seq_advanced_ = false;
   int staged_selected_ = -1;
   int staged_iteration_ = -1;
diff --git a/dcora_amd/csrc/rbcd.hip b/dcora_amd/csrc/rbcd.hip
--- a/dcora_amd/csrc/rbcd.hip
+++ b/dcora_amd/csrc/rbcd.hip
@@ -81,6 +81,7 @@
 int RbcdSession::init(const HostDataset &ds, const dcora_rbcd_options &o) {
   t0_ = std::chrono::steady_clock::now();
   opt = o;
+  chain_rides_ = env::chain_rides();
   d = ds.d;
   n = ds.n;
   r = o.r;
@@ -642,7 +643,11 @@
       return DCORA_OK;
     }
     const double *nsrc = a.detached ? a.nbr[opt.acceleration ? 1 : 0].p : Xg.p;
-    launch_spmm(st, r, a.coupling.view(), buf1(nsrc), 0, nullptr, buf1(pb.G.p), 0, nullptr, Gate{});
+    const CsrDev Cv = a.coupling.view();
+    if (chain_rides_ && !a.detached && Cv.n_long == 0)
+      pb.ride_G(Cv, nsrc);
+    else
+      launch_spmm(st, r, Cv, buf1(nsrc), 0, nullptr, buf1(pb.G.p), 0, nullptr, Gate{});
     pb.has_G = true;
     last_solver = &pb;
     if (opt.acceleration) {
@@ -900,12 +905,14 @@
 int RbcdSession::iterate(int selected, double *cost2, double *gradnorm, double *block_norms, int *next_selected) {
   int rc = check_selected(selected);
   if (rc) return rc;
+  const long launches0 = g_chain_launches.load(std::memory_order_relaxed);
   rc = phase_nonselected(selected);
   if (rc) return rc;
   rc = phase_selected(selected);
   if (rc) return rc;
   int nxt = selected;
   rc = evaluate_central(cost2, gradnorm, block_norms, &nxt);
+  chain_launches += g_chain_launches.load(std::memory_order_relaxed) - launches0;
   if (rc) return rc;
   if (next_selected) *next_selected = (agents[selected].coupling.nnz > 0) ? nxt : selected;
   return DCORA_OK;
diff --git a/dcora_amd/csrc/solver_fused.hip b/dcora_amd/csrc/solver_fused.hip
--- a/dcora_amd/csrc/solver_fused.hip
+++ b/dcora_amd/csrc/solver_fused.hip
@@ -371,11 +371,35 @@
   if (threadIdx.x == 0) p1[blockIdx.x] = tot;
 }
 
-template <int D>
+__device__ __forceinline__ double coupling_row(const GradRide &c, int r, int j, int t) {
+  const int RB = kBlock / r;
+  const int pb0 = c.c_rp[(j / RB) * RB];
+  const int myb = c.c_rp[j], mye = c.c_rp[j + 1];
+  double acc = 0;
+  int lo = myb;
+  while (lo < mye) {
+    const int hi = min(mye, pb0 + ((lo - pb0) / kSpmmTile + 1) * kSpmmTile);
+    for (int p = lo; p < hi; p += 8) {
+      double x8[8], w8[8];
+#pragma unroll
+      for (int q = 0; q < 8; ++q) {
+        const bool ok = p + q < hi;
+        const int pp = ok ? p + q : lo;
+        w8[q] = ok ? c.c_v[pp] : 0.0;
+        x8[q] = c.c_X[(size_t)c.c_ci[pp] * r + t];
+      }
+#pragma unroll
+      for (int q = 0; q < 8; ++q) acc = fma(w8[q], x8[q], acc);
+    }
+    lo = hi;
+  }
+  return acc;
+}
+template <int D, bool RIDE>
 __global__ __launch_bounds__(kBlock) void k_fused_grad(ManiDesc m, CsrDev Q, Buf2 Xb, const double *__restrict__ G,
                                                        Buf2 EGb, Buf2 RGb, Buf2 Sb, int sel,
                                                        double *__restrict__ pA, double *__restrict__ pB,
-                                                       double *__restrict__ posenorm, Gate g) {
+                                                       double *__restrict__ posenorm, Gate g, GradRide ride) {
   if (gated(g.ctl, g.seq, g.gate)) return;
   __shared__ int s_ci[kHessTile];
   __shared__ double s_v[kHessTile];
@@ -400,7 +424,15 @@
   const int myb = act ? Q.rp[j] : 0, mye = act ? Q.rp[j + 1] : 0;
   const size_t oown = (size_t)j * r + t;
   const double x_own = act ? X[oown] : 0.0;
-  const double g_own = (act && G) ? G[oown] : 0.0;
+  double g_own = 0.0;
+  if (RIDE) {
+    if (act) {
+      g_own = coupling_row(ride, r, j, t);
+      ride.G_out[oown] = g_own;
+    }
+  } else {
+    g_own = (act && G) ? G[oown] : 0.0;
+  }
   double acc = 0;
   for (int base = pbeg; base < pend; base += kHessTile) {
     const int cnt = min(kHessTile, pend - base);
@@ -2156,6 +2188,7 @@
 void launch_eval_finish(hipStream_t st, int R, const int *pose_start, const double *posenorm, const double *pA,
                         int npA, EvalOut *out_dev, int seq, double *split_scratch, int nposes,
                         const double *agent_partials, int wg_per_agent) {
+  count_launch();
   const bool split = !agent_partials && split_scratch && nposes >= 16384;
   if (split)
     hipLaunchKernelGGL(k_eval_partial, dim3(R * kEvalSplit), dim3(kBlock), 0, st, pose_start, posenorm, split_scratch);
@@ -2241,6 +2274,7 @@
 int launch_fused_hess(hipStream_t st, const ManiDesc &m, const CsrDev &Q, const double *z, const double *d_old,
                       double *d_new, Buf2 X, Buf2 S, double *Hd, const double *p3, int np3, double *p1,
                       SolverCtl *ctl, int seq, int iter, const BsrDev *Ab) {
+  count_launch();
   if (Ab) {
     const int gridb = (m.n + kPosesPerBlock - 1) / kPosesPerBlock;
     if (m.d == 3)
@@ -2402,6 +2436,7 @@
 int launch_tcg_run(hipStream_t st, const ManiDesc &m, int ldm, const double *Minv, const CsrDev &Q, Buf2 grad, Buf2 X,
                    Buf2 S, double *d0, double *d1, double *Hd, double *eta, double *Heta, double *z, double *p1r,
                    double *p3, double *pC, unsigned *sync, SolverCtl *ctl, HostFlags *hf, int seq) {
+  count_launch();
   int fault = 0;
   bool skipped = false;
   for (int sk = g_tcg_run_fault_skip.load(); sk > 0;)
@@ -2450,6 +2485,7 @@
                     const double *delta, const double *Hd, double *eta, double *Heta, const double *res_old,
                     double *res_new, double *z, const double *p1, int np1, double *p3, SolverCtl *ctl, HostFlags *hf,
                     int seq, int iter, int first, double *pC) {
+  count_launch();
   return fused_pc_dispatch(st, m, ldm, Minv, grad, X, delta, Hd, eta, Heta, res_old, res_new, z, p1, np1, p3, ctl, hf,
                            seq, iter, first, pC, false);
 }
@@ -2481,14 +2517,21 @@
   return grid;
 }
 int launch_fused_grad(hipStream_t st, const ManiDesc &m, const CsrDev &Q, Buf2 X, const double *G, Buf2 EG, Buf2 RG,
-                      Buf2 Sblk, int sel, double *pA, double *pB, double *posenorm, Gate g) {
+                      Buf2 Sblk, int sel, double *pA, double *pB, double *posenorm, Gate g, const GradRide *ride) {
   const int grid = fused_pose_blocks(m);
-  if (m.d == 3)
-    hipLaunchKernelGGL(k_fused_grad<3>, dim3(grid), dim3(kBlock), 0, st, m, Q, X, G, EG, RG, Sblk, sel, pA, pB, posenorm,
-                       g);
-  else
-    hipLaunchKernelGGL(k_fused_grad<2>, dim3(grid), dim3(kBlock), 0, st, m, Q, X, G, EG, RG, Sblk, sel, pA, pB, posenorm,
-                       g);
+  const GradRide rd = ride ? *ride : GradRide();
+  count_launch();
+#define DCORA_FUSED_GRAD(D_, RIDE_)                                                                                  \
+  hipLaunchKernelGGL((k_fused_grad<D_, RIDE_>), dim3(grid), dim3(kBlock), 0, st, m, Q, X, G, EG, RG, Sblk, sel, pA, pB, \
+                     posenorm, g, rd)
+  if (m.d == 3) {
+    if (rd.c_rp) DCORA_FUSED_GRAD(3, true);
+    else DCORA_FUSED_GRAD(3, false);
+  } else {
+    if (rd.c_rp) DCORA_FUSED_GRAD(2, true);
+    else DCORA_FUSED_GRAD(2, false);
+  }
+#undef DCORA_FUSED_GRAD
   return grid;
 }
 int launch_g_retract(hipStream_t st, const ManiDesc &m, Buf2 X, const double *V, double alpha, Buf2 out, int selOut,
@@ -2505,6 +2548,7 @@
 void launch_g_nesterov(hipStream_t st, const ManiDesc &m, int mode, int restart, int skip_lo, int skip_hi,
                        double alpha, double gamma, double *X, double *V, double *Y, double *XPrev, double *Yloc,
                        Buf2 Xloc, const SolverCtl *ctl, double *inner_Yloc) {
+  count_launch();
   GNesterovArgs a{mode, restart, skip_lo, skip_hi, alpha, gamma, X, V, Y, XPrev, Yloc, inner_Yloc, Xloc, ctl};
   const int grid = group_grid(m.n);
   if (m.d == 3)
diff --git a/dcora_amd/csrc/team_status.hip b/dcora_amd/csrc/team_status.hip
--- a/dcora_amd/csrc/team_status.hip
+++ b/dcora_amd/csrc/team_status.hip
@@ -40,6 +40,7 @@
 
 void launch_rel_change(hipStream_t st, int r, int d, const double *X, const double *XPrev, const int *pose_start,
                        const RelChangeSet &set, double *out) {
+  count_launch();
   if (set.count < 1) return;
   hipLaunchKernelGGL(k_rel_change, dim3(set.count), dim3(kBlock), 0, st, r, d + 1, X, XPrev, pose_start, set, out);
 }
diff --git a/include/dcora_hip.h b/include/dcora_hip.h
--- a/include/dcora_hip.h
+++ b/include/dcora_hip.h
@@ -177,6 +177,7 @@
 int dcora_rbcd_unpack_public_dev(dcora_rbcd_t s, int agent, const double *packed_dev);
 int dcora_rbcd_phase_nonselected(dcora_rbcd_t s, int selected);
 int dcora_rbcd_phase_selected(dcora_rbcd_t s, int selected);
+int dcora_debug_rbcd_launches(dcora_rbcd_t s, long long *launches);
 int dcora_rbcd_phase_evaluate_dev(dcora_rbcd_t s, double *out_dev);
 int dcora_rbcd_synchronize(dcora_rbcd_t s);
 int dcora_rbcd_profile_tcg_runs(dcora_rbcd_t s, int enable);
```

Result: faster. 4296, median of 6 (+1.6%).
